# dakom/awsm-renderer

Hardware: AMD Instinct MI355X
Metric: frames/sec + shaded Mpix/s, 4K Sponza glTF, 1/2/4/8 MI355X (higher is better)
Workload: dtype f32; 1 GPU; Sponza-class procedural atrium (configs[3]): 262144 triangles, 25 materials, 69 textures, 3840x2160, geometry pass + opaque pass, single-sample, MipmapMode::None; triangles=262144, width=3840, height=2160, draws=92, frame_overlap=True, stream_handoff=device flags (k_handoff_signal / k_handoff_wait), camera=orbit, one turn per 240 frames, environment=uniform cubes (builder default), opaque_route=lean (k_shade_lean + k_shade_todo), library=awsm-renderer_amd/libawsm_hip.so

## Files before the change

__graft_entry__.py:

```python
import os
import subprocess
import sys

ROOT = os.path.dirname(os.path.abspath(__file__))
if ROOT not in sys.path:
    sys.path.insert(0, ROOT)


def build() -> None:
    import awsm_renderer_amd
    from awsm_renderer_amd import build as b
    hip_so, host_so = b.build_all()
    for p in (hip_so, host_so):
        assert os.path.exists(p), p
    from oracle import oracle_lib
    oracle_lib.build()
    mock_dir = os.path.join(ROOT, "tests", "mock")
    subprocess.check_call(["gcc", "-O1", "-std=c11", "-fPIC", "-shared", "-Wall", "-o", os.path.join(mock_dir, "libmock_backend.so"),
                           os.path.join(mock_dir, "mock_backend.c")])
    from awsm_renderer_amd import hip_backend, host
    host.load_library()
    import ctypes
    lib = ctypes.CDLL(hip_so)
    for name in hip_backend.EXPORTS:
        getattr(lib, name)
    print(f"built {hip_so}, {host_so}, oracle + mock; package {awsm_renderer_amd.__name__} imported")


def smoke() -> None:
    import numpy as np
    from awsm_renderer_amd import scenes
    from awsm_renderer_amd.hip_backend import HipDevice
    from awsm_renderer_amd.host import Renderer
    from oracle import oracle_lib
    from tests import helpers

    scene = scenes.helmet_scene(320, 180, segments=48, rings=36, tex_size=64)
    lut = oracle_lib.brdf_lut(32, 32)
    r = Renderer(scene, parity_tap=True, lut_rgba16f=oracle_lib.lut_rg_to_rgba16f(lut))
    stats = r.render(sync=True)
    dev = HipDevice.from_ctx(r.host.device_ctx, scene.width, scene.height)
    model = helpers.build_model(scene)
    orc = helpers.oracle_frame(model, lut)
    res = helpers.compare_frames(orc, dev)
    dev.close()
    r.close()
    assert res["key_mismatch"] == 0 and res["clip_mismatch"] == 0, res
    assert res["rgb_over_tol"] == 0 and res["f16_max_ulp"] <= 2, res
    print("smoke ok:", {k: stats[k] for k in ("ms_total", "triangles_in", "covered_pixels")}, res)


if __name__ == "__main__":
    build()
    if len(sys.argv) > 1 and sys.argv[1] == "smoke":
        smoke()
```

awsm-renderer_amd/build.py:

```python
from __future__ import annotations

import os
import shutil
import subprocess
import sys

from . import PACKAGE_DIR


def _run_make(directory: str, target: str, env=None):
    e = dict(os.environ)
    if env:
        e.update(env)
    proc = subprocess.run(["make", "-C", directory, target], stdout=subprocess.PIPE, stderr=subprocess.STDOUT, text=True, env=e)
    if proc.returncode != 0:
        raise RuntimeError(f"building {target} in {directory} failed:\n{proc.stdout[-4000:]}")
    return proc.stdout


def build_hip(jobs: int = 3, arch: str = "gfx950") -> str:
    hipcc = shutil.which("hipcc") or "/opt/rocm/bin/hipcc"
    if not os.path.exists(hipcc):
        raise RuntimeError("hipcc not found: libawsm_hip.so cannot be built and there is no CPU fallback")
    proc = subprocess.run(["make", "-C", os.path.join(PACKAGE_DIR, "csrc"), f"-j{jobs}", "../libawsm_hip.so", f"HIPCC={hipcc}", f"ARCH={arch}"],
                          stdout=subprocess.PIPE, stderr=subprocess.STDOUT, text=True)
    if proc.returncode != 0:
        raise RuntimeError(f"hipcc build failed:\n{proc.stdout[-4000:]}")
    try:
        over = check_register_budgets(hipcc, arch)
    except (OSError, subprocess.CalledProcessError) as e:
        print(f"awsm-renderer_amd build: VGPR budgets not checked ({e})", file=sys.stderr)
        over = []
    for line in over:
        print("awsm-renderer_amd build: " + line, file=sys.stderr)
    if over and os.environ.get("AWSM_STRICT_VGPR") == "1":
        raise RuntimeError("VGPR budgets exceeded (AWSM_STRICT_VGPR=1):\n" + "\n".join(over))
    return os.path.join(PACKAGE_DIR, "libawsm_hip.so")


VGPR_BUDGETS = {"kernels_shade.o": {"k_shade_leanILb0ELi0ELb0E": 80, "k_shade_todoILi0ELb0E": 112,
                                    "k_shade_leanILb0ELi0ELb1E": 80, "k_shade_leanILb0ELi1ELb0E": 96, "k_shade_leanILb0ELi1ELb1E": 96,
                                    "k_shade_todoILi1ELb0E": 128, "k_shade_todoILi0ELb1E": 128, "k_shade_todoILi1ELb1E": 128},
                "kernels_geometry.o": {"k_deform_transformILb0E": 80, "k_binILb0E": 112, "k_binILb1E": 112, "k_bin_bigILb0E": 112, "k_bin_scan": 112, "k_raster_tileILi1E": 112, "k_raster_tileILi4E": 96,
                                       "k_handoff_signal": 32, "k_handoff_wait": 32}}


def check_register_budgets(hipcc: str, arch: str = "gfx950") -> list:
    import re
    import tempfile
    llvm = os.path.join(os.path.dirname(os.path.dirname(os.path.realpath(hipcc))), "lib", "llvm", "bin")
    if not os.path.exists(os.path.join(llvm, "llvm-objcopy")):
        llvm = "/opt/rocm/lib/llvm/bin"
    over = []
    with tempfile.TemporaryDirectory() as tmp:
        for obj, budgets in VGPR_BUDGETS.items():
            fat, co = os.path.join(tmp, "fat.bin"), os.path.join(tmp, "code.co")
            subprocess.check_call([os.path.join(llvm, "llvm-objcopy"), f"--dump-section=.hip_fatbin={fat}", os.path.join(PACKAGE_DIR, "csrc", obj)])
            subprocess.check_call([os.path.join(llvm, "clang-offload-bundler"), "--unbundle", "--type=o", f"--targets=hipv4-amdgcn-amd-amdhsa--{arch}", f"--input={fat}", f"--output={co}"])
            notes = subprocess.run([os.path.join(llvm, "llvm-readelf"), "--notes", co], stdout=subprocess.PIPE, text=True, check=True).stdout
            found = dict(re.findall(r"\.name:\s+(\S+)\n(?:.*\n)*?\s+\.vgpr_count:\s+(\d+)", notes))
            for key, budget in budgets.items():
                hits = {n: int(v) for n, v in found.items() if key in n}
                if not hits:
                    over.append(f"{obj}: no kernel matching {key} in the code object (budget list out of date?)")
                for n, v in hits.items():
                    if v > budget:
                        over.append(f"{obj}: {n} uses {v} VGPRs, more than the {budget} it may use to be placed beside k_shade_lean (slower overlap, same results)")
    return over


def build_host() -> str:
    _run_make(os.path.join(PACKAGE_DIR, "host"), "../libawsm_host.so")
    return os.path.join(PACKAGE_DIR, "libawsm_host.so")


def build_all():
    return build_hip(), build_host()
```

awsm-renderer_amd/csrc/awsm_hip.cpp:

```cpp
#include <hip/hip_runtime.h>
#include <algorithm>
#include <cmath>
#include <cstdarg>
#include <cstdio>
#include <cstring>
#include <ctime>
#include <string>
#include <vector>

#include "frame_params.hpp"
#include "dirty_log.hpp"

using namespace awsm;

extern "C" {
void awsm_launch_bin_big(const FrameDev* f, int fill, hipStream_t s);
void awsm_launch_gen_mip_level(uint8_t* chain, uint32_t src_off, uint32_t dst_off, uint32_t sw, uint32_t sh, uint32_t dw, uint32_t dh, uint32_t layers,
                               const uint32_t* kinds, hipStream_t s);
void awsm_launch_pick(const DevScene* sc, const FrameDev* f, int x, int y, uint32_t* out, hipStream_t s);
void awsm_launch_transform(const DevScene* sc, const FrameDev* f, uint32_t n_blocks, hipStream_t s);
void awsm_launch_hud_merge(const unsigned long long* world, const unsigned long long* hud, unsigned long long* out, size_t first, size_t n, hipStream_t s);
void awsm_launch_transform_forward(const DevScene* sc, const FrameDev* f, uint32_t n_blocks, hipStream_t s);
void awsm_launch_forward(const DevScene* sc, const FrameDev* f, hipStream_t s);
void awsm_launch_post(const void* args, uint32_t flags, uint32_t msaa, void* bloom_a, void* bloom_b, hipStream_t s);
void awsm_launch_upload_words(void* dst, const void* src_pinned, uint32_t n_words, hipStream_t s);
void awsm_launch_bin_count(const FrameDev* f, hipStream_t s);
void awsm_launch_bin_scan(const FrameDev* f, hipStream_t s);
void awsm_launch_bin_fill(const FrameDev* f, hipStream_t s);
void awsm_launch_raster(const FrameDev* f, hipStream_t s);
void awsm_launch_shade(const DevScene* sc, const FrameDev* f, hipStream_t s);
int awsm_shade_is_lean(const FrameDev* f);
int awsm_launch_shade_todo(const DevScene* sc, const FrameDev* f, hipStream_t s);
void awsm_launch_gbuffer_dump(const FrameDev* f, float* out, hipStream_t s);
void awsm_launch_handoff_signal(uint32_t* flag, uint32_t serial, unsigned long long* stamp, hipStream_t s);
void awsm_launch_handoff_wait(const uint32_t* flag, uint32_t serial, unsigned long long budget_ticks, uint32_t* timeouts_host, uint32_t timeouts_known,
                              uint32_t* poison, uint32_t poison_serial, hipStream_t s);
void awsm_launch_resolve_draws(const DevScene* sc, const FrameDev* f, hipStream_t s);
void awsm_launch_count_covered(const FrameDev* f, hipStream_t s);
void awsm_launch_msaa_halo_export(const FrameDev* f, unsigned long long* dst, uint32_t bands_out, hipStream_t s);
void awsm_launch_vis_digest(const unsigned long long* vis, size_t n, unsigned long long* out, hipStream_t s);
void awsm_launch_brdf_lut(uint32_t* out_rg16f, uint32_t w, uint32_t h, hipStream_t s);
void awsm_launch_cube_border(const awsm::CubeDev* cd, uint2* out, uint32_t total, hipStream_t s);
void awsm_launch_rgba16f_to_rg16f(const uint16_t* in, uint32_t* out, uint32_t n, hipStream_t s);
}

namespace {

#ifndef AWSM_SLOTS
#define AWSM_SLOTS 2
#endif
constexpr int kSlots = AWSM_SLOTS;
constexpr int kLeanWgsPerCu = 0;
struct DevBuf {
    void* ptr = nullptr;
    size_t size = 0;
};

enum { EV_START = 0, EV_TRANSFORM, EV_BIN, EV_RASTER, EV_SHADE_BEGIN, EV_SHADE_LEAN, EV_SHADE, EV_FWD_BEGIN, EV_FWD, EV_COUNT };

struct FrameBufs {
    DevBuf wpos;
    DevBuf frag_rec, frag_color, frag_first;
    uint32_t frag_cap = 0;
    DevBuf tex_slots;
    DevBuf draw_mat;
    DevBuf tri_shade, draw_lean;
    DevBuf clip, nrm, tan, tri_rec, tri_flags, draws_dev, draw_shade, tile_count, tile_offset, tile_cursor, tile_order, bin_list, big_list, counters, vis;
    DevBuf camera;
    DevBuf scan_tmp;
    DevBuf tile_split, raster_scratch;
    uint32_t raster_extra_cap = 0, raster_slot_cap = 0;
    uint32_t bin_capacity = 0;
    float pix2view[16] = {}, view_rot[9] = {}, cam_pos[3] = {}, ortho_view_dir[3] = {};
    uint32_t cam_ortho = 0;
    size_t tri_cap = 0, draw_cap = 0;
    uint32_t sized_w = 0, sized_h = 0;
    std::vector<DrawDev> draws_uploaded;
    void* draws_uploaded_ptr = nullptr;
    bool draws_uploaded_valid = false;
    uint64_t draws_version = 0;
    std::vector<DrawDev> tail_uploaded;
    void* tail_uploaded_ptr = nullptr;
    size_t tail_uploaded_at = 0;
    bool tail_uploaded_valid = false;
    DevBuf wcache, draws_prev;
    DevBuf block_map;
    bool block_map_valid = false;
    DevBuf cache_mark;
    uint32_t cached_n_draws = 0;
    bool cache_valid = false;
    bool cached_is_prev = false;
    bool cache_had_tri_shade = false;
    uint64_t cache_seq = 0;
    uint32_t cache_serial = 0;
};

}

struct AwsmHipCtx {
    int device = 0;
    uint32_t flags = 0;
    hipStream_t stream = nullptr;
    bool own_stream = false;
    bool stage_timers = true;
    std::string last_error;

    DevBuf bufs[AWSM_BUF_COUNT];
    bool camera_written_since_snapshot = false;
    uint8_t camera_host[512] = {};
    DevScene scene{};
    DevScene* scene_dev = nullptr;
    bool scene_dirty = true;
    DevBuf tex[kMaxTexArrays];
    DevBuf lut;
    DevBuf cube_tex[3], cube_bordered[3];

    uint32_t width = 0, height = 0;
    uint32_t y0 = 0, y1 = 0;
    uint32_t band_n = 1, band_r = 0, band_compact = 0;
    uint32_t msaa = 0;
    DevBuf mip_kinds;
    DevBuf msaa_color0[kSlots], msaa_edges[kSlots];
    DevBuf msaa_edge_bits[kSlots];
    DevBuf msaa_cells[kSlots];
    DevBuf out16[kSlots], out32[kSlots];
    DevBuf digest;
    uint32_t lean_grid = 0;
    DevBuf shade_todo[kSlots];
    void* bound_out = nullptr;
    size_t bound_out_bytes = 0;
    const uint8_t* slot_out_lo[kSlots] = {}; const uint8_t* slot_out_hi[kSlots] = {};

    bool overlap = false;
    hipStream_t shade_streams[kSlots] = {};
    bool shade_recorded[kSlots] = {};
    bool uploads_recorded[kSlots] = {};
    struct ResolveKey { uint64_t write_seq, draws_version; const void* ptrs[5]; uint32_t n_draws, mipmap, has_opaque, lights_cap; } resolved[kSlots] = {};
    hipEvent_t ev_geom_done[kSlots] = {}, ev_shade_done[kSlots] = {}, ev_uploads[kSlots] = {} ;
    hipEvent_t ev_flush = nullptr;
    uint64_t write_seq = 0, geom_write_seq[kSlots] = {};
    DirtyLog dirty_log;
    bool geometry_cache = true;
    uint32_t cache_blocks_last = 0;
    bool shade_pending[kSlots] = {};
    bool handoff = false;
    uint32_t* handoff_flags = nullptr;
    uint32_t geom_sig[kSlots] = {}, shade_sig[kSlots] = {}, lean_sig[kSlots] = {};
    bool lean_flagged[kSlots] = {};
    unsigned long long handoff_budget_ticks = 400000000ull;
    uint32_t clock_khz = 100000;
// ... 190 lines not shown
    if (rc) return rc;
    memcpy(st, src, len);
    if (len <= kKernelUploadMax && (len & 3u) == 0 && ((uintptr_t)dst & 3u) == 0 && ((uintptr_t)st & 3u) == 0) {
        awsm_launch_upload_words(dst, st, (uint32_t)(len >> 2), c->stream);
        HIPCHK(c, hipGetLastError());
    } else {
        HIPCHK(c, hipMemcpyAsync(dst, st, len, hipMemcpyHostToDevice, c->stream));
    }
    return AWSM_OK;
}

void shard(const AwsmHipCtx* c, uint32_t* y0, uint32_t* y1) {
    *y0 = c->y0; *y1 = c->y1;
    if (*y1 == 0 || *y1 > c->height) *y1 = c->height;
    if (*y0 > *y1) *y0 = *y1;
}

void log_dirty(AwsmHipCtx* c, AwsmBuf which, size_t lo, size_t hi) {
    if (c->geometry_cache) c->dirty_log.log((uint32_t)which, lo, hi, c->write_seq);
}

int scene_write_barrier(AwsmHipCtx* c, bool is_write = true) {
    if (is_write) c->write_seq++;
    if (!c->overlap) return AWSM_OK;
    for (int s = 0; s < kSlots; s++)
        if (c->shade_pending[s]) { HIPCHK(c, hipStreamWaitEvent(c->stream, c->ev_shade_done[s], 0)); c->shade_pending[s] = false; }
    return AWSM_OK;
}
int sync_all(AwsmHipCtx* c) {
    HIPCHK(c, hipStreamSynchronize(c->stream));
    HIPCHK(c, sync_shade_streams(c));
    for (bool& b : c->shade_pending) b = false;
    return AWSM_OK;
}

int sync_scene(AwsmHipCtx* c) {
    if (!c->scene_dirty) return AWSM_OK;
    c->write_seq++;
    { int rcb = scene_write_barrier(c, false); if (rcb) return rcb; }
    for (int i = 0; i < AWSM_BUF_COUNT; i++) c->scene.buf[i] = (const uint8_t*)c->bufs[i].ptr;
    c->scene.lut_rg16f = (const uint16_t*)c->lut.ptr;
    int rc = upload_small(c, c->scene_dev, &c->scene, sizeof(DevScene));
    if (rc) return rc;
    c->scene_dirty = false;
    return AWSM_OK;
}

void fill_frame(AwsmHipCtx* c, FrameDev* f) {
    memset(f, 0, sizeof *f);
    uint32_t y0, y1;
    shard(c, &y0, &y1);
    f->width = c->width; f->height = c->height; f->y0 = y0; f->y1 = y1; f->sy0 = y0; f->sy1 = y1;
    if (c->msaa && (y0 > 0 || y1 < c->height)) {
        f->y0 = y0 > 0 ? y0 - 1 : 0; f->y1 = std::min(c->height, y1 + 1);
    }
    f->tiles_x = (c->width + kTile - 1) / kTile;
    f->band_n = 1; f->band_r = 0; f->out_compact = 0;
    f->tile_row0 = f->y0 >> kTileShift;
    f->tiles_y = (f->y1 > f->y0) ? ((f->y1 + kTile - 1) / kTile - f->tile_row0) : 0;
    if (c->band_n > 1) {
        const uint32_t rows_full = (c->height + kTile - 1) / kTile;
        f->band_n = c->band_n; f->band_r = c->band_r; f->out_compact = c->band_compact;
        f->tile_row0 = c->band_r;
        f->tiles_y = c->band_r < rows_full ? (rows_full - c->band_r + c->band_n - 1) / c->band_n : 0;
    }
    f->n_draws = (uint32_t)c->draws_host.size();
    f->total_tris = c->total_tris; f->total_verts = c->total_verts;
    f->bin_capacity = FB(c).bin_capacity;
    f->draws = (const DrawDev*)FB(c).draws_dev.ptr;
    f->draw_shade = (DrawShadeDev*)FB(c).draw_shade.ptr;
    f->tex_slots = (TexSlotDev*)FB(c).tex_slots.ptr;
    f->draw_mat = (DrawMatDev*)FB(c).draw_mat.ptr;
    f->clip = (float4*)FB(c).clip.ptr; f->nrm = (float4*)FB(c).nrm.ptr; f->tan = (float4*)FB(c).tan.ptr;
    f->tri_info = (uint32_t*)FB(c).tri_flags.ptr;
    const bool lean_ok = !(c->flags & AWSM_CFG_GENERAL_SHADE_ONLY) && (uint64_t)c->width * c->height * (c->msaa == 4 ? 32u : 8u) < (1ull << 32) && (c->msaa == 0 || (c->msaa_edge_bits[c->slot].ptr && c->msaa_cells[c->slot].ptr)) && FB(c).tri_shade.ptr && FB(c).draw_lean.ptr && c->shade_todo[c->slot].ptr && ((uint64_t)c->total_tris + (c->hud_merged ? c->hud_total_tris : 0u)) * kTriRecBytes < (1ull << 32) &&
                         c->bufs[AWSM_BUF_ATTR_DATA].size < (1ull << 32) - 64;
    f->tri_shade = lean_ok ? (uint4*)FB(c).tri_shade.ptr : nullptr;
    f->attr_data_bytes = (uint32_t)std::min<size_t>(c->bufs[AWSM_BUF_ATTR_DATA].size, 0xFFFFFFFFu);
    f->draw_lean = lean_ok ? (LeanDrawDev*)FB(c).draw_lean.ptr : nullptr;
    f->shade_todo = (uint32_t*)c->shade_todo[c->slot].ptr;
    f->shade_todo_cap = f->shade_todo ? (uint32_t)(c->shade_todo[c->slot].size / 4 - 4 - 1024) : 0u;
    f->lean_next = f->shade_todo ? f->shade_todo + 4 + f->shade_todo_cap : nullptr;
    f->lean_grid = c->lean_grid;
    f->tri_rec = (TriRec*)FB(c).tri_rec.ptr;
    f->tile_count = (uint32_t*)FB(c).tile_count.ptr; f->tile_offset = (uint32_t*)FB(c).tile_offset.ptr;
    f->tile_cursor = (uint32_t*)FB(c).tile_cursor.ptr; f->bin_list = (uint32_t*)FB(c).bin_list.ptr;
    f->tile_order = (uint32_t*)FB(c).tile_order.ptr;
    f->scan_tmp = (uint32_t*)FB(c).scan_tmp.ptr;
    f->tile_split = (uint32_t*)FB(c).tile_split.ptr; f->raster_scratch = (unsigned long long*)FB(c).raster_scratch.ptr;
    f->raster_extra_cap = FB(c).raster_extra_cap; f->raster_slot_cap = FB(c).raster_slot_cap;
    f->big_list = (uint32_t*)FB(c).big_list.ptr;
    f->counters = (uint32_t*)FB(c).counters.ptr;
#ifdef AWSM_STAMP
    {
        static unsigned long long* stamps = nullptr;
        if (!stamps && hipMalloc((void**)&stamps, 4ull * 16384 * 8 * 8) == hipSuccess) (void)hipMemset(stamps, 0, 4ull * 16384 * 8 * 8);
        f->stamps = stamps;
        static bool told = false;
        if (!told) { told = true; FILE* fp = fopen("/tmp/awsm_stamps_ptr", "w"); if (fp) { fprintf(fp, "%llu\n", (unsigned long long)(uintptr_t)stamps); fclose(fp); } }
    }
#endif
    f->poison = c->handoff_poison ? c->handoff_poison + c->slot : nullptr;
    f->host_bin_status = c->counters_host + 16 + 2 * c->slot;
    f->frame_serial = c->frame_serial;
    f->vis = (unsigned long long*)FB(c).vis.ptr;
    f->camera = (const uint8_t*)FB(c).camera.ptr;
    f->camera_snap = nullptr; f->camera_snap_words = 0;
    memcpy(f->pix2view, FB(c).pix2view, sizeof f->pix2view); memcpy(f->view_rot, FB(c).view_rot, sizeof f->view_rot); memcpy(f->cam_pos, FB(c).cam_pos, sizeof f->cam_pos);
    memcpy(f->ortho_view_dir, FB(c).ortho_view_dir, sizeof f->ortho_view_dir); f->cam_ortho = FB(c).cam_ortho;
    f->msaa = c->msaa;
    f->msaa_color0 = (float4*)c->msaa_color0[c->slot].ptr;
    f->msaa_edges = (uint32_t*)c->msaa_edges[c->slot].ptr;
    f->msaa_edge_bits = (lean_ok && c->msaa == 4) ? (unsigned long long*)c->msaa_edge_bits[c->slot].ptr : nullptr;
    f->msaa_cells = (uint2*)c->msaa_cells[c->slot].ptr;
    f->hud_vis = c->hud_geometry_done ? (const unsigned long long*)c->hud[c->slot].vis.ptr : nullptr;
    f->hud_draws = (const DrawDev*)c->hud[c->slot].draws_dev.ptr; f->hud_tri_info = (const uint32_t*)c->hud[c->slot].tri_flags.ptr;
    if (c->hud_geometry_done && c->hud_merged) {
        f->n_draws = (uint32_t)c->hud_combined.size();
        f->total_tris = c->total_tris + c->hud_total_tris; f->total_verts = 3u * f->total_tris;
        f->vis = (unsigned long long*)c->merged_vis[c->slot].ptr;
        f->hud_draws = f->draws; f->hud_tri_info = f->tri_info;
    }
    f->hud_pass = 0;
    f->msaa_halo = (const unsigned long long*)c->msaa_halo;
    f->halo_bands = c->band_n > 1 ? ((c->height + kTile - 1) / kTile + c->band_n - 1) / c->band_n : 0u;
    f->out_rgba16f = (uint16_t*)(c->bound_out ? (uint8_t*)c->bound_out - (size_t)c->out_first_row * c->width * 8 : c->out16[c->slot].ptr);
    f->out_rgba32f = (float*)c->out32[c->slot].ptr;
    f->lights_pre = (float4*)c->lights_pre[c->slot].ptr;
    f->lights_cap = (uint32_t)(c->lights_pre[c->slot].size / 32);
}

void compose_pixel_to_view(AwsmHipCtx* c, FrameBufs& b) {
    float cam[128];
    memcpy(cam, c->camera_host, 512);
    const float* proj = cam + 16; const float* inv_proj = cam + 64; const float* inv_view = cam + 80;
    const double W = (double)c->width, H = (double)c->height;
    const double A[16] = {2.0 / W, 0, 0, 0,   0, -2.0 / H, 0, 0,   0, 0, 1, 0,   1.0 / W - 1.0, 1.0 - 1.0 / H, 0, 1};
    for (int col = 0; col < 4; col++) for (int row = 0; row < 4; row++) {
        double s = 0.0;
        for (int k = 0; k < 4; k++) s += (double)inv_proj[k * 4 + row] * A[col * 4 + k];
        b.pix2view[col * 4 + row] = (float)s;
    }
    for (int col = 0; col < 3; col++) for (int row = 0; row < 3; row++) b.view_rot[col * 3 + row] = inv_view[col * 4 + row];
    for (int i = 0; i < 3; i++) b.cam_pos[i] = cam[96 + i];
    b.cam_ortho = proj[15] > 0.9f ? 1u : 0u;
    const double vx = inv_view[8], vy = inv_view[9], vz = inv_view[10], l = std::sqrt(vx * vx + vy * vy + vz * vz);
    b.ortho_view_dir[0] = l > 0.0 ? (float)(vx / l) : 0.0f; b.ortho_view_dir[1] = l > 0.0 ? (float)(vy / l) : 0.0f; b.ortho_view_dir[2] = l > 0.0 ? (float)(vz / l) : 1.0f;
}

int record(AwsmHipCtx* c, int which, hipStream_t s = nullptr) {
    if (!c->stage_timers) { c->ev_valid[which] = false; return AWSM_OK; }
    HIPCHK(c, hipEventRecord(c->ev[which], s ? s : c->stream));
    c->ev_valid[which] = true;
    return AWSM_OK;
}

AwsmHipCtx::ResolveKey resolve_key(AwsmHipCtx* c, const FrameDev& f) {
    AwsmHipCtx::ResolveKey k;
    memset(&k, 0, sizeof k);
    k.write_seq = c->write_seq + (c->scene_dirty ? 1u : 0u); k.draws_version = FB(c).draws_version;
    k.ptrs[0] = f.draw_shade; k.ptrs[1] = f.draw_mat; k.ptrs[2] = f.tex_slots; k.ptrs[3] = f.draw_lean; k.ptrs[4] = f.lights_pre;
    k.n_draws = f.n_draws; k.mipmap = c->last_opaque.mipmap; k.has_opaque = c->last_opaque.has_opaque; k.lights_cap = f.lights_cap;
    return k;
}
bool resolve_stale(AwsmHipCtx* c, const FrameDev& f) {
    const AwsmHipCtx::ResolveKey k = resolve_key(c, f);
    return memcmp(&k, &c->resolved[c->slot], sizeof k) != 0;
// ... 82 lines not shown
    HostTrace ht(c->frame_serial);
    FrameDev f;
    fill_frame(c, &f);
    f.has_opaque = c->last_opaque.has_opaque;
    f.mipmap = c->last_opaque.mipmap;
    f.aniso = (c->flags & AWSM_CFG_ANISOTROPIC) ? 1u : 0u;
    if (c->bound_out) {
        if (c->out_rows_mode) {
            if (f.out_compact || f.sy0 < c->out_first_row || (size_t)(f.sy1 - c->out_first_row) * c->width * 8 > c->bound_out_bytes)
                return fail(c, AWSM_ERR_INVALID_ARGUMENT, "opaque_pass: bound output starts at row %u and holds %zu bytes, the shard shades rows [%u, %u)", c->out_first_row, c->bound_out_bytes, f.sy0, f.sy1);
        } else {
            const size_t need = (f.out_compact ? (size_t)f.tiles_y * kTile : (size_t)c->height) * c->width * 8;
            if (c->bound_out_bytes < need) return fail(c, AWSM_ERR_INVALID_ARGUMENT, "opaque_pass: bound output holds %zu bytes, this shard layout writes %zu", c->bound_out_bytes, need);
        }
    }
    int rc = sync_scene(c);
    if (rc) return rc;
    hipStream_t ss = shade_stream_of(c);
    const bool want_resolve = f.sy1 > f.sy0 && f.has_opaque && (resolve_stale(c, f) || c->stage_timers);
    if (want_resolve) c->resolved[c->slot] = resolve_key(c, f);
    const bool early = c->uploads_recorded[c->slot] && c->overlap && !c->stage_timers && want_resolve && c->geometry_done && c->geom_write_seq[c->slot] == c->write_seq;
    if (early) {
        HIPCHK(c, hipStreamWaitEvent(ss, c->ev_uploads[c->slot], 0));
        awsm_launch_resolve_draws(c->scene_dev, &f, ss);
    }
    ht.mark("opaque: sync_scene + early resolve");
    if (c->overlap) {
        if (c->handoff) {
            ++c->geom_sig[c->slot];
            if (c->handoff_test_drop) c->handoff_test_drop--;
            else awsm_launch_handoff_signal(c->handoff_flags + c->slot, c->geom_sig[c->slot], trace_slot(c, 1), c->stream);
            awsm_launch_handoff_wait(c->handoff_flags + c->slot, c->geom_sig[c->slot], c->handoff_budget_ticks, handoff_timeouts(c), c->handoff_timeouts_seen, c->handoff_poison + c->slot, c->frame_serial, ss);
        } else {
            if (c->trace_dev) awsm_launch_handoff_signal(nullptr, 0u, trace_slot(c, 1), c->stream);
            HIPCHK(c, hipEventRecord(c->ev_geom_done[c->slot], c->stream));
            HIPCHK(c, hipStreamWaitEvent(ss, c->ev_geom_done[c->slot], 0));
        }
        const uint8_t* lo = (const uint8_t*)c->bound_out; const uint8_t* hi = lo ? lo + c->bound_out_bytes : nullptr;
        const int p = prev_slot(c);
        const bool same_image = lo && c->slot_out_lo[p] && lo < c->slot_out_hi[p] && c->slot_out_lo[p] < hi;
        if (c->shade_recorded[p]) HIPCHK(c, wait_prev_slot(c, ss, !(same_image || (c->msaa != 0 && c->msaa_halo))));
        c->slot_out_lo[c->slot] = lo; c->slot_out_hi[c->slot] = hi;
    }
    ht.mark("opaque: hand-off launches");
    if (want_resolve && !early) awsm_launch_resolve_draws(c->scene_dev, &f, ss);
    if ((rc = record(c, EV_SHADE_BEGIN, ss))) return rc;
    c->ev_valid[EV_SHADE_LEAN] = false;
    c->lean_flagged[c->slot] = false;
    if (c->overlap && c->handoff && f.sy1 > f.sy0 && awsm_shade_is_lean(&f)) {
        f.lean_done_flag = c->handoff_flags + 2 * kSlots + c->slot; f.lean_done_serial = ++c->lean_sig[c->slot];
        c->lean_flagged[c->slot] = true;
    }
    if (f.sy1 > f.sy0) {
        awsm_launch_shade(c->scene_dev, &f, ss);
        if (c->stage_timers && awsm_shade_is_lean(&f) && (rc = record(c, EV_SHADE_LEAN, ss))) return rc;
        (void)awsm_launch_shade_todo(c->scene_dev, &f, ss);
    }
    if ((rc = record(c, EV_SHADE, ss))) return rc;
    ht.mark("opaque: shade launches");
    if (c->overlap) HIPCHK(c, mark_shade_done(c, ss));
    else if (c->trace_dev) awsm_launch_handoff_signal(nullptr, 0u, trace_slot(c, 2), ss);
    ht.mark("opaque: shade-done signal + event");
    HIPCHK(c, hipGetLastError());
    return AWSM_OK;
}

inline FrameBufs& TR(AwsmHipCtx* c) { return (c->hud_transparent ? c->htr : c->tr)[c->slot]; }

void fill_frame_forward(AwsmHipCtx* c, FrameDev* f) {
    fill_frame(c, f);
    FrameBufs& t = TR(c);
    const int which = c->hud_transparent ? 1 : 0;
    f->vis = (unsigned long long*)FB(c).vis.ptr;
    f->n_draws = (uint32_t)c->tr_draws_host[which].size();
    f->total_tris = c->tr_total_tris[which]; f->total_verts = 3u * c->tr_total_tris[which];
    f->bin_capacity = t.bin_capacity;
    f->draws = (const DrawDev*)t.draws_dev.ptr;
    f->draw_shade = (DrawShadeDev*)t.draw_shade.ptr;
    f->tex_slots = (TexSlotDev*)t.tex_slots.ptr;
    f->draw_mat = (DrawMatDev*)t.draw_mat.ptr;
    f->clip = (float4*)t.clip.ptr; f->nrm = (float4*)t.nrm.ptr; f->tan = (float4*)t.tan.ptr; f->wpos = (float4*)t.wpos.ptr;
    f->tri_info = (uint32_t*)t.tri_flags.ptr;
    f->tri_shade = nullptr; f->draw_lean = nullptr; f->shade_todo = nullptr; f->shade_todo_cap = 0; f->lean_next = nullptr; f->lean_grid = 0;
    f->tri_rec = (TriRec*)t.tri_rec.ptr;
    f->tile_count = (uint32_t*)t.tile_count.ptr; f->tile_offset = (uint32_t*)t.tile_offset.ptr;
    f->tile_cursor = (uint32_t*)t.tile_cursor.ptr; f->bin_list = (uint32_t*)t.bin_list.ptr;
    f->tile_order = (uint32_t*)t.tile_order.ptr;
    f->scan_tmp = (uint32_t*)t.scan_tmp.ptr;
    f->tile_split = (uint32_t*)t.tile_split.ptr; f->raster_scratch = nullptr;
    f->raster_extra_cap = 0; f->raster_slot_cap = 0;
    f->big_list = (uint32_t*)t.big_list.ptr;
    f->counters = (uint32_t*)t.counters.ptr;
    f->opaque_rgba16f = c->opaque_src ? (const uint16_t*)c->opaque_src : f->out_rgba16f;
    f->out_compact = 0;
    f->frag_rec = (uint4*)t.frag_rec.ptr; f->frag_color = (float4*)t.frag_color.ptr; f->frag_first = (uint32_t*)t.frag_first.ptr; f->frag_cap = t.frag_cap;
    f->out_rgba16f = (uint16_t*)(c->bound_comp ? c->bound_comp : c->comp16.ptr);
    f->out_rgba32f = (float*)c->comp32.ptr;
    f->has_opaque = c->last_opaque.has_opaque;
    f->mipmap = c->last_opaque.mipmap;
    f->aniso = (c->flags & AWSM_CFG_ANISOTROPIC) ? 1u : 0u;
    if (c->hud_transparent) {
        f->hud_pass = 1;
        f->opaque_rgba16f = f->out_rgba16f;
    }
}

int enqueue_transparent(AwsmHipCtx* c) {
    FrameDev f;
    fill_frame_forward(c, &f);
    const uint32_t n_tiles = f.tiles_x * f.tiles_y;
    int rc = sync_scene(c);
    if (rc) return rc;
    hipStream_t ss = shade_stream_of(c);
    if (c->overlap && c->shade_recorded[prev_slot(c)]) HIPCHK(c, wait_prev_slot(c, ss));
    if ((rc = record(c, EV_FWD_BEGIN, ss))) return rc;
    const bool has_geometry = f.total_tris && n_tiles;
    if (!has_geometry) {
        HIPCHK(c, hipMemsetAsync(TR(c).counters.ptr, 0, 8 * sizeof(uint32_t), ss));
        HIPCHK(c, hipMemsetAsync((uint32_t*)TR(c).counters.ptr + 12, 0, 2 * sizeof(uint32_t), ss));
        if (n_tiles) HIPCHK(c, hipMemsetAsync(TR(c).tile_count.ptr, 0, n_tiles * sizeof(uint32_t), ss));
    } else {
        awsm_launch_resolve_draws(c->scene_dev, &f, ss);
        awsm_launch_transform_forward(c->scene_dev, &f, c->tr_n_blocks[c->hud_transparent ? 1 : 0], ss);
    }
    if (n_tiles) {
        if (f.total_tris) { awsm_launch_bin_count(&f, ss); awsm_launch_bin_big(&f, 0, ss); }
        awsm_launch_bin_scan(&f, ss);
        if (f.total_tris) { awsm_launch_bin_fill(&f, ss); awsm_launch_bin_big(&f, 1, ss); }
        awsm_launch_forward(c->scene_dev, &f, ss);
    }
    if ((rc = record(c, EV_FWD, ss))) return rc;
    if (c->overlap) HIPCHK(c, mark_shade_done(c, ss));
    HIPCHK(c, hipGetLastError());
    return AWSM_OK;
}

int ensure_bin_capacity_of(AwsmHipCtx* c, FrameBufs& b, uint32_t entries) {
    if (entries <= b.bin_capacity && b.bin_list.ptr) return AWSM_OK;
    uint32_t cap = std::max(entries, b.bin_capacity + b.bin_capacity / 2);
    int rc = dev_realloc(c, b.bin_list, (size_t)cap * 4, false);
    if (rc) return rc;
    b.bin_capacity = cap;
    return AWSM_OK;
}

int ensure_fragment_capacity(AwsmHipCtx* c, FrameBufs& b, uint32_t fragments) {
    if (fragments <= b.frag_cap && b.frag_rec.ptr) return AWSM_OK;
    const uint32_t cap = std::max(fragments, b.frag_cap + b.frag_cap / 2);
    int rc = dev_realloc(c, b.frag_rec, (size_t)cap * 16, false);
    if (!rc) rc = dev_realloc(c, b.frag_color, (size_t)cap * 16, false);
    if (rc) return rc;
    b.frag_cap = cap;
    return AWSM_OK;
}

int build_draw_list(AwsmHipCtx* c, const char* pass, const AwsmDraw* draws, uint32_t n, AwsmBuf data, uint32_t bytes_per_tri,
                    std::vector<DrawDev>& out, uint64_t* tris_out, uint64_t* blocks_out) {
    out.clear();
    uint64_t tris = 0, blocks = 0;
    for (uint32_t i = 0; i < n; i++) {
        const AwsmDraw& d = draws[i];
        if (d.inst_count != 0) {
            const DevBuf& ib = c->bufs[AWSM_BUF_INSTANCES];
            if (!ib.ptr) return fail(c, AWSM_ERR_NOT_READY, "%s: draw %u: instanced, but the instance-transform buffer was never created", pass, i);
            if ((d.inst_off & 15u) || (uint64_t)d.inst_off + 64ull * d.inst_count > ib.size)
                return fail(c, AWSM_ERR_OUT_OF_RANGE, "%s: draw %u: %u instances at %u exceed the instance-transform buffer", pass, i, d.inst_count, d.inst_off);
        }
        if (d.vis_data_off & (bytes_per_tri ? 15u : 3u)) return fail(c, AWSM_ERR_INVALID_ARGUMENT, "%s: draw %u: vertex data offset %u misaligned", pass, i, d.vis_data_off);
        if ((uint64_t)d.vis_data_off + (uint64_t)bytes_per_tri * d.tri_count > c->bufs[data].size || (!bytes_per_tri && d.tri_count && (uint64_t)d.vis_data_off + 40 > c->bufs[data].size))
            return fail(c, AWSM_ERR_OUT_OF_RANGE, "%s: draw %u: %u triangles at %u exceed the vertex buffer", pass, i, d.tri_count, d.vis_data_off);
        if ((uint64_t)d.geom_meta_off + 40 > c->bufs[AWSM_BUF_GEOM_META].size || (d.geom_meta_off & 3u))
            return fail(c, AWSM_ERR_OUT_OF_RANGE, "%s: draw %u: geometry meta offset %u out of range", pass, i, d.geom_meta_off);
        if (d.tri_count == 0) continue;
        const uint32_t copies = d.inst_count ? d.inst_count : 1u;
        for (uint32_t k = 0; k < copies; k++) {
            DrawDev dd{};
            dd.geom_meta_off = d.geom_meta_off; dd.vis_data_off = d.vis_data_off; dd.tri_count = d.tri_count; dd.flags = d.flags & 0x7Fu;
            if (d.inst_count) { dd.flags |= kDrawInstanced; dd.inst_off = d.inst_off + 64u * k; }
            dd.first_tri = (uint32_t)tris; dd.first_block = (uint32_t)blocks;
            out.push_back(dd);
            tris += d.tri_count;
            blocks += (3ull * d.tri_count + 255) / 256;
            if (tris > 0x55555555ull) return fail(c, AWSM_ERR_UNSUPPORTED, "%s: more than 2^32/3 triangles in one pass", pass);
            if (out.size() >= (1u << 24)) return fail(c, AWSM_ERR_UNSUPPORTED, "%s: more than 2^24 non-empty draws (instances included) in one pass", pass);
        }
    }
    *tris_out = tris; *blocks_out = blocks;
    return AWSM_OK;
}

int reserve_raster_items(AwsmHipCtx* c, FrameBufs& b, bool forward) {
    const uint32_t tiles_x = (c->width + kTile - 1) / kTile, tiles_y_full = (c->height + kTile - 1) / kTile;
    const size_t n_tiles_full = (size_t)tiles_x * tiles_y_full;
    const uint32_t extra_cap = forward ? 0u : b.bin_capacity / 256u + 1u, slot_cap = forward ? 0u : b.bin_capacity / 128u + 2u;
    int rc;
    if ((rc = dev_reserve(c, b.tile_order, (n_tiles_full + extra_cap) * 4))) return rc;
    if (!forward && (rc = dev_reserve(c, b.raster_scratch, (size_t)slot_cap * kTile * kTile * 8 * (c->msaa == 4u ? 4u : 1u)))) return rc;
    b.raster_extra_cap = extra_cap; b.raster_slot_cap = slot_cap;
    return AWSM_OK;
}

int size_pass_buffers(AwsmHipCtx* c, FrameBufs& b, size_t tri_cap, size_t draw_cap, bool forward) {
    int rc;
    const size_t nd = std::max<size_t>(draw_cap, 1), nv = std::max<size_t>(3 * tri_cap, 1), nt = std::max<size_t>(tri_cap, 1);
    if ((rc = dev_reserve(c, b.draws_dev, nd * sizeof(DrawDev)))) return rc;
    const bool world_pass = &b >= c->fb && &b < c->fb + kSlots;
    if (world_pass && c->geometry_cache) {
        if ((rc = dev_reserve(c, b.draws_prev, nd * sizeof(DrawDev)))) return rc;
        if ((rc = dev_reserve(c, b.wcache, nv * 16))) return rc;
        const size_t blocks_bound = nv / 256 + nd + 1;
        if ((rc = dev_reserve(c, b.block_map, blocks_bound * 4))) return rc;
        b.block_map_valid = false;
        if (b.cache_mark.size < blocks_bound * 4) { if ((rc = dev_realloc(c, b.cache_mark, (blocks_bound + blocks_bound / 2) * 4, true))) return rc; }
    }
    b.cache_valid = false;
    if ((rc = dev_reserve(c, b.draw_shade, nd * sizeof(DrawShadeDev)))) return rc;
    if ((rc = dev_reserve(c, b.tex_slots, nd * kCoreTextures * sizeof(TexSlotDev)))) return rc;
    if ((rc = dev_reserve(c, b.draw_mat, nd * sizeof(DrawMatDev)))) return rc;
    if ((rc = dev_reserve(c, b.clip, nv * 16))) return rc;
    if ((rc = dev_reserve(c, b.nrm, nv * 16))) return rc;
    if ((rc = dev_reserve(c, b.tan, nv * 16))) return rc;
    if (forward && (rc = dev_reserve(c, b.wpos, nv * 16))) return rc;
    if ((rc = dev_reserve(c, b.tri_flags, nt * 4))) return rc;
    if (!forward && (rc = dev_reserve(c, b.tri_shade, nt * 32))) return rc;
    if (!forward && (rc = dev_reserve(c, b.draw_lean, nd * sizeof(LeanDrawDev)))) return rc;
    if ((rc = dev_reserve(c, b.big_list, nt * 4))) return rc;
    if ((rc = dev_reserve(c, b.tri_rec, nt * kTriRecBytes))) return rc;
    const uint32_t tiles_x = (c->width + kTile - 1) / kTile, tiles_y_full = (c->height + kTile - 1) / kTile;
    const size_t n_tiles_full = (size_t)tiles_x * tiles_y_full;
    if ((rc = dev_reserve(c, b.tile_count, n_tiles_full * 4))) return rc;
    if ((rc = dev_reserve(c, b.tile_offset, (n_tiles_full + 1) * 4))) return rc;
    if ((rc = dev_reserve(c, b.tile_cursor, n_tiles_full * 4))) return rc;
    if ((rc = dev_reserve(c, b.tile_split, n_tiles_full * 8))) return rc;
    if ((rc = dev_reserve(c, b.scan_tmp, (((n_tiles_full + 255) / 256) * 2 + 1) * 40 * 4))) return rc;
    if ((rc = ensure_bin_capacity_of(c, b, (c->flags & AWSM_CFG_SMALL_BIN_LIST) ? 4096u : (uint32_t)std::min<size_t>(std::max<size_t>(4 * tri_cap + 65536u, 1u << 18), 0xFFFFFFF0u)))) return rc;
    if ((rc = reserve_raster_items(c, b, forward))) return rc;
    b.tri_cap = tri_cap; b.draw_cap = draw_cap; b.sized_w = c->width; b.sized_h = c->height;
    return AWSM_OK;
}

int ensure_pass_capacity(AwsmHipCtx* c, FrameBufs& b, const std::vector<DrawDev>& draws_host, uint32_t total_tris, bool forward) {
    int rc;
    if (total_tris > b.tri_cap || draws_host.size() > b.draw_cap || b.sized_w != c->width || b.sized_h != c->height || !b.bin_list.ptr) {
        bool instanced = false;
        for (const DrawDev& d : draws_host) instanced |= (d.flags & kDrawInstanced) != 0;
        const size_t tri_bound = forward || instanced ? ~size_t(0) : c->bufs[AWSM_BUF_VIS_GEOM_DATA].size / 168u;
        const size_t tri_cap = std::max<size_t>(std::min<size_t>((size_t)total_tris + total_tris / 4 + 4096, std::max<size_t>(tri_bound, total_tris)), b.tri_cap);
        const size_t draw_cap = std::max<size_t>(draws_host.size() + draws_host.size() / 4 + 64, b.draw_cap);
        FrameBufs* set = forward ? ((&b >= c->htr && &b < c->htr + kSlots) ? c->htr : c->tr) : ((&b >= c->hud && &b < c->hud + kSlots) ? c->hud : c->fb);
        for (int sl = 0; sl < n_slots(c); sl++) {
            FrameBufs& t = set[(c->slot + sl) % kSlots];
            if ((rc = size_pass_buffers(c, t, std::max(tri_cap, t.tri_cap), std::max(draw_cap, t.draw_cap), forward))) return rc;
        }
    }
    return AWSM_OK;
}

int upload_draws_at(AwsmHipCtx* c, FrameBufs& b, size_t at, const std::vector<DrawDev>& list) {
    const size_t bytes = list.size() * sizeof(DrawDev);
    uint8_t* dst = (uint8_t*)b.draws_dev.ptr + at * sizeof(DrawDev);
    if (bytes <= (1u << 20)) return upload_small(c, dst, list.data(), bytes);
    HIPCHK(c, hipMemcpyAsync(dst, list.data(), bytes, hipMemcpyHostToDevice, c->stream));
    HIPCHK(c, hipStreamSynchronize(c->stream));
    return AWSM_OK;
}

int upload_draw_list(AwsmHipCtx* c, FrameBufs& b, const std::vector<DrawDev>& draws_host, bool keep_prev) {
    const bool same_draws = b.draws_uploaded_valid && b.draws_uploaded_ptr == b.draws_dev.ptr && b.draws_uploaded.size() == draws_host.size() &&
                            (draws_host.empty() || memcmp(b.draws_uploaded.data(), draws_host.data(), draws_host.size() * sizeof(DrawDev)) == 0);
    auto upload_block_map = [&]() -> int {
        b.block_map_valid = false;
        if (!keep_prev || !b.block_map.ptr) return AWSM_OK;
        std::vector<uint32_t> map;
        for (size_t i = 0; i < draws_host.size(); i++) map.insert(map.end(), (3ull * draws_host[i].tri_count + 255) / 256, (uint32_t)i);
        if (map.size() * 4 > b.block_map.size || map.size() * 4 > (1u << 20)) return AWSM_OK;
        const int rc = upload_small(c, b.block_map.ptr, map.data(), map.size() * 4);
        if (!rc) b.block_map_valid = true;
        return rc;
    };
    if (draws_host.empty()) return AWSM_OK;
    if (same_draws) return (keep_prev && !b.block_map_valid) ? upload_block_map() : AWSM_OK;
    if (keep_prev && b.cache_valid && !b.cached_is_prev && b.draws_prev.ptr && b.draws_prev.size == b.draws_dev.size) {
        std::swap(b.draws_dev, b.draws_prev);
        b.cached_is_prev = true;
    } else if (keep_prev && !b.cached_is_prev) b.cache_valid = false;
    b.draws_uploaded = draws_host; b.draws_uploaded_ptr = b.draws_dev.ptr; b.draws_uploaded_valid = true; b.draws_version++;
    b.tail_uploaded_valid = false;
    { const int rc = upload_block_map(); if (rc) return rc; }
    return upload_draws_at(c, b, 0, draws_host);
}

int reserve_pass_buffers(AwsmHipCtx* c, FrameBufs& b, const std::vector<DrawDev>& draws_host, uint32_t total_tris, bool forward) {
    int rc = ensure_pass_capacity(c, b, draws_host, total_tris, forward);
    if (rc) return rc;
    return upload_draw_list(c, b, draws_host, !forward && &b >= c->fb && &b < c->fb + kSlots);
}

uint32_t mip_levels_full(uint32_t w, uint32_t h) {
    uint32_t m = std::max(w, h), n = 0;
    while (m > 1u) { m >>= 1; n++; }
    return n + 1u;
}

int ensure_bin_capacity(AwsmHipCtx* c, uint32_t entries) { return ensure_bin_capacity_of(c, FB(c), entries); }

}

extern "C" {

uint32_t awsm_hip_abi_version(void) { return AWSM_HIP_ABI_VERSION; }
// ... 20 lines not shown
    }
    if (cfg->stream) { c->stream = (hipStream_t)cfg->stream; c->own_stream = false; }
    else { if (hipStreamCreateWithFlags(&c->stream, hipStreamNonBlocking) != hipSuccess) return bail(AWSM_ERR_DEVICE); c->own_stream = true; }
    for (int i = 0; i < EV_COUNT; i++) if (hipEventCreate(&c->ev[i]) != hipSuccess) return bail(AWSM_ERR_DEVICE);
    if (hipMalloc((void**)&c->scene_dev, sizeof(DevScene)) != hipSuccess) return bail(AWSM_ERR_OUT_OF_MEMORY);
    c->overlap = (cfg->flags & AWSM_CFG_OVERLAP_FRAMES) != 0;
    { const char* e = getenv("AWSM_GEOMETRY_CACHE"); c->geometry_cache = !(e && e[0] == '0'); }
    {
        const char* e = getenv("AWSM_LEAN_WGS_PER_CU");
        const int per_cu = e ? atoi(e) : (c->overlap ? kLeanWgsPerCu : 0);
        c->lean_grid = per_cu > 0 ? (uint32_t)(per_cu * prop.multiProcessorCount) & ~7u : 0u;
    }
    for (int s = 0; s < n_slots(c); s++) {
        if (hipMalloc(&c->fb[s].counters.ptr, 16 * sizeof(uint32_t)) != hipSuccess || hipMemset(c->fb[s].counters.ptr, 0, 16 * sizeof(uint32_t)) != hipSuccess) return bail(AWSM_ERR_OUT_OF_MEMORY);
        c->fb[s].counters.size = 16 * sizeof(uint32_t);
        if (hipMalloc(&c->tr[s].counters.ptr, 16 * sizeof(uint32_t)) != hipSuccess) return bail(AWSM_ERR_OUT_OF_MEMORY);
        c->tr[s].counters.size = 16 * sizeof(uint32_t);
        if (hipMalloc(&c->htr[s].counters.ptr, 16 * sizeof(uint32_t)) != hipSuccess) return bail(AWSM_ERR_OUT_OF_MEMORY);
        c->htr[s].counters.size = 16 * sizeof(uint32_t);
        if (hipMalloc(&c->hud[s].counters.ptr, 16 * sizeof(uint32_t)) != hipSuccess) return bail(AWSM_ERR_OUT_OF_MEMORY);
        c->hud[s].counters.size = 16 * sizeof(uint32_t);
        if (hipMalloc(&c->fb[s].camera.ptr, 512) != hipSuccess || hipMemset(c->fb[s].camera.ptr, 0, 512) != hipSuccess) return bail(AWSM_ERR_OUT_OF_MEMORY);
        c->fb[s].camera.size = 512;
    }

    if (c->overlap) {
        for (int s = 0; s < kSlots; s++) {
#ifdef AWSM_DEBUG_SWITCHES
            if (const char* m = getenv("AWSM_SHADE_CU_MASK")) {
                std::vector<uint32_t> words;
                for (const char* p = m; *p; ) { char* end = nullptr; words.push_back((uint32_t)strtoul(p, &end, 16)); p = (*end == ',') ? end + 1 : end; if (end == p && *p) break; }
                if (words.empty() || hipExtStreamCreateWithCUMask(&c->shade_streams[s], (uint32_t)words.size(), words.data()) != hipSuccess) return bail(AWSM_ERR_DEVICE);
            } else
#endif
            if (hipStreamCreateWithFlags(&c->shade_streams[s], hipStreamNonBlocking) != hipSuccess) return bail(AWSM_ERR_DEVICE);
            const unsigned ev_flags = hipEventDisableTiming | hipEventReleaseToDevice;
            if (hipEventCreateWithFlags(&c->ev_geom_done[s], ev_flags) != hipSuccess || hipEventCreateWithFlags(&c->ev_shade_done[s], ev_flags) != hipSuccess ||
                hipEventCreateWithFlags(&c->ev_uploads[s], ev_flags) != hipSuccess) return bail(AWSM_ERR_DEVICE);
            if (s == 0 && hipEventCreateWithFlags(&c->ev_flush, hipEventDisableTiming) != hipSuccess) return bail(AWSM_ERR_DEVICE);
        }
    }
    if (hipHostMalloc((void**)&c->counters_host, (16 + 2 * kSlots + 1) * sizeof(uint32_t), hipHostMallocDefault) != hipSuccess) return bail(AWSM_ERR_OUT_OF_MEMORY);
    memset(c->counters_host, 0, (16 + 2 * kSlots + 1) * sizeof(uint32_t));
    if (c->overlap) {
        const char* e = getenv("AWSM_DEVICE_HANDOFF");
        c->handoff = !(e && e[0] == '0');
        { int khz = 0; if (hipDeviceGetAttribute(&khz, hipDeviceAttributeWallClockRate, c->device) == hipSuccess && khz > 0) c->clock_khz = (uint32_t)khz; }
        double budget_ms = 4000.0;
        if (const char* p = getenv("AWSM_HANDOFF_TIMEOUT_MS")) { const double v = atof(p); if (v > 0.0) budget_ms = v; }
        c->handoff_budget_ticks = (unsigned long long)(budget_ms * (double)c->clock_khz) + 1ull;
        if (hipMalloc((void**)&c->handoff_flags, 3 * kSlots * sizeof(uint32_t)) != hipSuccess || hipMalloc((void**)&c->handoff_poison, kSlots * sizeof(uint32_t)) != hipSuccess) return bail(AWSM_ERR_OUT_OF_MEMORY);
        if (hipMemset(c->handoff_flags, 0, 3 * kSlots * sizeof(uint32_t)) != hipSuccess || hipMemset(c->handoff_poison, 0xFF, kSlots * sizeof(uint32_t)) != hipSuccess ||
            hipDeviceSynchronize() != hipSuccess) return bail(AWSM_ERR_DEVICE);
        if (const char* d = getenv("AWSM_TEST_HANDOFF_DROP")) c->handoff_test_drop = (uint32_t)atoi(d);
        for (int k = 0; c->handoff && k < 2 * kSlots; k++) {
            hipStream_t ss = c->shade_streams[k % kSlots], waiter = k < kSlots ? ss : c->stream, setter = k < kSlots ? c->stream : ss;
            const uint32_t serial = ++c->geom_sig[0];
            awsm_launch_handoff_wait(c->handoff_flags, serial, 10ull * c->clock_khz , handoff_timeouts(c), 0u, nullptr, 0u, waiter);
            awsm_launch_handoff_signal(c->handoff_flags, serial, nullptr, setter);
            if (hipStreamSynchronize(waiter) != hipSuccess || hipStreamSynchronize(setter) != hipSuccess) return bail(AWSM_ERR_DEVICE);
            if (*(volatile uint32_t*)handoff_timeouts(c) != 0u) { c->handoff = false; c->handoff_timeouts_seen = *(volatile uint32_t*)handoff_timeouts(c); }
        }
    }
    memset(&c->scene, 0, sizeof c->scene);
    c->scene.skybox_rgba[3] = 1.0f;
    for (int i = 0; i < 3; i++) { c->scene.prefiltered_rgb[i] = 1.0f; c->scene.irradiance_rgb[i] = 1.0f; }
    *out = c;
    return AWSM_OK;
}

int awsm_hip_destroy(AwsmHipCtx* c) {
    if (!c) return AWSM_ERR_INVALID_ARGUMENT;
    (void)hipSetDevice(c->device);
    if (c->stream) (void)hipStreamSynchronize(c->stream);
    (void)sync_shade_streams(c);
    auto fr = [](DevBuf& b) { if (b.ptr) (void)hipFree(b.ptr); b.ptr = nullptr; b.size = 0; };
    for (auto& b : c->bufs) fr(b);
    for (auto& b : c->tex) fr(b);
    for (auto& b : c->merged_vis) fr(b);
    fr(c->lut); for (auto& b : c->cube_tex) fr(b); for (auto& b : c->cube_bordered) fr(b); fr(c->digest); for (auto& b : c->shade_todo) fr(b); for (int sl = 0; sl < kSlots; sl++) { fr(c->msaa_color0[sl]); fr(c->msaa_edges[sl]); fr(c->msaa_edge_bits[sl]); fr(c->msaa_cells[sl]); } fr(c->mip_kinds); for (auto& b : c->out16) fr(b); for (auto& b : c->out32) fr(b); fr(c->comp16); fr(c->comp32); for (auto& b : c->lights_pre) fr(b);
    for (auto& b : c->display8) fr(b); fr(c->effects16); fr(c->bloom_a); fr(c->bloom_b); fr(c->dof_lc); fr(c->dof_blur);
    for (int k = 0; k < 4 * kSlots; k++) {
        FrameBufs& b = k < kSlots ? c->fb[k] : (k < 2 * kSlots ? c->tr[k - kSlots] : (k < 3 * kSlots ? c->hud[k - 2 * kSlots] : c->htr[k - 3 * kSlots]));
        fr(b.vis); fr(b.wpos); fr(b.frag_rec); fr(b.frag_color); fr(b.frag_first); fr(b.tex_slots); fr(b.draw_mat); fr(b.clip); fr(b.nrm); fr(b.tan); fr(b.tri_rec); fr(b.tri_flags); fr(b.tri_shade); fr(b.draw_lean); fr(b.draws_dev); fr(b.draw_shade); fr(b.tile_count); fr(b.tile_offset);
        fr(b.wcache); fr(b.draws_prev); fr(b.cache_mark); fr(b.block_map); fr(b.tile_cursor); fr(b.tile_order); fr(b.scan_tmp); fr(b.tile_split); fr(b.raster_scratch); fr(b.bin_list); fr(b.big_list); fr(b.counters); fr(b.camera);
    }
    for (hipStream_t st : c->shade_streams) if (st) (void)hipStreamDestroy(st);
    for (int i = 0; i < kSlots; i++) { if (c->ev_geom_done[i]) (void)hipEventDestroy(c->ev_geom_done[i]); if (c->ev_shade_done[i]) (void)hipEventDestroy(c->ev_shade_done[i]); if (c->ev_uploads[i]) (void)hipEventDestroy(c->ev_uploads[i]); }
    if (c->ev_flush) (void)hipEventDestroy(c->ev_flush);
    if (c->scene_dev) (void)hipFree(c->scene_dev);
    if (c->stage) (void)hipHostFree(c->stage);
    if (c->counters_host) (void)hipHostFree(c->counters_host);
    if (c->handoff_flags) (void)hipFree(c->handoff_flags);
    if (c->handoff_poison) (void)hipFree(c->handoff_poison);
    if (c->trace_dev) (void)hipFree(c->trace_dev);
    for (int i = 0; i < EV_COUNT; i++) if (c->ev[i]) (void)hipEventDestroy(c->ev[i]);
    if (c->own_stream && c->stream) (void)hipStreamDestroy(c->stream);
    delete c;
    return AWSM_OK;
}

int awsm_hip_device_info(AwsmHipCtx* c, char* name_out, size_t name_cap, uint32_t* cu_count, uint64_t* hbm_bytes) {
    if (!c) return AWSM_ERR_INVALID_ARGUMENT;
    hipDeviceProp_t prop;
    HIPCHK(c, hipGetDeviceProperties(&prop, c->device));
    if (name_out && name_cap) snprintf(name_out, name_cap, "%s (%s)", prop.name, prop.gcnArchName);
    if (cu_count) *cu_count = (uint32_t)prop.multiProcessorCount;
    if (hbm_bytes) *hbm_bytes = (uint64_t)prop.totalGlobalMem;
    return AWSM_OK;
}

int awsm_hip_buffer_create(AwsmHipCtx* c, AwsmBuf which, size_t bytes) {
    if (!c || (int)which < 0 || which >= AWSM_BUF_COUNT) return fail(c, AWSM_ERR_INVALID_ARGUMENT, "buffer_create: bad buffer id %d", (int)which);
    HIPCHK(c, hipSetDevice(c->device));
    { int rcb = scene_write_barrier(c); if (rcb) return rcb; }
    log_dirty(c, which, 0, ~size_t(0));
    if (bytes && c->bufs[which].ptr && c->bufs[which].size == bytes) {
        if (which == AWSM_BUF_CAMERA) memset(c->camera_host, 0, sizeof c->camera_host);
        HIPCHK(c, hipMemsetAsync(c->bufs[which].ptr, 0, bytes + 16, c->stream));
        return AWSM_OK;
    }
    int rc = dev_realloc(c, c->bufs[which], bytes ? bytes + 16 : 0, true);
    if (rc) return rc;
    if (bytes) c->bufs[which].size = bytes;
    if (which == AWSM_BUF_CAMERA) memset(c->camera_host, 0, sizeof c->camera_host);
    if (which == AWSM_BUF_LIGHTS) for (int sl = 0; sl < n_slots(c); sl++) if ((rc = dev_realloc(c, c->lights_pre[sl], std::max<size_t>(bytes / 64, 1) * 32, true))) return rc;
    c->scene_dirty = true;
    return AWSM_OK;
}

int awsm_hip_buffer_write(AwsmHipCtx* c, AwsmBuf which, size_t dst_off, const void* src, size_t len) {
    if (!c || (int)which < 0 || which >= AWSM_BUF_COUNT || (!src && len)) return fail(c, AWSM_ERR_INVALID_ARGUMENT, "buffer_write: bad argument");
    if ((dst_off & 3) || (len & 3)) return fail(c, AWSM_ERR_INVALID_ARGUMENT, "buffer_write: offset %zu / size %zu not 4-byte aligned", dst_off, len);
    DevBuf& b = c->bufs[which];
    if (!b.ptr) return fail(c, AWSM_ERR_NOT_READY, "buffer_write: buffer %d was never created", (int)which);
    if (dst_off > b.size || len > b.size - dst_off) return fail(c, AWSM_ERR_OUT_OF_RANGE, "buffer_write: [%zu,+%zu) outside buffer %d of %zu bytes", dst_off, len, (int)which, b.size);
    if (len == 0) return AWSM_OK;
    HIPCHK(c, hipSetDevice(c->device));
    if (which != AWSM_BUF_CAMERA) { int rcb = scene_write_barrier(c); if (rcb) return rcb; log_dirty(c, which, dst_off, dst_off + len); }
    else { if (dst_off < 512) memcpy(c->camera_host + dst_off, src, std::min<size_t>(len, 512 - dst_off)); c->camera_written_since_snapshot = true; }
    uint8_t* dst = (uint8_t*)b.ptr + dst_off;
    if (len <= (1u << 20)) return upload_small(c, dst, src, len);
    HIPCHK(c, hipMemcpyAsync(dst, src, len, hipMemcpyHostToDevice, c->stream));
    HIPCHK(c, hipStreamSynchronize(c->stream));
    return AWSM_OK;
}

int awsm_hip_resize(AwsmHipCtx* c, uint32_t width, uint32_t height, uint32_t msaa) {
    if (!c || width == 0 || height == 0 || width > 16384 || height > 16384) return fail(c, AWSM_ERR_INVALID_ARGUMENT, "resize: bad size %ux%u", width, height);
    if (msaa == 1) msaa = 0;
    if (msaa != 0 && msaa != 4) return fail(c, AWSM_ERR_UNSUPPORTED, "resize: MSAA x%u (the reference supports None or 4, anti_alias.rs:28-38)", msaa);
    HIPCHK(c, hipSetDevice(c->device));
    const size_t px = (size_t)width * height, samples = msaa == 4 ? 4 : 1;
    int rc;
    if ((rc = sync_all(c))) return rc;
    for (int s = 0; s < n_slots(c); s++) {
        if ((rc = dev_realloc(c, c->fb[s].vis, px * samples * 8, false))) return rc;
        HIPCHK(c, hipMemsetAsync(c->fb[s].vis.ptr, 0xFF, px * samples * 8, c->stream));
    }
    if (msaa == 4) for (int sl = 0; sl < n_slots(c); sl++) {
        const size_t blocks = (size_t)((width + 15) / 16) * ((height + 15) / 16);
        if ((rc = dev_realloc(c, c->msaa_edge_bits[sl], blocks * 4 * 16, true))) return rc;
        if ((rc = dev_realloc(c, c->msaa_cells[sl], px * 8, false))) return rc;
        if ((rc = dev_realloc(c, c->msaa_color0[sl], px * 16, false))) return rc;
        if ((rc = dev_realloc(c, c->msaa_edges[sl], blocks * 260, false))) return rc;
    }
    c->msaa = msaa;
// ... 197 lines not shown
    c->scene_dirty = true;
    return AWSM_OK;
}

int awsm_hip_read_brdf_lut(AwsmHipCtx* c, uint16_t* out) {
    if (!c || !out) return AWSM_ERR_INVALID_ARGUMENT;
    if (!c->lut.ptr) return fail(c, AWSM_ERR_NOT_READY, "no BRDF LUT");
    HIPCHK(c, hipSetDevice(c->device));
    HIPCHK(c, hipStreamSynchronize(c->stream));
    HIPCHK(c, hipMemcpy(out, c->lut.ptr, (size_t)c->scene.lut_w * c->scene.lut_h * 4, hipMemcpyDeviceToHost));
    return AWSM_OK;
}

int awsm_hip_geometry_pass(AwsmHipCtx* c, const AwsmDraw* draws, uint32_t n) {
    if (!c || (!draws && n)) return AWSM_ERR_INVALID_ARGUMENT;
    if (c->width == 0) return fail(c, AWSM_ERR_NOT_READY, "geometry_pass before resize");
    static const AwsmBuf need[] = {AWSM_BUF_TRANSFORMS, AWSM_BUF_CAMERA, AWSM_BUF_GEOM_META, AWSM_BUF_VIS_GEOM_DATA};
    if (n) for (AwsmBuf b : need) if (!c->bufs[b].ptr) return fail(c, AWSM_ERR_NOT_READY, "geometry_pass: buffer %d missing", (int)b);
    HIPCHK(c, hipSetDevice(c->device));

    HostTrace ht(c->frame_serial + 1u);
    std::vector<DrawDev> new_draws;
    uint64_t tris = 0, blocks = 0;
    int rc = build_draw_list(c, "geometry_pass", draws, n, AWSM_BUF_VIS_GEOM_DATA, 168u, new_draws, &tris, &blocks);
    if (rc) return rc;
    ht.mark("geometry_pass: draw list");
    if ((rc = handoff_check(c))) return rc;
    c->hud_geometry_done = false; c->hud_merged = false;
    c->frame_serial++;
    if (c->overlap) {
        c->slot = (c->slot + 1) % kSlots;
        if (c->shade_pending[c->slot]) {
            if (hipEventQuery(c->ev_shade_done[c->slot]) != hipSuccess) HIPCHK(c, wait_slot_free(c));
            c->shade_pending[c->slot] = false;
        }
    }
    ht.mark("geometry_pass: slot-free wait");
    c->draws_api.assign(draws, draws + n);
    c->draws_host.swap(new_draws);
    {
        uint32_t need = 0;
        for (int s = 0; s < kSlots; s++) {
            const volatile uint32_t* st = c->counters_host + 16 + 2 * s;
            const uint32_t entries = st[0], serial = st[1];
            if (serial == c->status_seen[s]) continue;
            c->status_seen[s] = serial;
            if (serial >> 31) c->dropped_frames++;
            need = std::max(need, entries);
        }
        for (int s = 0; s < n_slots(c); s++)
            if (need && (uint64_t)need * 4 > (uint64_t)c->fb[s].bin_capacity * 3 && c->fb[s].bin_list.ptr && !(c->flags & AWSM_CFG_SMALL_BIN_LIST)) {
                if ((rc = ensure_bin_capacity_of(c, c->fb[s], need + need / 2 + 1024))) return rc;
                if ((rc = reserve_raster_items(c, c->fb[s], false))) return rc;
            }
    }
    c->total_tris = (uint32_t)tris; c->total_verts = (uint32_t)(3 * tris); c->n_blocks = (uint32_t)blocks;
    ht.mark("geometry_pass: bin capacity");
    compose_pixel_to_view(c, FB(c));
    if ((rc = reserve_pass_buffers(c, FB(c), c->draws_host, c->total_tris, false))) return rc;
    ht.mark("geometry_pass: reserve + draw-list upload");
    if ((rc = enqueue_geometry(c))) return rc;
    c->camera_written_since_snapshot = false;
    c->geometry_done = true; c->opaque_done = false; c->transparent_done = false; c->hud_transparent_done = false; c->hud_geometry_done = false; c->post_done = false;
    return AWSM_OK;
}

static int enqueue_hud_geometry(AwsmHipCtx* c) {
    FrameBufs& hb = c->hud[c->slot];
    FrameDev f;
    { const bool hd = c->hud_geometry_done; c->hud_geometry_done = false; fill_frame(c, &f); c->hud_geometry_done = hd; }
    f.bin_capacity = hb.bin_capacity;
    f.shade_todo = nullptr; f.shade_todo_cap = 0; f.lean_next = nullptr; f.lean_grid = 0;
    if (c->hud_merged) {
        f.n_draws = (uint32_t)c->hud_combined.size();
        f.total_tris = c->total_tris + c->hud_total_tris; f.total_verts = 3u * f.total_tris;
        f.rank0 = c->total_tris; f.block0 = c->n_blocks;
    } else {
    f.n_draws = (uint32_t)c->hud_draws_host.size();
    f.total_tris = c->hud_total_tris; f.total_verts = 3u * c->hud_total_tris;
    f.draws = (const DrawDev*)hb.draws_dev.ptr;
    f.clip = (float4*)hb.clip.ptr; f.nrm = (float4*)hb.nrm.ptr; f.tan = (float4*)hb.tan.ptr;
    f.tri_info = (uint32_t*)hb.tri_flags.ptr;
    f.tri_shade = nullptr; f.draw_lean = nullptr;
    f.tri_rec = (TriRec*)hb.tri_rec.ptr;
    }
    f.tile_count = (uint32_t*)hb.tile_count.ptr; f.tile_offset = (uint32_t*)hb.tile_offset.ptr;
    f.tile_cursor = (uint32_t*)hb.tile_cursor.ptr; f.bin_list = (uint32_t*)hb.bin_list.ptr;
    f.tile_order = (uint32_t*)hb.tile_order.ptr; f.scan_tmp = (uint32_t*)hb.scan_tmp.ptr;
    f.tile_split = (uint32_t*)hb.tile_split.ptr; f.raster_scratch = (unsigned long long*)hb.raster_scratch.ptr;
    f.raster_extra_cap = hb.raster_extra_cap; f.raster_slot_cap = hb.raster_slot_cap;
    f.big_list = (uint32_t*)hb.big_list.ptr;
    f.counters = (uint32_t*)hb.counters.ptr;
    f.host_bin_status = nullptr;
    f.camera_snap = nullptr; f.camera_snap_words = 0;
    f.vis = (unsigned long long*)hb.vis.ptr;
    f.hud_vis = nullptr;
    int rc;
    if ((rc = sync_scene(c))) return rc;
    const uint32_t n_tiles = f.tiles_x * f.tiles_y;
    awsm_launch_transform(c->scene_dev, &f, c->hud_n_blocks, c->stream);
    if (n_tiles) {
        awsm_launch_bin_count(&f, c->stream); awsm_launch_bin_big(&f, 0, c->stream);
        awsm_launch_bin_scan(&f, c->stream);
        awsm_launch_bin_fill(&f, c->stream); awsm_launch_bin_big(&f, 1, c->stream);
        awsm_launch_raster(&f, c->stream);
    }
    if (c->hud_merged) {
        const size_t spp = c->msaa == 4 ? 4 : 1, first = (size_t)f.y0 * c->width * spp, n = (size_t)(f.y1 - f.y0) * c->width * spp;
        awsm_launch_hud_merge((const unsigned long long*)FB(c).vis.ptr, (const unsigned long long*)hb.vis.ptr, (unsigned long long*)c->merged_vis[c->slot].ptr, first, n, c->stream);
    }
    HIPCHK(c, hipGetLastError());
    return AWSM_OK;
}

int awsm_hip_hud_geometry_pass(AwsmHipCtx* c, const AwsmDraw* draws, uint32_t n) {
    if (!c || (!draws && n)) return AWSM_ERR_INVALID_ARGUMENT;
    if (!c->geometry_done || c->opaque_done) return fail(c, AWSM_ERR_NOT_READY, "hud_geometry_pass goes between the geometry pass and the opaque pass of a frame");
    HIPCHK(c, hipSetDevice(c->device));
    uint64_t tris = 0, blocks = 0;
    int rc = build_draw_list(c, "hud_geometry_pass", draws, n, AWSM_BUF_VIS_GEOM_DATA, 168u, c->hud_draws_host, &tris, &blocks);
    if (rc) return rc;
    c->hud_total_tris = (uint32_t)tris; c->hud_n_blocks = (uint32_t)blocks;
    c->hud_merged = false;
    if (!tris) { c->hud_geometry_done = false; return AWSM_OK; }
    FrameBufs& hb = c->hud[c->slot];
    const size_t px = (size_t)c->width * c->height, spp = c->msaa == 4 ? 4 : 1;
    if ((rc = dev_reserve(c, hb.vis, px * 8 * spp))) return rc;
    if ((rc = reserve_pass_buffers(c, hb, c->hud_draws_host, c->hud_total_tris, false))) return rc;
    if (c->msaa == 4) {
        if ((uint64_t)c->total_tris + tris > 0x55555555ull) return fail(c, AWSM_ERR_UNSUPPORTED, "hud_geometry_pass: more than 2^32/3 triangles in the frame");
        c->hud_combined = c->draws_host;
        for (DrawDev d : c->hud_draws_host) { d.first_tri += c->total_tris; d.first_block += c->n_blocks; c->hud_combined.push_back(d); }
        if (c->hud_combined.size() >= (1u << 24)) return fail(c, AWSM_ERR_UNSUPPORTED, "hud_geometry_pass: more than 2^24 draws in the frame");
        FrameBufs& wb = FB(c);
        const void* before[3] = {wb.clip.ptr, wb.tri_rec.ptr, wb.tri_flags.ptr};
        if ((rc = ensure_pass_capacity(c, wb, c->hud_combined, c->total_tris + c->hud_total_tris, false))) return rc;
        if ((rc = upload_draw_list(c, wb, c->draws_host, true))) return rc;
        {
            const size_t at = c->draws_host.size();
            const std::vector<DrawDev> tail(c->hud_combined.begin() + (long)at, c->hud_combined.end());
            const bool same = wb.tail_uploaded_valid && wb.tail_uploaded_ptr == wb.draws_dev.ptr && wb.tail_uploaded_at == at && wb.tail_uploaded.size() == tail.size() &&
                              memcmp(wb.tail_uploaded.data(), tail.data(), tail.size() * sizeof(DrawDev)) == 0;
            if (!same) {
                if ((rc = upload_draws_at(c, wb, at, tail))) return rc;
                wb.tail_uploaded = tail; wb.tail_uploaded_ptr = wb.draws_dev.ptr; wb.tail_uploaded_at = at; wb.tail_uploaded_valid = true; wb.draws_version++;
                c->uploads_recorded[c->slot] = false;
            }
        }
        if ((rc = dev_reserve(c, c->merged_vis[c->slot], px * 8 * spp))) return rc;
        if (before[0] != wb.clip.ptr || before[1] != wb.tri_rec.ptr || before[2] != wb.tri_flags.ptr) {
            if ((rc = enqueue_geometry(c, true))) return rc;
        }
        c->hud_merged = true;
    }
    if ((rc = enqueue_hud_geometry(c))) return rc;
    c->hud_geometry_done = true;
    return AWSM_OK;
}

int awsm_hip_opaque_pass(AwsmHipCtx* c, const AwsmOpaqueParams* p) {
    if (!c || !p) return AWSM_ERR_INVALID_ARGUMENT;
    if (p->mipmap > 1) return fail(c, AWSM_ERR_INVALID_ARGUMENT, "opaque_pass: mipmap must be 0 (MipmapMode::None) or 1 (MipmapMode::Gradient)");
    if (c->width == 0) return fail(c, AWSM_ERR_NOT_READY, "opaque_pass before resize");
    if (p->has_opaque) {
        if (!c->geometry_done) return fail(c, AWSM_ERR_NOT_READY, "opaque_pass before geometry_pass");
        static const AwsmBuf need[] = {AWSM_BUF_CAMERA, AWSM_BUF_GEOM_META, AWSM_BUF_MATERIAL_META, AWSM_BUF_MATERIALS, AWSM_BUF_ATTR_INDEX,
                                       AWSM_BUF_ATTR_DATA, AWSM_BUF_TEXTURE_TRANSFORMS, AWSM_BUF_LIGHTS_INFO, AWSM_BUF_LIGHTS};
        for (AwsmBuf b : need) if (!c->bufs[b].ptr) return fail(c, AWSM_ERR_NOT_READY, "opaque_pass: buffer %d missing", (int)b);
        if (!c->lut.ptr) return fail(c, AWSM_ERR_NOT_READY, "opaque_pass: no BRDF LUT (env_upload or brdf_lut_generate)");
    }
    if (c->msaa == 4 && c->band_n > 1 && p->has_opaque) {
        const size_t need = (size_t)c->band_n * awsm_hip_msaa_halo_bands(c) * 2 * c->width * 8;
        if (!c->msaa_halo || c->msaa_halo_bytes < need)
            return fail(c, AWSM_ERR_NOT_READY, "opaque_pass: MSAA with band sharding needs the gathered halo keys (awsm_hip_msaa_halo_export -> all-gather -> awsm_hip_msaa_halo_bind, %zu bytes)", need);
    }
    HIPCHK(c, hipSetDevice(c->device));
    c->last_opaque = *p;
    if (!p->has_opaque && c->camera_written_since_snapshot && c->bufs[AWSM_BUF_CAMERA].ptr) {
        int rcs = sync_all(c);
        if (rcs) return rcs;
        compose_pixel_to_view(c, FB(c));
        HIPCHK(c, hipMemcpy(FB(c).camera.ptr, c->bufs[AWSM_BUF_CAMERA].ptr, std::min<size_t>(512, c->bufs[AWSM_BUF_CAMERA].size), hipMemcpyDeviceToDevice));
        c->camera_written_since_snapshot = false;
    }
    int rc = enqueue_opaque(c);
    if (rc) return rc;
    c->opaque_done = true; c->transparent_done = false; c->hud_transparent_done = false;
    return AWSM_OK;
}

static int transparent_pass_body(AwsmHipCtx* c, const AwsmDraw* draws, uint32_t n, bool hud);
static int transparent_pass_impl(AwsmHipCtx* c, const AwsmDraw* draws, uint32_t n, bool hud) {
    const int rc = transparent_pass_body(c, draws, n, hud);
    if (c) c->hud_transparent = false;
    return rc;
}
static int transparent_pass_body(AwsmHipCtx* c, const AwsmDraw* draws, uint32_t n, bool hud) {
    if (!c || (!draws && n)) return AWSM_ERR_INVALID_ARGUMENT;
    if (!c->geometry_done || !c->opaque_done) return fail(c, AWSM_ERR_NOT_READY, "transparent_pass needs the geometry and opaque passes of the same frame first");
    if (hud && !c->transparent_done) return fail(c, AWSM_ERR_NOT_READY, "hud_transparent_pass draws over the composite: call transparent_pass first (n_draws = 0 is valid)");
    c->hud_transparent = hud;
    const bool sharded = c->band_n > 1 || (c->y1 != 0 && !(c->y0 == 0 && c->y1 >= c->height));
    if (sharded && !c->opaque_src)
        return fail(c, AWSM_ERR_UNSUPPORTED, "transparent_pass on a sharded context: screen-space transmission reads the whole opaque image — gather it and bind it with awsm_hip_bind_opaque_source first");
    if (c->opaque_src && c->opaque_src_bytes < (size_t)c->width * c->height * 8)
        return fail(c, AWSM_ERR_INVALID_ARGUMENT, "transparent_pass: the bound opaque source holds %zu bytes, the frame needs %zu", c->opaque_src_bytes, (size_t)c->width * c->height * 8);
    static const AwsmBuf need[] = {AWSM_BUF_TRANSFORMS, AWSM_BUF_CAMERA, AWSM_BUF_GEOM_META, AWSM_BUF_MATERIAL_META, AWSM_BUF_MATERIALS, AWSM_BUF_ATTR_INDEX,
                                   AWSM_BUF_ATTR_DATA, AWSM_BUF_TEXTURE_TRANSFORMS, AWSM_BUF_LIGHTS_INFO, AWSM_BUF_LIGHTS, AWSM_BUF_TRANSPARENCY_GEOM_DATA};
    if (n) {
        for (AwsmBuf b : need) if (!c->bufs[b].ptr) return fail(c, AWSM_ERR_NOT_READY, "transparent_pass: buffer %d missing", (int)b);
        if (!c->lut.ptr) return fail(c, AWSM_ERR_NOT_READY, "transparent_pass: no BRDF LUT (env_upload or brdf_lut_generate)");
    }
    HIPCHK(c, hipSetDevice(c->device));
    uint64_t tris = 0, blocks = 0;
    const int which = hud ? 1 : 0;
    int rc = build_draw_list(c, hud ? "hud_transparent_pass" : "transparent_pass", draws, n, AWSM_BUF_TRANSPARENCY_GEOM_DATA, 0u, c->tr_draws_host[which], &tris, &blocks);
    if (rc) return rc;
    c->tr_total_tris[which] = (uint32_t)tris; c->tr_n_blocks[which] = (uint32_t)blocks;
    const size_t px = (size_t)c->width * c->height;
    if (!c->bound_comp && (rc = dev_reserve(c, c->comp16, px * 8))) return rc;
    if (c->bound_comp && c->bound_comp_bytes < px * 8) return fail(c, AWSM_ERR_INVALID_ARGUMENT, "transparent_pass: bound composite holds %zu bytes, the frame needs %zu", c->bound_comp_bytes, px * 8);
    if ((c->flags & AWSM_CFG_PARITY_TAP) && (rc = dev_reserve(c, c->comp32, px * 16))) return rc;
    if ((rc = reserve_pass_buffers(c, TR(c), c->tr_draws_host[which], c->tr_total_tris[which], true))) return rc;
    if ((rc = dev_reserve(c, TR(c).frag_first, px * 4))) return rc;
    if ((rc = ensure_fragment_capacity(c, TR(c), (c->flags & AWSM_CFG_SMALL_BIN_LIST) ? 4096u : (uint32_t)std::max<size_t>(px / 2, 1u << 20)))) return rc;
    if (c->overlap) {
        HIPCHK(c, hipEventRecord(c->ev_geom_done[c->slot], c->stream));
        HIPCHK(c, hipStreamWaitEvent(shade_stream_of(c), c->ev_geom_done[c->slot], 0));
    }
    if ((rc = enqueue_transparent(c))) return rc;
    if (hud) c->hud_transparent_done = true; else { c->transparent_done = true; c->hud_transparent_done = false; }
    return AWSM_OK;
}
// ... 426 lines not shown
```

awsm-renderer_amd/csrc/frame_params.hpp:

```cpp
#pragma once
#include <hip/hip_runtime.h>
#include <stdint.h>
#include "../../include/awsm_hip.h"

namespace awsm {

constexpr int kTile = 32;
constexpr int kTileShift = 5;
constexpr int kMaxTexArrays = 64;
constexpr int kMaxSamplers = 32;

constexpr uint32_t kDrawInstanced = 0x80u;

struct DrawDev {
    uint32_t geom_meta_off;
    uint32_t vis_data_off;
    uint32_t tri_count;
    uint32_t flags;
    uint32_t first_tri;
    uint32_t first_block;
    uint32_t inst_off;
    uint32_t pad1;
};

struct DrawShadeDev {
    uint32_t first_tri;
    uint32_t material_word;
    uint32_t attr_indices_word;
    uint32_t attr_data_word;
    uint32_t stride_words;
    uint32_t uv_sets_index;
    uint32_t flags;
    uint32_t color_sets;
};

struct TexSlotDev {
    const uint32_t* base;
    uint32_t width, height;
    uint32_t flags;
    float tt[6];
    uint32_t layer_levels;
    const uint32_t* level_off;
    const uint32_t* array_base;
};
static_assert(sizeof(TexSlotDev) == 64, "TexSlotDev must be 64 bytes");
constexpr int kCoreTextures = 5;

struct DrawMatDev {
    float base_color[4];
    float metallic, roughness, normal_scale, occlusion_strength;
    float emissive[3];
    float ior;
    uint32_t shader_alpha;
    uint32_t debug_bitmask;
    uint32_t ext_mask;
    float alpha_cutoff;
};
static_assert(sizeof(DrawMatDev) == 64, "DrawMatDev must be 64 bytes");

struct LeanDrawDev {
    uint32_t flags;
    float metallic, roughness, normal_scale;
    float base_color[3]; float occlusion_strength;
    float emissive[3];
    float normal_bias;
    uint32_t tex[kCoreTextures][2];
    float occlusion_bias;
    uint32_t pad1;
    uint32_t gtex[kCoreTextures][4];
    float tt[6];
    uint32_t pad2[2];
};
static_assert(sizeof(LeanDrawDev) == 208, "LeanDrawDev must be 208 bytes");

constexpr int kMaxMipLevels = 16;
struct TexArrayDev {
    const uint8_t* texels;
    uint32_t width, height, layers;
    uint32_t mips;
    uint32_t level_off[kMaxMipLevels];
};

struct CubeDev {
    const uint2* texels;
    uint32_t size, mips;
    uint32_t level_off[kMaxMipLevels];
    const uint2* bordered;
    uint32_t b_level_off[kMaxMipLevels];
};
enum { kCubeSkybox = 0, kCubePrefiltered = 1, kCubeIrradiance = 2 };

struct DevScene {
    const uint8_t* buf[AWSM_BUF_COUNT];
    TexArrayDev tex[kMaxTexArrays];
    AwsmSampler samplers[kMaxSamplers];
    uint32_t n_tex, n_samplers;
    float skybox_rgba[4];
    float prefiltered_rgb[4];
    float irradiance_rgb[4];
    const uint16_t* lut_rg16f;
    uint32_t lut_w, lut_h;
    CubeDev cube[3];
};

struct TriRec;
constexpr size_t kTriRecBytes = 80;
constexpr uint32_t kMaxDirtyRanges = 12;

struct FrameDev {
    uint32_t width, height;
    uint32_t y0, y1;
    uint32_t sy0, sy1;
    uint32_t tiles_x, tiles_y;
    uint32_t tile_row0;
    uint32_t band_n, band_r;
    uint32_t out_compact;
    uint32_t n_draws;
    uint32_t total_tris;
    uint32_t total_verts;
    uint32_t rank0, block0;
    uint32_t bin_capacity;
    uint32_t has_opaque;
    uint32_t mipmap;
    uint32_t aniso;
    uint32_t msaa;
    const uint8_t* camera;
    float pix2view[16];
    float view_rot[9];
    float cam_pos[3];
    float ortho_view_dir[3];
    uint32_t cam_ortho;
    const DrawDev* draws;
    DrawShadeDev* draw_shade;
    TexSlotDev* tex_slots;
    DrawMatDev* draw_mat;
    float4* lights_pre;
    uint32_t lights_cap;
    float4* clip;
    float4* nrm;
    float4* tan;
    float4* wpos;
    const uint32_t* block_draw;
    float4* wcache;
    const DrawDev* prev_draws;
    uint32_t prev_n_draws;
    uint32_t cache_on;
    uint32_t cache_serial;
    uint32_t* cache_mark;
    uint32_t n_dirty;
    uint32_t dirty[12][3];
    TriRec* tri_rec;
    uint32_t* tri_info;
    uint4* tri_shade;
    uint32_t attr_data_bytes;
    LeanDrawDev* draw_lean;
    uint32_t* shade_todo;
    uint32_t shade_todo_cap;
    uint32_t* lean_done_flag;
    uint32_t lean_done_serial;
    uint32_t* camera_snap;
    uint32_t camera_snap_words;
    uint32_t* lean_next;
    uint32_t lean_grid;
    uint32_t* tile_count;
    uint32_t* tile_offset;
    uint32_t* tile_cursor;
    uint32_t* scan_tmp;
    uint32_t* tile_order;
    uint32_t* tile_split;
    unsigned long long* raster_scratch;
    uint32_t raster_extra_cap, raster_slot_cap;
    uint32_t* bin_list;
    uint32_t* big_list;
#ifdef AWSM_STAMP
    unsigned long long* stamps;
#endif
    const uint32_t* poison;
    uint32_t* host_bin_status;
    uint32_t frame_serial;
    uint32_t* counters;
    unsigned long long* vis;
    uint16_t* out_rgba16f;
    float* out_rgba32f;
    float4* msaa_color0;
    uint32_t* msaa_edges;
    unsigned long long* msaa_edge_bits;
    uint2* msaa_cells;
    const unsigned long long* hud_vis;
    const DrawDev* hud_draws;
    const uint32_t* hud_tri_info;
    uint32_t hud_pass;
    const unsigned long long* msaa_halo;
    uint32_t halo_bands;
    const uint16_t* opaque_rgba16f;
    uint4* frag_rec;
    float4* frag_color;
    uint32_t* frag_first;
    uint32_t frag_cap;
};

struct PostArgs {
    uint32_t width, height;
    const uint2* src;
    const unsigned long long* vis;
    const uint32_t* frag_first;
    const uint4* frag_rec;
    uint32_t frag_cap;
    const TriRec* tri_rec;
    const float* camera;
    float2* dof_lc;
    float4* dof_blur;
    const uint2* stage_in;
    uint2* stage_out;
    uint2* effects;
    uint32_t* display;
    uint32_t tonemap;
    uint32_t dof;
    const uint32_t* poison;
    uint32_t frame_serial;
};

#ifdef __HIPCC__
__device__ __forceinline__ bool frame_poisoned(const FrameDev& f) {
    return f.poison != nullptr && *(const __attribute__((address_space(4))) uint32_t*)f.poison == f.frame_serial;
}
#endif

}
```

awsm-renderer_amd/csrc/kernels_geometry.hip:

```cpp
#include "frame_params.hpp"
#include "raster_setup.hpp"

#ifndef AWSM_GEOM_PRIO
#define AWSM_GEOM_PRIO 3
#endif

namespace awsm {

#ifdef AWSM_STAMP
#define AWSM_STAMP_AT(f, kernel, slot) do { if (threadIdx.x == 0 && (f).stamps && blockIdx.x < 16384u) (f).stamps[((size_t)(kernel) * 16384u + blockIdx.x) * 8u + (slot)] = __builtin_amdgcn_s_memrealtime(); } while (0)
#else
#define AWSM_STAMP_AT(f, kernel, slot) do { } while (0)
#endif

struct GeomMetaDev {
    uint32_t mesh_key_high, mesh_key_low;
    uint32_t morph_len, morph_weights_off, morph_values_off;
    uint32_t skin_sets, skin_matrices_off, skin_index_weights_off;
    uint32_t transform_off, material_meta_off;
};

AWSM_DI bool draw_unchanged(const DevScene* __restrict__ sc, const FrameDev& f, const DrawDev& d, const DrawDev& p, const uint32_t* __restrict__ gmp) {
    if (d.geom_meta_off != p.geom_meta_off || d.vis_data_off != p.vis_data_off || d.tri_count != p.tri_count || d.flags != p.flags || d.first_tri != p.first_tri ||
        d.first_block != p.first_block || d.inst_off != p.inst_off) return false;
// ... 164 lines not shown
    f3 tangent_ortho = tangent_raw - world_normal * dot(tangent_raw, world_normal);
    const float tlen_sq = dot(tangent_ortho, tangent_ortho);
    if (tlen_sq > 1e-8f) {
        tangent_ortho = tangent_ortho * inverse_sqrt(tlen_sq);
    } else {
        const f3 axis = (fabsf(world_normal.z) > 0.999f) ? mk3(0.0f, 1.0f, 0.0f) : mk3(0.0f, 0.0f, 1.0f);
        tangent_ortho = normalize(cross(axis, world_normal));
    }

    const uint32_t lv = local0 + tid;
    const size_t gv = (size_t)3u * d.first_tri + lv;
    f.clip[gv] = make_float4(clip.x, clip.y, clip.z, clip.w);
    if (!FWD && f.wcache) f.wcache[gv] = make_float4(world_pos.x, world_pos.y, world_pos.z, world_pos.w);
    f.nrm[gv] = make_float4(world_normal.x, world_normal.y, world_normal.z, 0.0f);
    f.tan[gv] = make_float4(tangent_ortho.x, tangent_ortho.y, tangent_ortho.z, tangent.w);
    if (FWD) f.wpos[gv] = make_float4(world_pos.x, world_pos.y, world_pos.z, 1.0f);
    if (lv % 3u == 0u) {
        const uint32_t info = lo | ((d.flags & 0x7Fu) << 24)  | ((FWD && (f.draw_shade[lo].flags & 2u)) ? 0x80000000u : 0u);
        f.tri_info[d.first_tri + lv / 3u] = info;
        if (!FWD && f.tri_shade) {
            uint4 ts0 = make_uint4(info, 0u, 0u, 0u), ts1 = make_uint4(0u, 0u, 0u, 0u);
            if (sc->buf[AWSM_BUF_MATERIAL_META] && sc->buf[AWSM_BUF_ATTR_INDEX] && sc->buf[AWSM_BUF_ATTR_DATA]) {
                const uint32_t* mm = reinterpret_cast<const uint32_t*>(sc->buf[AWSM_BUF_MATERIAL_META] + (size_t)(gmp[9] / 256u) * 256u);
                const uint32_t* ai = reinterpret_cast<const uint32_t*>(sc->buf[AWSM_BUF_ATTR_INDEX]) + mm[9] / 4u + lv;
                const uint32_t data_word = mm[10] / 4u, stride_words = mm[11] / 4u, uv0 = mm[12];
                const uint32_t* ad = reinterpret_cast<const uint32_t*>(sc->buf[AWSM_BUF_ATTR_DATA]);
                const uint32_t w0 = data_word + ai[0] * stride_words + uv0, w1 = data_word + ai[1] * stride_words + uv0, w2 = data_word + ai[2] * stride_words + uv0;
                const uint32_t n_words = f.attr_data_bytes >> 2;
                if (w0 < n_words && w0 + 1u < n_words) { ts0.z = ad[w0]; ts0.w = ad[w0 + 1u]; }
                if (w1 < n_words && w1 + 1u < n_words) { ts1.x = ad[w1]; ts1.y = ad[w1 + 1u]; }
                if (w2 < n_words && w2 + 1u < n_words) { ts1.z = ad[w2]; ts1.w = ad[w2 + 1u]; }
            }
            f.tri_shade[2u * (d.first_tri + lv / 3u)] = ts0;
            f.tri_shade[2u * (d.first_tri + lv / 3u) + 1u] = ts1;
        }
    }
}

constexpr uint32_t kBinWindow = 2048;

template <bool FILL>
AWSM_DI void bin_emit(const FrameDev& f, int tx, int l, uint32_t rank) {
    const uint32_t idx = (uint32_t)l * f.tiles_x + (uint32_t)tx;
    if (!FILL) {
        atomicAdd(&f.tile_count[idx], 1u);
    } else {
        const uint32_t slot = atomicAdd(&f.tile_cursor[idx], 1u);
        const uint32_t pos = f.tile_offset[idx] + slot;
        if (pos < f.bin_capacity) f.bin_list[pos] = rank;
    }
}

struct BinTri {
    TriSetup t;
    int tx0, tx1, ty0, ty1, wdt, ntiles;
    bool ok, big, small;
};
template <bool SETUP>
AWSM_DI void bin_tri_load(const FrameDev& f, uint32_t r, BinTri& b) {
    b.ok = false;
    if (r < f.total_tris) {
        if (SETUP) {
            const float4 v0 = f.clip[(size_t)r * 3], v1 = f.clip[(size_t)r * 3 + 1], v2 = f.clip[(size_t)r * 3 + 2];
            bool outside = false;
            if ((f.band_n > 1u || f.y0 > 0u || f.y1 < f.height) && v0.w > 0.0f && v1.w > 0.0f && v2.w > 0.0f) {
                const float hh = 0.5f * (float)f.height;
                const float ya = (1.0f - v0.y / v0.w) * hh, yb = (1.0f - v1.y / v1.w) * hh, yc = (1.0f - v2.y / v2.w) * hh;
                const float lo = fminf(fminf(ya, yb), yc) - 1.0f, hi = fmaxf(fmaxf(ya, yb), yc) + 1.0f;
                if (hi < (float)f.y0 || lo >= (float)f.y1) outside = true;
                else if (f.band_n > 1u && lo >= (float)f.y0 && hi < (float)f.y1) {
                    const int bn = (int)f.band_n, row0 = (int)f.tile_row0;
                    const int a0 = ((int)floorf(lo) >> kTileShift) - row0, a1 = ((int)floorf(hi) >> kTileShift) - row0;
                    const int t0 = (max(a0, 0) + bn - 1) / bn, t1 = a1 >= 0 ? a1 / bn : -1;
                    outside = t0 > t1;
                }
            }
            if (outside) { tri_rec_store_invalid(f.tri_rec + r); b.ok = false; }
            else {
                const bool cull_back = ((f.tri_info[r] >> 24) & AWSM_DRAW_CULL_BACK) != 0;
                b.ok = tri_setup(v0, v1, v2, cull_back, f.width, f.height, f.y0, f.y1, b.t);
                if (!b.ok) { b.t.minx = 0; b.t.maxx = 0; b.t.miny = 0; b.t.maxy = 0; }
                tri_rec_store(f.tri_rec + r, b.t, b.ok);
            }
        } else {
            b.ok = tri_rec_load(f.tri_rec + r, b.t);
        }
    }
    b.tx0 = 0; b.tx1 = -1; b.ty0 = 0; b.ty1 = -1;
    const int bn = (int)f.band_n, row0 = (int)f.tile_row0;
    if (b.ok) {
        b.tx0 = b.t.minx >> kTileShift; b.tx1 = b.t.maxx >> kTileShift;
        const int a0 = (b.t.miny >> kTileShift) - row0, a1 = (b.t.maxy >> kTileShift) - row0;
        b.ty0 = (a0 + bn - 1) / bn; b.ty1 = a1 >= 0 ? a1 / bn : -1;
        b.ok = b.ty0 <= b.ty1;
    }
    b.wdt = b.tx1 - b.tx0 + 1;
    b.ntiles = b.ok ? b.wdt * (b.ty1 - b.ty0 + 1) : 0;
    b.big = b.ntiles > 16;
    b.small = b.ok && !b.big;
}
AWSM_DI bool bin_tile_hit(const FrameDev& f, const TriSetup& t, int ntiles, int tx, int l) {
    const int ty = (int)f.tile_row0 + l * (int)f.band_n;
    return ntiles == 1 || tile_may_overlap(t, tx << kTileShift, ty << kTileShift, (tx + 1) << kTileShift, (ty + 1) << kTileShift);
}

constexpr uint32_t kBinBatches = 1;
static_assert(kBinBatches == 1, "k_bin keeps its triangle in registers across the phases");

template <bool FILL>
AWSM_DI void bin_big_walk(const FrameDev& f, uint32_t block, uint32_t n_blocks) {
    const uint32_t n_big = f.counters[4];
    const int lane = threadIdx.x & 63;
    const uint32_t wave = block * 4u + (threadIdx.x >> 6), n_waves = n_blocks * 4u;
    for (uint32_t i = wave; i < n_big; i += n_waves) {
        const uint32_t r = f.big_list[i];
        BinTri b;
        bin_tri_load<false>(f, r, b);
        for (int k = lane; k < b.ntiles; k += 64) {
            const int l = b.ty0 + k / b.wdt, tx = b.tx0 + k % b.wdt;
            if (bin_tile_hit(f, b.t, b.ntiles, tx, l)) bin_emit<FILL>(f, tx, l, r);
        }
    }
}
constexpr uint32_t kBinBigBlocks = 64;

template <bool FILL>
__global__ __launch_bounds__(256) void k_bin(FrameDev f) {
#if AWSM_GEOM_PRIO
    __builtin_amdgcn_s_setprio(AWSM_GEOM_PRIO);
#endif
    __shared__ int win[4];
    __shared__ uint32_t n_ok, n_big_wg, big_base;
    __shared__ uint32_t lcount[kBinWindow];
    __shared__ uint32_t lbase[FILL ? kBinWindow : 1];

    const uint32_t tid = threadIdx.x;
    if (frame_poisoned(f)) return;
    AWSM_STAMP_AT(f, FILL ? 2 : 0, 0);
    if (FILL && blockIdx.x < kBinBigBlocks) { bin_big_walk<true>(f, blockIdx.x, kBinBigBlocks); AWSM_STAMP_AT(f, 2, 7); return; }
    const uint32_t r0 = f.rank0 + (blockIdx.x - (FILL ? kBinBigBlocks : 0u)) * (256u * kBinBatches) + tid;
    const int lane = tid & 63;
    if (tid == 0) { win[0] = 0x7fffffff; win[1] = 0x7fffffff; win[2] = -1; win[3] = -1; n_ok = 0; n_big_wg = 0; }
    __syncthreads();

    uint32_t my_ok = 0;
    BinTri keep;
    for (uint32_t j = 0; j < kBinBatches; j++) {
        const uint32_t r = r0 + j * 256u;
        BinTri& b = keep;
        bin_tri_load<!FILL>(f, r, b);
        AWSM_STAMP_AT(f, FILL ? 2 : 0, 7);
        my_ok += b.ok ? 1u : 0u;
        {
            int wx0 = b.small ? b.tx0 : 0x7fffffff, wy0 = b.small ? b.ty0 : 0x7fffffff, wx1 = b.small ? b.tx1 : -1, wy1 = b.small ? b.ty1 : -1;
#pragma unroll
            for (int off = 32; off > 0; off >>= 1) {
                wx0 = min(wx0, __shfl_xor(wx0, off)); wy0 = min(wy0, __shfl_xor(wy0, off));
                wx1 = max(wx1, __shfl_xor(wx1, off)); wy1 = max(wy1, __shfl_xor(wy1, off));
            }
            if (lane == 0 && wx1 >= 0) { atomicMin(&win[0], wx0); atomicMin(&win[1], wy0); atomicMax(&win[2], wx1); atomicMax(&win[3], wy1); }
        }
    }
    uint32_t big_slot = 0;
    if (!FILL) {
        const unsigned long long mask = __ballot(keep.big);
        if (mask) {
// ... 702 lines not shown
```

awsm-renderer_amd/csrc/kernels_shade.hip:

```cpp
#include <type_traits>
#include "frame_params.hpp"
#include "raster_setup.hpp"

#ifndef AWSM_LEAN_WAVES
#define AWSM_LEAN_WAVES 6
#endif

namespace awsm {

struct GBufferTexel {
    f4 packed_nt;
    float bx, by;
    f4 bary_derivs;
};
template <bool DERIVS>
AWSM_DI GBufferTexel reconstruct_core(const TriSetup& t, float4 n0, float4 n1, float4 n2, float4 t0, float4 t1, float4 t2, int cx, int cy) {
    GBufferTexel g;
    g.bary_derivs = {0.0f, 0.0f, 0.0f, 0.0f};
    const double Xc = sample_coord((cx << 8) + 128), Yc = sample_coord((cy << 8) + 128);
    const EdgeVals ev = tri_edges_d(t, Xc, Yc);
    const float e0 = (float)ev.E[0] * t.iw[0], e1 = (float)ev.E[1] * t.iw[1], e2 = (float)ev.E[2] * t.iw[2];
    const float inv_esum = 1.0f / ((e0 + e1) + e2);
    const float b0 = e0 * inv_esum, b1 = e1 * inv_esum, b2 = e2 * inv_esum;
    const f3 Ni = {(b0 * n0.x + b1 * n1.x) + b2 * n2.x, (b0 * n0.y + b1 * n1.y) + b2 * n2.y, (b0 * n0.z + b1 * n1.z) + b2 * n2.z};
    const f4 Ti = {(b0 * t0.x + b1 * t1.x) + b2 * t2.x, (b0 * t0.y + b1 * t1.y) + b2 * t2.y,
                   (b0 * t0.z + b1 * t1.z) + b2 * t2.z, (b0 * t0.w + b1 * t1.w) + b2 * t2.w};
    const f4 p = pack_normal_tangent(normalize(Ni), normalize(mk3(Ti.x, Ti.y, Ti.z)), Ti.w);
    g.packed_nt = {round_f16(p.x), round_f16(p.y), round_f16(p.z), round_f16(p.w)};
    g.bx = round_f16(b0);
    g.by = round_f16(b1);
    if (DERIVS) {
        const EdgeVals eh = tri_edges_d(t, sample_coord(((cx ^ 1) << 8) + 128), Yc), evv = tri_edges_d(t, Xc, sample_coord(((cy ^ 1) << 8) + 128));
        const float h0 = (float)eh.E[0] * t.iw[0], h1 = (float)eh.E[1] * t.iw[1], h2 = (float)eh.E[2] * t.iw[2];
        const float w0 = (float)evv.E[0] * t.iw[0], w1 = (float)evv.E[1] * t.iw[1], w2 = (float)evv.E[2] * t.iw[2];
        const float ish = 1.0f / ((h0 + h1) + h2), isv = 1.0f / ((w0 + w1) + w2);
        const float hb0 = h0 * ish, hb1 = h1 * ish, vb0 = w0 * isv, vb1 = w1 * isv;
        const float ddx0 = (cx & 1) ? b0 - hb0 : hb0 - b0, ddx1 = (cx & 1) ? b1 - hb1 : hb1 - b1;
        const float ddy0 = (cy & 1) ? b0 - vb0 : vb0 - b0, ddy1 = (cy & 1) ? b1 - vb1 : vb1 - b1;
        g.bary_derivs = {round_f16(ddx0), round_f16(ddy0), round_f16(ddx1), round_f16(ddy1)};
    }
    return g;
}
template <bool DERIVS>
AWSM_DI GBufferTexel reconstruct_gbuffer(const FrameDev& f, uint32_t rank, int cx, int cy) {
    TriSetup t;
    tri_rec_load(f.tri_rec + rank, t);
    const float4 n0 = f.nrm[(size_t)rank * 3], n1 = f.nrm[(size_t)rank * 3 + 1], n2 = f.nrm[(size_t)rank * 3 + 2];
    const float4 t0 = f.tan[(size_t)rank * 3], t1 = f.tan[(size_t)rank * 3 + 1], t2 = f.tan[(size_t)rank * 3 + 2];
    return reconstruct_core<DERIVS>(t, n0, n1, n2, t0, t1, t2, cx, cy);
}

AWSM_DI f2 strict_oct_of(const FrameDev& f, uint32_t rank, int cx, int cy) {
    TriSetup t;
    tri_rec_load(f.tri_rec + rank, t);
    const float4 n0 = f.nrm[(size_t)rank * 3], n1 = f.nrm[(size_t)rank * 3 + 1], n2 = f.nrm[(size_t)rank * 3 + 2];
    const double Xc = sample_coord((cx << 8) + 128), Yc = sample_coord((cy << 8) + 128);
    const EdgeVals ev = tri_edges_d(t, Xc, Yc);
    const float e0 = (float)ev.E[0] * t.iw[0], e1 = (float)ev.E[1] * t.iw[1], e2 = (float)ev.E[2] * t.iw[2];
    const float inv_esum = 1.0f / ((e0 + e1) + e2);
    const float b0 = e0 * inv_esum, b1 = e1 * inv_esum, b2 = e2 * inv_esum;
    const f3 Ni = {(b0 * n0.x + b1 * n1.x) + b2 * n2.x, (b0 * n0.y + b1 * n1.y) + b2 * n2.y, (b0 * n0.z + b1 * n1.z) + b2 * n2.z};
    const f2 oct = encode_octahedral(normalize(Ni));
    return mk2(round_f16(oct.x), round_f16(oct.y));
}
AWSM_DI f3 strict_normal_of(const FrameDev& f, uint32_t rank, int cx, int cy) { return decode_octahedral(strict_oct_of(f, rank, cx, cy)); }
AWSM_DI uint32_t oct_word(f2 oct) { return (uint32_t)f16_bits(oct.x) | ((uint32_t)f16_bits(oct.y) << 16); }
AWSM_DI f2 oct_of_word(uint32_t w) { return mk2(__half2float(__ushort_as_half((unsigned short)(w & 0xFFFFu))), __half2float(__ushort_as_half((unsigned short)(w >> 16)))); }

AWSM_DI bool row_owned(const FrameDev& f, int py) {
    if (py < (int)f.sy0 || py >= (int)f.sy1) return false;
    return f.band_n <= 1u || (((uint32_t)py >> kTileShift) % f.band_n) == f.band_r;
}

constexpr float kEdgeNormalThreshold = 0.95f, kEdgeDepthThreshold = 0.02f, kEdgeMsaaDepthThreshold = 0.02f;
AWSM_DI float view_space_depth(const m4& inv_proj, float depth, float px, float py, float W, float H) {
    if (inv_proj.c[0].z == 0.0f && inv_proj.c[1].z == 0.0f && inv_proj.c[0].w == 0.0f && inv_proj.c[1].w == 0.0f)
        return (inv_proj.c[2].z * depth + inv_proj.c[3].z) / (inv_proj.c[2].w * depth + inv_proj.c[3].w);
    const f4 view_pos = mul(inv_proj, mk4((px / W) * 2.0f - 1.0f, 1.0f - (py / H) * 2.0f, depth, 1.0f));
    return view_pos.z / view_pos.w;
}
AWSM_DI float key_depth(unsigned long long k) { return k == ~0ull ? 1.0f : __uint_as_float((uint32_t)(k >> 32)); }
AWSM_DI uint32_t key_rank(unsigned long long k) { return 0xFFFFFFFFu - (uint32_t)(k & 0xFFFFFFFFull); }
AWSM_DI bool edge_mask_depth_msaa(const m4& inv_proj, const unsigned long long k4[4], float pcx, float pcy, float W, float H) {
    uint32_t count = 0; float dmin = 1e9f, dmax = -1e9f;
#pragma unroll
    for (int s = 0; s < 4; s++) {
        if (k4[s] == ~0ull) continue;
        count++;
        const float vd = view_space_depth(inv_proj, key_depth(k4[s]), pcx, pcy, W, H);
        dmin = fminf(dmin, vd); dmax = fmaxf(dmax, vd);
    }
    if (count < 2u) return false;
    return fabsf(dmax - dmin) > (kEdgeMsaaDepthThreshold * fabsf((dmax + dmin) * 0.5f));
}

AWSM_DI bool depth_only_projection(const m4& inv_proj) { return inv_proj.c[0].z == 0.0f && inv_proj.c[1].z == 0.0f && inv_proj.c[0].w == 0.0f && inv_proj.c[1].w == 0.0f; }
AWSM_DI float view_depth_approx(const m4& inv_proj, float depth) { return (inv_proj.c[2].z * depth + inv_proj.c[3].z) * __builtin_amdgcn_rcpf(inv_proj.c[2].w * depth + inv_proj.c[3].w); }
AWSM_DI bool edge_mask_depth_msaa_filtered(const m4& inv_proj, const unsigned long long k4[4], float pcx, float pcy, float W, float H) {
    if (depth_only_projection(inv_proj)) {
        uint32_t count = 0; float dmin = 1e9f, dmax = -1e9f;
#pragma unroll
        for (int s = 0; s < 4; s++) {
            if (k4[s] == ~0ull) continue;
            count++;
            const float vd = view_depth_approx(inv_proj, key_depth(k4[s]));
            dmin = fminf(dmin, vd); dmax = fmaxf(dmax, vd);
        }
        if (count < 2u) return false;
        const float lhs = fabsf(dmax - dmin), rhs = kEdgeMsaaDepthThreshold * fabsf((dmax + dmin) * 0.5f), margin = 4e-6f * fmaxf(fabsf(dmax), fabsf(dmin));
        if (lhs > rhs + margin) return true;
        if (lhs < rhs - margin) return false;
    }
    return edge_mask_depth_msaa(inv_proj, k4, pcx, pcy, W, H);
}

AWSM_DI f3 strict_world_position(const m4& inv_proj, const m4& inv_view, int cx, int cy, float W, float H, float depth) {
    const float uvx = ((float)cx + 0.5f) / W, uvy = ((float)cy + 0.5f) / H;
    const f4 view_h = mul(inv_proj, mk4(uvx * 2.0f - 1.0f, 1.0f - uvy * 2.0f, depth, 1.0f));
    const float vw = fmaxf(view_h.w, 1e-8f);
    const f4 wp = mul(inv_view, mk4(view_h.x / vw, view_h.y / vw, view_h.z / vw, 1.0f));
    return {wp.x, wp.y, wp.z};
}

#pragma clang fp contract(fast)
// ... 1484 lines not shown
#pragma unroll
    for (int i = 0; i < 4; i++) { const f32x4 v = cload<f32x4>(base, byte_off + 16u * i); m.c[i] = {v.x, v.y, v.z, v.w}; }
    return m;
}

namespace lean {
struct Tap { uint32_t t00, t10, t01, t11; float fx, fy; };
struct Tex { unsigned long long base; uint32_t lw, lh; };
AWSM_DI Tex decode(uint32_t lo, uint32_t hi) { return {((unsigned long long)(hi & 0xFFFFu) << 32) | lo, (hi >> 16) & 15u, (hi >> 20) & 15u}; }
AWSM_DI void fetch(const Tex& x, float u, float v, Tap& t) {
    const float xf = __builtin_amdgcn_ldexpf(u, (int)x.lw) - 0.5f, yf = __builtin_amdgcn_ldexpf(v, (int)x.lh) - 0.5f;
    const float flx = floorf(xf), fly = floorf(yf);
    t.fx = xf - flx; t.fy = yf - fly;
    const uint32_t xi = (uint32_t)(int)flx, yi = (uint32_t)(int)fly;
    const uint32_t i0 = __builtin_amdgcn_ubfe(xi, 0u, x.lw), j0 = __builtin_amdgcn_ubfe(yi, 0u, x.lh), j1 = __builtin_amdgcn_ubfe(yi + 1u, 0u, x.lh);
    const uint32_t sh = x.lw + 2u, i0b = i0 << 2;
    const u32x2a4 p0 = gload64<u32x2a4>(x.base, (j0 << sh) | i0b), p1 = gload64<u32x2a4>(x.base, (j1 << sh) | i0b);
    t.t00 = p0.x; t.t10 = p0.y; t.t01 = p1.x; t.t11 = p1.y;
    if (__builtin_amdgcn_ubfe(xi + 1u, 0u, x.lw) == 0u) {
        t.t10 = gload64<uint32_t>(x.base, j0 << sh); t.t11 = gload64<uint32_t>(x.base, j1 << sh);
    }
}
struct Weights { float w00, w10, w01, w11; };
AWSM_DI Weights weights(const Tap& t) {
    const float gx = 1.0f - t.fx, gy = 1.0f - t.fy;
    return {gx * gy, t.fx * gy, gx * t.fy, t.fx * t.fy};
}
template <int BYTE> AWSM_DI float ub(uint32_t t) {
    return (float)((t >> (8 * BYTE)) & 255u);
}
template <int BYTE> AWSM_DI float channel(const Tap& t, const Weights& w) {
    return ub<BYTE>(t.t00) * w.w00 + ub<BYTE>(t.t10) * w.w10 + ub<BYTE>(t.t01) * w.w01 + ub<BYTE>(t.t11) * w.w11;
}
AWSM_DI f2 brdf_lut(const uint16_t* lut, uint32_t lut_w, uint32_t lut_h, float n_dot_v, float roughness) {
    const float u = saturate(n_dot_v), v = saturate(roughness);
    const int W = (int)lut_w, H = (int)lut_h;
    const float x = u * (float)W - 0.5f, y = v * (float)H - 0.5f;
    const float flx = floorf(x), fly = floorf(y);
    const float fx = x - flx, fy = y - fly;
    const int xi = (int)flx, yi = (int)fly;
    const int i0 = max(xi, 0), i1 = min(xi + 1, W - 1), j0 = max(yi, 0), j1 = min(yi + 1, H - 1);
    const uint32_t r0 = (uint32_t)(j0 * W) << 2, r1 = (uint32_t)(j1 * W) << 2;
    const uint32_t t00 = gload<uint32_t>(lut, r0 + ((uint32_t)i0 << 2)), t10 = gload<uint32_t>(lut, r0 + ((uint32_t)i1 << 2));
    const uint32_t t01 = gload<uint32_t>(lut, r1 + ((uint32_t)i0 << 2)), t11 = gload<uint32_t>(lut, r1 + ((uint32_t)i1 << 2));
    const float gx = 1.0f - fx, gy = 1.0f - fy;
    const float r_top = f16_bits_to_f32((unsigned short)(t00 & 0xFFFFu)) * gx + f16_bits_to_f32((unsigned short)(t10 & 0xFFFFu)) * fx;
    const float r_bot = f16_bits_to_f32((unsigned short)(t01 & 0xFFFFu)) * gx + f16_bits_to_f32((unsigned short)(t11 & 0xFFFFu)) * fx;
    const float g_top = f16_bits_to_f32((unsigned short)(t00 >> 16)) * gx + f16_bits_to_f32((unsigned short)(t10 >> 16)) * fx;
    const float g_bot = f16_bits_to_f32((unsigned short)(t01 >> 16)) * gx + f16_bits_to_f32((unsigned short)(t11 >> 16)) * fx;
    return {r_top * gy + r_bot * fy, g_top * gy + g_bot * fy};
}
struct Lit {
    f3 n, v, F0, df90, bd;
    float ndv_raw, ndv_dir, ndv4, a2m1, a2_g1v, gk, one_m_gk, occlusion, F0max, df90max;
};
AWSM_DI void direct(const Lit& s, f3 l, f3 radiance, f3& color) {
    const float ndl = saturate(fm::fdot(s.n, l));
#ifndef AWSM_NO_LIGHT_SKIP
    if (__builtin_amdgcn_ballot_w64(ndl > 0.0f) == 0ull) return;
#endif
    const f3 sum = s.v + l;
    const float len_sq = fm::fdot(sum, sum);
    const bool has_half = len_sq > 1e-8f;
    const float inv_len = has_half ? fm::rsq(len_sq) : 0.0f;
    const float ndh = saturate(fm::fdot(s.n, sum) * inv_len);
    const float vdh = fm::fdot(s.v, sum) * inv_len;
    const float p = saturate(1.0f - (has_half ? vdh : s.ndv_dir));
    const float p2 = p * p, p5 = (p2 * p2) * p;
    const f3 F = {s.F0.x + s.df90.x * p5, s.F0.y + s.df90.y * p5, s.F0.z + s.df90.z * p5};
    const float dd = (ndh * ndh) * s.a2m1 + 1.0f;
    const float den = (((kPi * dd) * dd + kEps) * (ndl * s.one_m_gk + s.gk)) * fmaxf(s.ndv4 * ndl, kEps);
    const float spec = has_half ? (s.a2_g1v * ndl) * fm::rcp(den) : 0.0f;
    const float k_d = 1.0f - (s.F0max + s.df90max * p5);
    const float w = ndl * s.occlusion;
    color.x += (s.bd.x * k_d + F.x * spec) * (radiance.x * w);
    color.y += (s.bd.y * k_d + F.y * spec) * (radiance.y * w);
    color.z += (s.bd.z * k_d + F.z * spec) * (radiance.z * w);
}
}

#ifndef AWSM_LEAN_SLOTS
#define AWSM_LEAN_SLOTS 16u
#endif
constexpr uint32_t kLeanSlots = AWSM_LEAN_SLOTS, kLeanChunks = 13u, kLeanNone = 0xFFFFFFFFu;
struct LeanStage { uint4 q[kLeanSlots][kLeanChunks]; };
#define AWSM_AS3 __attribute__((address_space(3)))
AWSM_DI float4 bits_float4(uint4 v) { return make_float4(__uint_as_float(v.x), __uint_as_float(v.y), __uint_as_float(v.z), __uint_as_float(v.w)); }
AWSM_DI double2 bits_double2(uint4 v) { return make_double2(__hiloint2double((int)v.y, (int)v.x), __hiloint2double((int)v.w, (int)v.z)); }
AWSM_DI uint4 as_uint4(u32x4 v) { return make_uint4(v.x, v.y, v.z, v.w); }

namespace lean {
struct TexS { const void* base; uint32_t lw, lh; };
AWSM_DI TexS decode_s(uint32_t lo, uint32_t hi) { return {reinterpret_cast<const void*>(((unsigned long long)(hi & 0xFFFFu) << 32) | lo), (hi >> 16) & 15u, (hi >> 20) & 15u}; }
AWSM_DI void fetch_s(const TexS& x, float u, float v, Tap& t) {
    const float xf = __builtin_amdgcn_ldexpf(u, (int)x.lw) - 0.5f, yf = __builtin_amdgcn_ldexpf(v, (int)x.lh) - 0.5f;
    const float flx = floorf(xf), fly = floorf(yf);
    t.fx = xf - flx; t.fy = yf - fly;
    const uint32_t xi = (uint32_t)(int)flx, yi = (uint32_t)(int)fly;
    const uint32_t i0 = __builtin_amdgcn_ubfe(xi, 0u, x.lw), j0 = __builtin_amdgcn_ubfe(yi, 0u, x.lh), j1 = __builtin_amdgcn_ubfe(yi + 1u, 0u, x.lh);
    const uint32_t sh = x.lw + 2u, i0b = i0 << 2;
    const u32x2a4 p0 = gload<u32x2a4>(x.base, (j0 << sh) | i0b), p1 = gload<u32x2a4>(x.base, (j1 << sh) | i0b);
    t.t00 = p0.x; t.t10 = p0.y; t.t01 = p1.x; t.t11 = p1.y;
    if (__builtin_amdgcn_ubfe(xi + 1u, 0u, x.lw) == 0u) {
        t.t10 = gload<uint32_t>(x.base, j0 << sh); t.t11 = gload<uint32_t>(x.base, j1 << sh);
    }
}
template <typename BASE> struct TexGT { BASE base; uint32_t lw, levels, layer, layers; };
typedef TexGT<const void*> TexG;
typedef TexGT<unsigned long long> TexGL;
AWSM_DI TexG decode_g(uint32_t w0, uint32_t w1, uint32_t w2, uint32_t w3) {
    return {reinterpret_cast<const void*>(((unsigned long long)(w1 & 0xFFFFu) << 32) | w0), w1 >> 24, (w1 >> 16) & 15u, w2, w3};
}
AWSM_DI TexGL decode_gl(uint32_t w0, uint32_t w1, uint32_t w2, uint32_t w3) {
    return {((unsigned long long)(w1 & 0xFFFFu) << 32) | w0, w1 >> 24, (w1 >> 16) & 15u, w2, w3};
}
template <typename T> AWSM_DI T gload_any(const void* base, uint32_t off) { return gload<T>(base, off); }
template <typename T> AWSM_DI T gload_any(unsigned long long base, uint32_t off) { return gload64<T>(base, off); }
struct Lod { uint32_t lo, hi; float f; };
template <typename BASE> AWSM_DI Lod select_lod(const TexGT<BASE>& x, float m2) {
    const float rho2 = __builtin_amdgcn_ldexpf(m2, (int)(2u * x.lw));
    float lod = 0.5f * __builtin_amdgcn_logf(fmaxf(rho2, 1e-12f));
    Lod r = {0u, 0u, 0.0f};
    if (lod > 0.0f && x.levels > 1u) {
        lod = fminf(lod, (float)(x.levels - 1u));
        const float fl = floorf(lod);
        r.lo = (uint32_t)fl; r.hi = min(r.lo + 1u, x.levels - 1u); r.f = (r.hi != r.lo) ? lod - fl : 0.0f;
    }
    return r;
}
template <typename BASE> AWSM_DI void fetch_g(const TexGT<BASE>& x, uint32_t level, float u, float v, Tap& t) {
    const uint32_t lwl = x.lw - level;
    const uint32_t g_all = __builtin_amdgcn_ubfe(0x55555555u, 0u, 2u * (x.lw + 1u)), g_rest = __builtin_amdgcn_ubfe(0x55555555u, 0u, 2u * (lwl + 1u));
    const uint32_t first = x.layers * (g_all - g_rest) + (x.layer << (2u * lwl));
    const float xf = __builtin_amdgcn_ldexpf(u, (int)lwl) - 0.5f, yf = __builtin_amdgcn_ldexpf(v, (int)lwl) - 0.5f;
    const float flx = floorf(xf), fly = floorf(yf);
    t.fx = xf - flx; t.fy = yf - fly;
    const uint32_t xi = (uint32_t)(int)flx, yi = (uint32_t)(int)fly;
    const uint32_t i0 = __builtin_amdgcn_ubfe(xi, 0u, lwl), j0 = __builtin_amdgcn_ubfe(yi, 0u, lwl), j1 = __builtin_amdgcn_ubfe(yi + 1u, 0u, lwl);
    const uint32_t r0 = (first + (j0 << lwl)) << 2, r1 = (first + (j1 << lwl)) << 2, i0b = i0 << 2;
    const u32x2a4 p0 = gload_any<u32x2a4>(x.base, r0 + i0b), p1 = gload_any<u32x2a4>(x.base, r1 + i0b);
    t.t00 = p0.x; t.t10 = p0.y; t.t01 = p1.x; t.t11 = p1.y;
    if (__builtin_amdgcn_ubfe(xi + 1u, 0u, lwl) == 0u) {
        t.t10 = gload_any<uint32_t>(x.base, r0); t.t11 = gload_any<uint32_t>(x.base, r1);
    }
}
AWSM_DI f4 cube_level_b(const void* base, const void* scene, uint32_t which, uint32_t size, uint32_t level, uint32_t face, float sn, float tn) {
    const uint32_t N = max(size >> level, 1u), P = N + 2u;
    const uint32_t lvl0 = gload<uint32_t>(scene, (uint32_t)(offsetof(DevScene, cube) + which * sizeof(CubeDev) + offsetof(CubeDev, b_level_off)) + level * 4u);
    float x = sn * (float)N - 0.5f, y = tn * (float)N - 0.5f;
    if (!(x >= -0.5f)) x = -0.5f;
    if (!(y >= -0.5f)) y = -0.5f;
    x = fminf(x, (float)N - 0.5f); y = fminf(y, (float)N - 0.5f);
    const float flx = floorf(x), fly = floorf(y), fx = x - flx, fy = y - fly;
    const uint32_t ib = (uint32_t)((int)flx + 1), jb = (uint32_t)((int)fly + 1);
    const uint32_t t0 = (lvl0 + (face * P + jb) * P + ib) << 3;
    typedef uint32_t u32x4a8 __attribute__((ext_vector_type(4), aligned(8)));
    const u32x4a8 r0 = gload<u32x4a8>(base, t0), r1 = gload<u32x4a8>(base, t0 + (P << 3));
    const f4 c00 = half4(make_uint2(r0.x, r0.y)), c10 = half4(make_uint2(r0.z, r0.w)), c01 = half4(make_uint2(r1.x, r1.y)), c11 = half4(make_uint2(r1.z, r1.w));
    return lerp4(lerp4(c00, c10, fx), lerp4(c01, c11, fx), fy);
}
template <uint32_t WHICH>
AWSM_DI f4 cube_sample(const DevScene* sc, f3 d, float level) {
    const uint32_t o = (uint32_t)(offsetof(DevScene, cube) + WHICH * sizeof(CubeDev));
    const u32x2 bp = cload<u32x2>(sc, o + (uint32_t)offsetof(CubeDev, bordered));
    const u32x2 sm = cload<u32x2>(sc, o + (uint32_t)offsetof(CubeDev, size));
    const void* base = reinterpret_cast<const void*>(((unsigned long long)bp.y << 32) | bp.x);
    const uint32_t size = sm.x, mips = sm.y;
    const float ax = fabsf(d.x), ay = fabsf(d.y), az = fabsf(d.z);
    uint32_t face; float scd, tcd, ma;
    if (az >= ax && az >= ay) { face = d.z < 0.0f ? 5u : 4u; scd = d.z < 0.0f ? -d.x : d.x; tcd = -d.y; ma = az; }
    else if (ay >= ax) { face = d.y < 0.0f ? 3u : 2u; scd = d.x; tcd = d.y < 0.0f ? -d.z : d.z; ma = ay; }
    else { face = d.x < 0.0f ? 1u : 0u; scd = d.x < 0.0f ? d.z : -d.z; tcd = -d.y; ma = ax; }
    const float inv = fm::rcp(ma);
    const float sn = 0.5f * (scd * inv) + 0.5f, tn = 0.5f * (tcd * inv) + 0.5f;
    const float top = (float)(mips - 1u);
    float lod = level > 0.0f ? level : 0.0f;
    lod = fminf(lod, top);
    const float fl = floorf(lod), fr = lod - fl;
    const uint32_t l0 = (uint32_t)fl, l1 = min(l0 + 1u, mips - 1u);
    f4 r = cube_level_b(base, sc, WHICH, size, l0, face, sn, tn);
    if (__builtin_amdgcn_ballot_w64(fr > 0.0f && l1 != l0) != 0ull) { const f4 h = cube_level_b(base, sc, WHICH, size, l1, face, sn, tn); if (fr > 0.0f && l1 != l0) r = lerp4(r, h, fr); }
    return r;
}
AWSM_DI f3 irradiance(const DevScene* sc, f3 n) {
    if (!sc->cube[kCubeIrradiance].bordered) return sample_irradiance(sc, n);
    const f4 c = cube_sample<kCubeIrradiance>(sc, n, 0.0f);
    return {c.x, c.y, c.z};
}
AWSM_DI f3 prefiltered(const DevScene* sc, f3 dir, float roughness) {
// ... 19 lines not shown
    const float xf = __builtin_amdgcn_ldexpf(u, (int)lwl) - 0.5f, yf = __builtin_amdgcn_ldexpf(v, (int)lwl) - 0.5f;
    const float flx = floorf(xf), fly = floorf(yf);
    fx = xf - flx; fy = yf - fly;
    const uint32_t xi = (uint32_t)(int)flx, yi = (uint32_t)(int)fly;
    const uint32_t i0 = __builtin_amdgcn_ubfe(xi, 0u, lwl), j0 = __builtin_amdgcn_ubfe(yi, 0u, lwl), j1 = __builtin_amdgcn_ubfe(yi + 1u, 0u, lwl);
    ft.i0b = i0 << 2; ft.row0 = j0 << lwl; ft.row1 = j1 << lwl;
    ft.wrap = __builtin_amdgcn_ubfe(xi + 1u, 0u, lwl) == 0u;
    ft.g_rest = __builtin_amdgcn_ubfe(0x55555555u, 0u, 2u * (lwl + 1u)); ft.sh2 = 2u * lwl;
}
struct Quad { uint32_t t00, t10, t01, t11; };
template <typename BASE> AWSM_DI void fetch_q(const TexGT<BASE>& x, const Foot& ft, Quad& q) {
    const uint32_t g_all = __builtin_amdgcn_ubfe(0x55555555u, 0u, 2u * (x.lw + 1u));
    const uint32_t first = x.layers * (g_all - ft.g_rest) + (x.layer << ft.sh2);
    const uint32_t r0 = (first + ft.row0) << 2, r1 = (first + ft.row1) << 2;
    const u32x2a4 p0 = gload_any<u32x2a4>(x.base, r0 + ft.i0b), p1 = gload_any<u32x2a4>(x.base, r1 + ft.i0b);
    q.t00 = p0.x; q.t10 = p0.y; q.t01 = p1.x; q.t11 = p1.y;
    if (ft.wrap) { q.t10 = gload_any<uint32_t>(x.base, r0); q.t11 = gload_any<uint32_t>(x.base, r1); }
}
AWSM_DI TexG decode_any(const void*, uint32_t w0, uint32_t w1, uint32_t w2, uint32_t w3) { return decode_g(w0, w1, w2, w3); }
AWSM_DI TexGL decode_any(unsigned long long, uint32_t w0, uint32_t w1, uint32_t w2, uint32_t w3) { return decode_gl(w0, w1, w2, w3); }
struct W8 { float l00, l10, l01, l11, h00, h10, h01, h11; };
template <int BYTE> AWSM_DI float channel8(const Quad& lo, const Quad& hi, const W8& w) {
    return ((ub<BYTE>(lo.t00) * w.l00 + ub<BYTE>(lo.t10) * w.l10) + (ub<BYTE>(lo.t01) * w.l01 + ub<BYTE>(lo.t11) * w.l11)) +
           ((ub<BYTE>(hi.t00) * w.h00 + ub<BYTE>(hi.t10) * w.h10) + (ub<BYTE>(hi.t01) * w.h01 + ub<BYTE>(hi.t11) * w.h11));
}
}

struct LeanItem { int cx, cy; uint32_t rank; float depth; bool live; f3 color; };
template <int GRAD, bool MSAA, bool ITEMS>
AWSM_DI bool lean_core(const DevScene* __restrict__ sc, const FrameDev& f, const ShadeBlock& b, const uint32_t wg, const uint32_t tid, LeanStage* __restrict__ st, LeanItem* __restrict__ item) {
    const uint32_t lane = tid & 63u;
    const int cx = ITEMS ? item->cx : b.x0 + (int)(tid & 15u), cy = ITEMS ? item->cy : b.y0 + (int)(tid >> 4);
    const bool inside = ITEMS ? item->live : (cx < (int)f.width && cy < (int)f.sy1);
    const uint32_t pv = (uint32_t)cy * f.width + (uint32_t)cx;
    const uint32_t p = f.out_compact ? (((b.brow >> 1) << kTileShift) + ((uint32_t)cy & (uint32_t)(kTile - 1))) * f.width + (uint32_t)cx : pv;

    u32x2 key = {0xFFFFFFFFu, 0xFFFFFFFFu};
    bool want_c0 = false;
    if (ITEMS) { if (inside) key = {~item->rank, __float_as_uint(item->depth)}; }
    else if (!MSAA) { if (inside) key = gload<u32x2>(f.vis, pv << 3); }
    else {
        u32x4 ka = {0xFFFFFFFFu, 0xFFFFFFFFu, 0xFFFFFFFFu, 0xFFFFFFFFu}, kb = ka;
        if (inside) { ka = gload<u32x4>(f.vis, pv << 5); kb = gload<u32x4>(f.vis, (pv << 5) + 16u); }
        key = {ka.x, ka.y};
        const bool bg0 = (ka.x & ka.y) == 0xFFFFFFFFu, bg1 = (ka.z & ka.w) == 0xFFFFFFFFu, bg2 = (kb.x & kb.y) == 0xFFFFFFFFu, bg3 = (kb.z & kb.w) == 0xFFFFFFFFu;
        bool sure = false, test = false;
        if (!(bg0 && bg1 && bg2 && bg3)) {
            if (bg0) sure = true;
            else if (bg1 || bg2 || bg3 || ka.z != ka.x || kb.x != ka.x || kb.z != ka.x) {
                const m4 inv_proj = cload_m4(f.camera, 256u);
                const unsigned long long k4[4] = {((unsigned long long)ka.y << 32) | ka.x, ((unsigned long long)ka.w << 32) | ka.z, ((unsigned long long)kb.y << 32) | kb.x, ((unsigned long long)kb.w << 32) | kb.z};
                sure = edge_mask_depth_msaa_filtered(inv_proj, k4, (float)cx + 0.5f, (float)cy + 0.5f, (float)f.width, (float)f.height);
                test = !sure;
            }
        }
        const unsigned long long m_sure = __builtin_amdgcn_ballot_w64(sure), m_test = __builtin_amdgcn_ballot_w64(test);
        if (lane == 0u) *reinterpret_cast<ulonglong2*>(f.msaa_edge_bits + (size_t)(b.blk * 4u + (tid >> 6)) * 2u) = make_ulonglong2(m_sure, m_test);
        want_c0 = sure || test;
    }
    bool hud = false;
    if (!ITEMS && !MSAA && f.hud_vis && inside) { const u32x2 hk = gload<u32x2>(f.hud_vis, pv << 3); hud = (hk.x & hk.y) != 0xFFFFFFFFu; }
    if (hud) { store_pixel(f, p, f4{0.0f, 0.0f, 0.0f, 0.0f}); key = {0xFFFFFFFFu, 0xFFFFFFFFu}; }
    const bool hit = inside && (key.x & key.y) != 0xFFFFFFFFu;
    if (!ITEMS && inside && !hit && !hud) {
        const f4 sky = skybox_color(sc, f, cx, cy);
        store_pixel(f, p, sky);
        if (MSAA) {
            f.msaa_cells[pv] = make_uint2(0u, 0xFFFFFFFFu);
            if (want_c0) f.msaa_color0[pv] = make_float4(sky.x, sky.y, sky.z, sky.w);
        }
    }
    unsigned long long rem = __builtin_amdgcn_ballot_w64(hit);
    if (rem == 0ull) return true;
    const uint32_t rank = hit ? ~key.x : 0xFFFFFFFFu;
    const float depth = __uint_as_float(key.y);

    asm volatile("; MARK level1");
    unsigned long long src_base; uint32_t src_stride;
    {
        const uint32_t j = lane;
        const unsigned long long rec = (unsigned long long)f.tri_rec, nr = (unsigned long long)f.nrm, tn = (unsigned long long)f.tan, tsh = (unsigned long long)f.tri_shade;
        src_base = j < 5u ? rec + j * 16u : (j < 8u ? nr + (j - 5u) * 16u : (j < 11u ? tn + (j - 8u) * 16u : tsh + (j - 11u) * 16u));
        src_stride = j < 5u ? (uint32_t)kTriRecBytes : (j < 11u ? 48u : 32u);
    }
    uint32_t my_slot = kLeanNone, n_slots = 0u;
    while (rem != 0ull && n_slots < kLeanSlots) {
        const uint32_t r = (uint32_t)__builtin_amdgcn_readlane((int)rank, (int)__builtin_ctzll(rem));
        if (rank == r) my_slot = n_slots;
        if (lane < kLeanChunks)
            __builtin_amdgcn_global_load_lds((const AWSM_AS1 void*)(src_base + (unsigned long long)r * src_stride), (AWSM_AS3 void*)&st->q[n_slots][0], 16, 0, 0);
        rem &= ~__builtin_amdgcn_uicmp(rank, r, 32 );
        n_slots++;
    }
    asm volatile("s_waitcnt vmcnt(0)" ::: "memory");
    const bool staged = my_slot != kLeanNone;
    const uint4* rec = &st->q[staged ? my_slot : 0u][0];
    uint4 ts0 = rec[11], ts1 = rec[12];
    TriRecRaw raw;
    raw.q0 = bits_float4(rec[0]); raw.q1 = bits_float4(rec[1]); raw.q2 = bits_float4(rec[2]); raw.d3 = bits_double2(rec[3]); raw.d4 = bits_double2(rec[4]);
    float4 n0 = bits_float4(rec[5]), n1 = bits_float4(rec[6]), n2 = bits_float4(rec[7]);
    float4 t0 = bits_float4(rec[8]), t1 = bits_float4(rec[9]), t2 = bits_float4(rec[10]);
    if (hit && !staged) {
        ts0 = as_uint4(gload<u32x4>(f.tri_shade, rank << 5)); ts1 = as_uint4(gload<u32x4>(f.tri_shade, (rank << 5) + 16u));
        const uint32_t ro = rank * (uint32_t)kTriRecBytes, vo = rank * 48u;
        raw.q0 = as_float4(gload<f32x4>(f.tri_rec, ro)); raw.q1 = as_float4(gload<f32x4>(f.tri_rec, ro + 16u)); raw.q2 = as_float4(gload<f32x4>(f.tri_rec, ro + 32u));
        { const f64x2 a = gload<f64x2>(f.tri_rec, ro + 48u), c = gload<f64x2>(f.tri_rec, ro + 64u); raw.d3 = make_double2(a.x, a.y); raw.d4 = make_double2(c.x, c.y); }
        n0 = as_float4(gload<f32x4>(f.nrm, vo)); n1 = as_float4(gload<f32x4>(f.nrm, vo + 16u)); n2 = as_float4(gload<f32x4>(f.nrm, vo + 32u));
        t0 = as_float4(gload<f32x4>(f.tan, vo)); t1 = as_float4(gload<f32x4>(f.tan, vo + 16u)); t2 = as_float4(gload<f32x4>(f.tan, vo + 32u));
    }

    asm volatile("; MARK strict");
    TriSetup t;
    tri_rec_unpack(raw, t);
    const GBufferTexel g = reconstruct_core<(GRAD != 0)>(t, n0, n1, n2, t0, t1, t2, cx, cy);
    if (MSAA && hit) f.msaa_cells[pv] = make_uint2(oct_word(mk2(g.packed_nt.x, g.packed_nt.y)), key.y);
    const float bz = (1.0f - g.bx) - g.by;
    float u = interp3_strict(g.bx, g.by, bz, __uint_as_float(ts0.z), __uint_as_float(ts1.x), __uint_as_float(ts1.z));
    float v = interp3_strict(g.bx, g.by, bz, __uint_as_float(ts0.w), __uint_as_float(ts1.y), __uint_as_float(ts1.w));
    const uint32_t draw = ts0.x & 0x00FFFFFFu;
    const uint32_t d0 = (uint32_t)__builtin_amdgcn_readlane((int)draw, (int)__builtin_ctzll(__builtin_amdgcn_ballot_w64(hit)));
    const bool one_draw = __builtin_amdgcn_ballot_w64(hit && draw != d0) == 0ull;
    f2 ddx = {0.0f, 0.0f}, ddy = {0.0f, 0.0f};
    float m2 = 0.0f;
    float r2min = 0.0f; f2 major = {0.0f, 0.0f};
    if (GRAD) {
        const float x0 = __uint_as_float(ts0.z), y0 = __uint_as_float(ts0.w), x1 = __uint_as_float(ts1.x), y1 = __uint_as_float(ts1.y), x2 = __uint_as_float(ts1.z), y2 = __uint_as_float(ts1.w);
        const float dAlphaDx = g.bary_derivs.x, dAlphaDy = g.bary_derivs.y, dBetaDx = g.bary_derivs.z, dBetaDy = g.bary_derivs.w;
        const float dGammaDx = -dAlphaDx - dBetaDx, dGammaDy = -dAlphaDy - dBetaDy;
        ddx = {x0 * dAlphaDx + x1 * dBetaDx + x2 * dGammaDx, y0 * dAlphaDx + y1 * dBetaDx + y2 * dGammaDx};
        ddy = {x0 * dAlphaDy + x1 * dBetaDy + x2 * dGammaDy, y0 * dAlphaDy + y1 * dBetaDy + y2 * dGammaDy};
        const bool tiny = (fabsf(dAlphaDx) + fabsf(dAlphaDy) + fabsf(dBetaDx) + fabsf(dBetaDy)) < 1e-20f;
        const bool ok = (ddx.x == ddx.x) && (ddx.y == ddx.y) && (ddy.x == ddy.x) && (ddy.y == ddy.y);
        if (tiny || !ok) { ddx = {0.0f, 0.0f}; ddy = {0.0f, 0.0f}; }
    }
    if (GRAD == 0) {
    } else if (one_draw) {
        const uint32_t lo = d0 * (uint32_t)sizeof(LeanDrawDev);
        if (cload<uint32_t>(f.draw_lean, lo) & 8u) {
            const f32x4 ta = cload<f32x4>(f.draw_lean, lo + 176u); const f32x2a4 tb = cload<f32x2a4>(f.draw_lean, lo + 192u);
            const float u2 = affine2_strict(ta.x, ta.y, tb.x, u, v), v2 = affine2_strict(ta.z, ta.w, tb.y, u, v);
            u = u2; v = v2;
            if (GRAD) { ddx = {ta.x * ddx.x + ta.y * ddx.y, ta.z * ddx.x + ta.w * ddx.y}; ddy = {ta.x * ddy.x + ta.y * ddy.y, ta.z * ddy.x + ta.w * ddy.y}; }
        }
    } else {
        const uint32_t lo = draw * (uint32_t)sizeof(LeanDrawDev);
        const bool xf = (gload<uint32_t>(f.draw_lean, lo) & 8u) != 0u;
        if (__builtin_amdgcn_ballot_w64(xf) != 0ull) {
            const f32x4 ta = gload<f32x4>(f.draw_lean, lo + 176u); const f32x2a4 tb = gload<f32x2a4>(f.draw_lean, lo + 192u);
            const float u2 = affine2_strict(ta.x, ta.y, tb.x, u, v), v2 = affine2_strict(ta.z, ta.w, tb.y, u, v);
            if (xf) { u = u2; v = v2; }
            if (GRAD && xf) { ddx = {ta.x * ddx.x + ta.y * ddx.y, ta.z * ddx.x + ta.w * ddx.y}; ddy = {ta.x * ddy.x + ta.y * ddy.y, ta.z * ddy.x + ta.w * ddy.y}; }
        }
    }
    if (GRAD) {
        const float rx2 = ddx.x * ddx.x + ddx.y * ddx.y, ry2 = ddy.x * ddy.x + ddy.y * ddy.y;
        m2 = fmaxf(rx2, ry2);
        if (GRAD == 2) { r2min = fminf(rx2, ry2); major = rx2 >= ry2 ? ddx : ddy; }
    }
    bool todo = GRAD != 0 && __builtin_amdgcn_ballot_w64(hit && !(fabsf(u) <= 32768.0f && fabsf(v) <= 32768.0f)) != 0ull;

    asm volatile("; MARK fetch");
    f3 base, emissive;
    float metallic_in, roughness_in, normal_scale, occlusion_strength, normal_bias, occlusion_bias;
    uint32_t exists;
    lean::Tap tp0, tp1, tp2, tp3, tp4;
    lean::TapG tg0, tg1, tg2, tg3, tg4;
    constexpr uint32_t kNeed = GRAD == 2 ? 7u : (GRAD ? 3u : 1u);
    auto fetch_all = [&](float uu, float vv, float m2e, bool act, const uint32_t tex_mask = 31u, const bool factors = true) {
        if (one_draw) {
            const uint32_t lo = d0 * (uint32_t)sizeof(LeanDrawDev);
            const u32x4 L0 = cload<u32x4>(f.draw_lean, lo), L1 = cload<u32x4>(f.draw_lean, lo + 16u), L2 = cload<u32x4>(f.draw_lean, lo + 32u);
            const u32x4 L3 = cload<u32x4>(f.draw_lean, lo + 48u), L4 = cload<u32x4>(f.draw_lean, lo + 64u);
            const u32x2 L5 = cload<u32x2>(f.draw_lean, lo + 80u), L5s = cload<u32x2>(f.draw_lean, lo + 88u);
            if (GRAD == 0) {
                if (L0.x & 8u) {
                    const f32x4 ta = cload<f32x4>(f.draw_lean, lo + 176u); const f32x2a4 tb = cload<f32x2a4>(f.draw_lean, lo + 192u);
                    const float u2 = affine2_strict(ta.x, ta.y, tb.x, uu, vv), v2 = affine2_strict(ta.z, ta.w, tb.y, uu, vv);
                    uu = u2; vv = v2;
                }
                todo = todo || __builtin_amdgcn_ballot_w64(hit && !(fabsf(uu) <= 32768.0f && fabsf(vv) <= 32768.0f)) != 0ull;
            }
            todo = todo || (L0.x & kNeed) != kNeed;
            const uint32_t exs = todo ? 0u : L0.x >> 8;
            const uint32_t ex = act ? exs & tex_mask : 0u;
            if (GRAD) {
                const u32x4 G0 = cload<u32x4>(f.draw_lean, lo + 96u), G1 = cload<u32x4>(f.draw_lean, lo + 112u), G2 = cload<u32x4>(f.draw_lean, lo + 128u);
                const u32x4 G3 = cload<u32x4>(f.draw_lean, lo + 144u), G4 = cload<u32x4>(f.draw_lean, lo + 160u);
                if (ex & 1u) lean::fetch_trilinear(lean::decode_g(G0.x, G0.y, G0.z, G0.w), m2e, uu, vv, tg0);
                if (ex & 2u) lean::fetch_trilinear(lean::decode_g(G1.x, G1.y, G1.z, G1.w), m2e, uu, vv, tg1);
                if (ex & 4u) lean::fetch_trilinear(lean::decode_g(G2.x, G2.y, G2.z, G2.w), m2e, uu, vv, tg2);
                if (ex & 8u) lean::fetch_trilinear(lean::decode_g(G3.x, G3.y, G3.z, G3.w), m2e, uu, vv, tg3);
                if (ex & 16u) lean::fetch_trilinear(lean::decode_g(G4.x, G4.y, G4.z, G4.w), m2e, uu, vv, tg4);
            } else {
                if (ex & 1u) lean::fetch_s(lean::decode_s(L3.x, L3.y), uu, vv, tp0);
                if (ex & 2u) lean::fetch_s(lean::decode_s(L3.z, L3.w), uu, vv, tp1);
                if (ex & 4u) lean::fetch_s(lean::decode_s(L4.x, L4.y), uu, vv, tp2);
                if (ex & 8u) lean::fetch_s(lean::decode_s(L4.z, L4.w), uu, vv, tp3);
                if (ex & 16u) lean::fetch_s(lean::decode_s(L5.x, L5.y), uu, vv, tp4);
            }
            exists = exs;
            if (factors) {
            metallic_in = __uint_as_float(L0.y); roughness_in = __uint_as_float(L0.z); normal_scale = __uint_as_float(L0.w);
            base = {__uint_as_float(L1.x), __uint_as_float(L1.y), __uint_as_float(L1.z)}; occlusion_strength = __uint_as_float(L1.w);
            emissive = {__uint_as_float(L2.x), __uint_as_float(L2.y), __uint_as_float(L2.z)}; normal_bias = __uint_as_float(L2.w); occlusion_bias = __uint_as_float(L5s.x);
            }
        } else {
            const uint32_t lo = draw * (uint32_t)sizeof(LeanDrawDev);
            const u32x4 L0 = gload<u32x4>(f.draw_lean, lo), L1 = gload<u32x4>(f.draw_lean, lo + 16u), L2 = gload<u32x4>(f.draw_lean, lo + 32u);
            const u32x4 L3 = gload<u32x4>(f.draw_lean, lo + 48u), L4 = gload<u32x4>(f.draw_lean, lo + 64u);
            const u32x2 L5 = gload<u32x2>(f.draw_lean, lo + 80u), L5s = gload<u32x2>(f.draw_lean, lo + 88u);
            if (GRAD == 0) {
                if (__builtin_amdgcn_ballot_w64((L0.x & 8u) != 0u) != 0ull) {
                    const f32x4 ta = gload<f32x4>(f.draw_lean, lo + 176u); const f32x2a4 tb = gload<f32x2a4>(f.draw_lean, lo + 192u);
                    const float u2 = affine2_strict(ta.x, ta.y, tb.x, uu, vv), v2 = affine2_strict(ta.z, ta.w, tb.y, uu, vv);
                    if (L0.x & 8u) { uu = u2; vv = v2; }
                }
                todo = todo || __builtin_amdgcn_ballot_w64(hit && !(fabsf(uu) <= 32768.0f && fabsf(vv) <= 32768.0f)) != 0ull;
            }
            todo = todo || __builtin_amdgcn_ballot_w64(hit && (L0.x & kNeed) != kNeed) != 0ull;
            const uint32_t exs = (todo || !hit) ? 0u : L0.x >> 8;
            const uint32_t ex = act ? exs & tex_mask : 0u;
            if (GRAD) {
                const u32x4 G0 = gload<u32x4>(f.draw_lean, lo + 96u), G1 = gload<u32x4>(f.draw_lean, lo + 112u), G2 = gload<u32x4>(f.draw_lean, lo + 128u);
                const u32x4 G3 = gload<u32x4>(f.draw_lean, lo + 144u), G4 = gload<u32x4>(f.draw_lean, lo + 160u);
                if (ex & 1u) lean::fetch_trilinear(lean::decode_gl(G0.x, G0.y, G0.z, G0.w), m2e, uu, vv, tg0);
                if (ex & 2u) lean::fetch_trilinear(lean::decode_gl(G1.x, G1.y, G1.z, G1.w), m2e, uu, vv, tg1);
                if (ex & 4u) lean::fetch_trilinear(lean::decode_gl(G2.x, G2.y, G2.z, G2.w), m2e, uu, vv, tg2);
                if (ex & 8u) lean::fetch_trilinear(lean::decode_gl(G3.x, G3.y, G3.z, G3.w), m2e, uu, vv, tg3);
                if (ex & 16u) lean::fetch_trilinear(lean::decode_gl(G4.x, G4.y, G4.z, G4.w), m2e, uu, vv, tg4);
            } else {
                const lean::Tex x0 = lean::decode(L3.x, L3.y), x1 = lean::decode(L3.z, L3.w), x2 = lean::decode(L4.x, L4.y), x3 = lean::decode(L4.z, L4.w), x4 = lean::decode(L5.x, L5.y);
                if (ex & 1u) lean::fetch(x0, uu, vv, tp0);
                if (ex & 2u) lean::fetch(x1, uu, vv, tp1);
                if (ex & 4u) lean::fetch(x2, uu, vv, tp2);
                if (ex & 8u) lean::fetch(x3, uu, vv, tp3);
                if (ex & 16u) lean::fetch(x4, uu, vv, tp4);
            }
            exists = exs;
            if (factors) {
            metallic_in = __uint_as_float(L0.y); roughness_in = __uint_as_float(L0.z); normal_scale = __uint_as_float(L0.w);
            base = {__uint_as_float(L1.x), __uint_as_float(L1.y), __uint_as_float(L1.z)}; occlusion_strength = __uint_as_float(L1.w);
            emissive = {__uint_as_float(L2.x), __uint_as_float(L2.y), __uint_as_float(L2.z)}; normal_bias = __uint_as_float(L2.w); occlusion_bias = __uint_as_float(L5s.x);
            }
        }
    };
    float nf = 1.0f;
    if (GRAD == 2) {
        const uint32_t A = one_draw ? cload<uint32_t>(f.draw_lean, d0 * (uint32_t)sizeof(LeanDrawDev) + 92u) : gload<uint32_t>(f.draw_lean, draw * (uint32_t)sizeof(LeanDrawDev) + 92u);
        if (A > 1u && m2 > 0.0f) {
            const float Af = (float)min(A, 16u);
            nf = r2min * (Af * Af) <= m2 ? Af : __builtin_sqrtf(m2 / r2min);
            nf = fminf(fmaxf(nf, 1.0f), Af);
        }
    }
    const float m2c = GRAD == 2 ? m2 * fm::rcp(nf * nf) : m2;
    f3 world_position, surface_to_camera;
    TBN tbn;
    f3 normal;
    float occlusion = 1.0f;
    auto mid = [&]() {
    asm volatile("; MARK standard");
    const float pxf = (float)cx, pyf = (float)cy;
    const float* M = f.pix2view;
    const float hx = M[0] * pxf + (M[4] * pyf + (M[8] * depth + M[12])), hy = M[1] * pxf + (M[5] * pyf + (M[9] * depth + M[13]));
    const float hz = M[2] * pxf + (M[6] * pyf + (M[10] * depth + M[14])), hw = M[3] * pxf + (M[7] * pyf + (M[11] * depth + M[15]));
    const float ivw = fm::rcp(fmaxf(hw, 1e-8f));
    const f3 vp = {hx * ivw, hy * ivw, hz * ivw};
    const float* R = f.view_rot;
    const f3 rel = {R[0] * vp.x + (R[3] * vp.y + R[6] * vp.z), R[1] * vp.x + (R[4] * vp.y + R[7] * vp.z), R[2] * vp.x + (R[5] * vp.y + R[8] * vp.z)};
    world_position = {rel.x + f.cam_pos[0], rel.y + f.cam_pos[1], rel.z + f.cam_pos[2]};
#ifdef AWSM_STRICT_POSITION
    world_position = strict_world_position(cload_m4(f.camera, 256u), cload_m4(f.camera, 320u), cx, cy, (float)f.width, (float)f.height, depth);
#endif
    if (f.cam_ortho) {
        surface_to_camera = mk3(f.ortho_view_dir[0], f.ortho_view_dir[1], f.ortho_view_dir[2]);
    } else {
        const f3 to_camera = mk3(f.cam_pos[0], f.cam_pos[1], f.cam_pos[2]) - world_position;
        surface_to_camera = fm::fdot(to_camera, to_camera) > 0.0f ? fm::fsafe_normalize(to_camera) : mk3(0.0f, 0.0f, 1.0f);
    }
    asm volatile("; MARK tbn");
    tbn = fm::funpack_normal_tangent(g.packed_nt);
// ... 829 lines not shown
```

awsm-renderer_amd/csrc/raster_setup.hpp:

```cpp
#pragma once
#include "device_math.hpp"

namespace awsm {

struct TriSetup {
    float a[3], b[3];
    double c[3];
    float zq[3];
    float iw[3];
    int minx, maxx, miny, maxy;
    bool front;
    bool exact;
    bool small;
};

AWSM_DI bool finite4(float4 v) { return isfinite(v.x) && isfinite(v.y) && isfinite(v.z) && isfinite(v.w); }

constexpr float kSubPix = 256.0f;
constexpr float kGuardBand = 8388608.0f;

AWSM_DI bool tri_setup(float4 v0, float4 v1, float4 v2, bool cull_back, uint32_t width, uint32_t height,
                       uint32_t ry0, uint32_t ry1, TriSetup& t) {
    if (!finite4(v0) || !finite4(v1) || !finite4(v2)) return false;
    if (v0.x < -v0.w && v1.x < -v1.w && v2.x < -v2.w) return false;
// ... 48 lines not shown
        minx = max(minx, mnx >> 8); maxx = min(maxx, (mxx - 1) >> 8);
        miny = max(miny, mny >> 8); maxy = min(maxy, (mxy - 1) >> 8);
    } else {
        const float w0 = v0.w, w1 = v1.w, w2 = v2.w;
        const float X0 = (v0.x + v0.w) * hw, Y0 = (v0.w - v0.y) * hh;
        const float X1 = (v1.x + v1.w) * hw, Y1 = (v1.w - v1.y) * hh;
        const float X2 = (v2.x + v2.w) * hw, Y2 = (v2.w - v2.y) * hh;
        float a0 = Y1 * w2 - Y2 * w1, b0 = X2 * w1 - X1 * w2, c0 = X1 * Y2 - X2 * Y1;
        float a1 = Y2 * w0 - Y0 * w2, b1 = X0 * w2 - X2 * w0, c1 = X2 * Y0 - X0 * Y2;
        float a2 = Y0 * w1 - Y1 * w0, b2 = X1 * w0 - X0 * w1, c2 = X0 * Y1 - X1 * Y0;
        float det = (X0 * a0 + Y0 * b0) + w0 * c0;
        if (!(det != 0.0f) || !isfinite(det)) return false;
        if (cull_back && det > 0.0f) return false;
        t.front = det < 0.0f;
        t.exact = false; t.small = false;
        if (det < 0.0f) {
            a0 = -a0; b0 = -b0; c0 = -c0; a1 = -a1; b1 = -b1; c1 = -c1; a2 = -a2; b2 = -b2; c2 = -c2;
            det = -det;
        }
        t.a[0] = a0; t.b[0] = b0; t.c[0] = (double)c0;
        t.a[1] = a1; t.b[1] = b1; t.c[1] = (double)c1;
        t.a[2] = a2; t.b[2] = b2; t.c[2] = (double)c2;
        const float inv_det = 1.0f / det;
        t.zq[0] = v0.z * inv_det; t.zq[1] = v1.z * inv_det; t.zq[2] = v2.z * inv_det;
        t.iw[0] = 1.0f; t.iw[1] = 1.0f; t.iw[2] = 1.0f;
    }
    if (minx > maxx || miny > maxy) return false;
    t.minx = minx; t.maxx = maxx; t.miny = miny; t.maxy = maxy;
    return true;
}

struct alignas(16) TriRec {
    float a[3], b[3];
    float zq[3];
    float iw[3];
    double c[3];
    uint32_t bbox_x;
    uint32_t bbox_y;
};
static_assert(sizeof(TriRec) == 80, "TriRec must be 80 bytes");

AWSM_DI void tri_rec_store(TriRec* __restrict__ dst, const TriSetup& t, bool ok) {
    float4* q = reinterpret_cast<float4*>(dst);
    const uint32_t bx = ok ? ((uint32_t)t.minx | (t.small ? 0x8000u : 0u) | ((uint32_t)t.maxx << 16) | (t.exact ? 0x80000000u : 0u)) : 1u;
    const uint32_t by = ok ? ((uint32_t)t.miny | ((uint32_t)t.maxy << 16) | (t.front ? 0x80000000u : 0u)) : 1u;
    q[0] = make_float4(t.a[0], t.a[1], t.a[2], t.b[0]);
    q[1] = make_float4(t.b[1], t.b[2], t.zq[0], t.zq[1]);
    q[2] = make_float4(t.zq[2], t.iw[0], t.iw[1], t.iw[2]);
    double2* d = reinterpret_cast<double2*>(dst);
    d[3] = make_double2(t.c[0], t.c[1]);
    d[4] = make_double2(t.c[2], __hiloint2double((int)by, (int)bx));
}
AWSM_DI void tri_rec_store_invalid(TriRec* __restrict__ dst) {
    reinterpret_cast<double2*>(dst)[4] = make_double2(0.0, __hiloint2double(1, 1));
}
struct TriRecRaw { float4 q0, q1, q2; double2 d3, d4; };
AWSM_DI TriRecRaw tri_rec_fetch(const TriRec* __restrict__ src) {
    const float4* q = reinterpret_cast<const float4*>(src);
    const double2* d = reinterpret_cast<const double2*>(src);
    TriRecRaw r;
    r.q0 = q[0]; r.q1 = q[1]; r.q2 = q[2]; r.d3 = d[3]; r.d4 = d[4];
    return r;
}
AWSM_DI bool tri_rec_unpack(const TriRecRaw& r, TriSetup& t) {
    t.a[0] = r.q0.x; t.a[1] = r.q0.y; t.a[2] = r.q0.z; t.b[0] = r.q0.w;
    t.b[1] = r.q1.x; t.b[2] = r.q1.y; t.zq[0] = r.q1.z; t.zq[1] = r.q1.w;
    t.zq[2] = r.q2.x; t.iw[0] = r.q2.y; t.iw[1] = r.q2.z; t.iw[2] = r.q2.w;
    t.c[0] = r.d3.x; t.c[1] = r.d3.y; t.c[2] = r.d4.x;
    const uint32_t bx = (uint32_t)__double2loint(r.d4.y), by = (uint32_t)__double2hiint(r.d4.y);
    t.minx = (int)(bx & 0x7FFFu); t.small = (bx & 0x8000u) != 0u; t.maxx = (int)((bx >> 16) & 0x7FFFu); t.exact = (bx >> 31) != 0u; t.miny = (int)(by & 0xFFFFu); t.maxy = (int)((by >> 16) & 0x7FFFu);
    t.front = (by >> 31) != 0u;
    return t.minx <= t.maxx;
}
AWSM_DI bool tri_rec_load(const TriRec* __restrict__ src, TriSetup& t) { return tri_rec_unpack(tri_rec_fetch(src), t); }

struct EdgeVals { double E[3]; };
AWSM_DI double sample_coord(int p_sub) { return (double)p_sub * 0.00390625; }
AWSM_DI EdgeVals tri_edges_d(const TriSetup& t, double X, double Y) {
    EdgeVals r;
#pragma unroll
    for (int i = 0; i < 3; i++) r.E[i] = fma((double)t.a[i], X, fma((double)t.b[i], Y, t.c[i]));
    return r;
}
AWSM_DI bool edge_inside(double e, float a, float b) {
    return e > 0.0 || (e == 0.0 && (a > 0.0f || (a == 0.0f && b > 0.0f)));
}

AWSM_DI int msaa4_x(int k) { return k == 0 ? 96 : (k == 1 ? 224 : (k == 2 ? 32 : 160)); }
AWSM_DI int msaa4_y(int k) { return k == 0 ? 32 : (k == 1 ? 96 : (k == 2 ? 160 : 224)); }

AWSM_DI double edge_threshold(float a, float b) {
    return (a > 0.0f || (a == 0.0f && b > 0.0f)) ? __longlong_as_double((long long)0x8000000000000001ull) : 0.0;
}

AWSM_DI bool depth_key_bits(float zn, uint32_t& bits) { bits = __float_as_uint(zn + 0.0f); return bits <= 0x3F800000u; }
AWSM_DI bool depth_key_bits_sum(float zc_canonical, float dz, uint32_t& bits) { bits = __float_as_uint(zc_canonical + dz); return bits <= 0x3F800000u; }

AWSM_DI unsigned long long tri_key_from_edges(const TriSetup& t, const EdgeVals& ev, uint32_t rank);
AWSM_DI unsigned long long tri_sample_key_at(const TriSetup& t, double X, double Y, uint32_t rank) {
    return tri_key_from_edges(t, tri_edges_d(t, X, Y), rank);
}
AWSM_DI bool tri_covers(const TriSetup& t, const EdgeVals& ev) {
    return ((int)(ev.E[0] > edge_threshold(t.a[0], t.b[0])) & (int)(ev.E[1] > edge_threshold(t.a[1], t.b[1])) & (int)(ev.E[2] > edge_threshold(t.a[2], t.b[2]))) != 0;
}
AWSM_DI float tri_plane_depth(const TriSetup& t, const EdgeVals& ev) {
    const float e0 = (float)ev.E[0], e1 = (float)ev.E[1], e2 = (float)ev.E[2];
    return (e0 * t.zq[0] + e1 * t.zq[1]) + e2 * t.zq[2];
}
AWSM_DI void msaa_depth_steps(const float a[3], const float b[3], const float zq[3], float dz[4]) {
    const float gx = (a[0] * zq[0] + a[1] * zq[1]) + a[2] * zq[2];
    const float gy = (b[0] * zq[0] + b[1] * zq[1]) + b[2] * zq[2];
    dz[0] = gx * 0.375f + gy * 0.125f; dz[1] = gx * 0.875f + gy * 0.375f; dz[2] = gx * 0.125f + gy * 0.625f; dz[3] = gx * 0.625f + gy * 0.875f;
}
AWSM_DI unsigned long long tri_msaa_sample_key(const TriSetup& t, int px, int py, int k, float zc, const float dz[4], uint32_t rank) {
    if (!tri_covers(t, tri_edges_d(t, sample_coord((px << 8) + msaa4_x(k)), sample_coord((py << 8) + msaa4_y(k))))) return ~0ull;
    uint32_t zbits;
    if (!depth_key_bits_sum(zc, dz[k], zbits)) return ~0ull;
    return ((unsigned long long)zbits << 32) | (unsigned long long)(0xFFFFFFFFu - rank);
}
AWSM_DI unsigned long long tri_key_from_edges(const TriSetup& t, const EdgeVals& ev, uint32_t rank) {
    if (!tri_covers(t, ev)) return ~0ull;
    const float zn = tri_plane_depth(t, ev);
    uint32_t zbits;
    if (!depth_key_bits(zn, zbits)) return ~0ull;
    return ((unsigned long long)zbits << 32) | (unsigned long long)(0xFFFFFFFFu - rank);
}

AWSM_DI bool tile_may_overlap(const TriSetup& t, int tx0, int ty0, int tx1, int ty1 ) {
#pragma unroll
    for (int i = 0; i < 3; i++) {
        const double X = t.a[i] > 0.0f ? (double)tx1 : (double)tx0;
        const double Y = t.b[i] > 0.0f ? (double)ty1 : (double)ty0;
        const double ax = (double)t.a[i] * X, by = (double)t.b[i] * Y;
        const double e = (ax + by) + t.c[i];
        const double slack = 1e-15 * ((fabs(ax) + fabs(by)) + fabs(t.c[i]));
        if (e < -slack) return false;
    }
    return true;
}

}
```

Baseline: 3451 frames/s.

## Precompute integer edge equations for small triangles and share texel coordinates across textures

```diff
diff --git a/__graft_entry__.py b/__graft_entry__.py
--- a/__graft_entry__.py
+++ b/__graft_entry__.py
@@ -13,6 +13,7 @@
     hip_so, host_so = b.build_all()
     for p in (hip_so, host_so):
         assert os.path.exists(p), p
+    b.build_hip_variant("lean_percall_off", b.LEAN_PERCALL_OFF)
     from oracle import oracle_lib
     oracle_lib.build()
     mock_dir = os.path.join(ROOT, "tests", "mock")
diff --git a/awsm-renderer_amd/build.py b/awsm-renderer_amd/build.py
--- a/awsm-renderer_amd/build.py
+++ b/awsm-renderer_amd/build.py
@@ -38,6 +38,30 @@
     return os.path.join(PACKAGE_DIR, "libawsm_hip.so")
 
 
+LEAN_PERCALL_OFF = ("-DAWSM_NO_INT_EDGES", "-DAWSM_NO_SHARED_TEXCOORDS")
+
+
+def build_hip_variant(name: str, defines, arch: str = "gfx950") -> str:
+    hipcc = shutil.which("hipcc") or "/opt/rocm/bin/hipcc"
+    csrc = os.path.join(PACKAGE_DIR, "csrc")
+    out_dir = os.path.join(os.path.dirname(PACKAGE_DIR), "build", "variants")
+    os.makedirs(out_dir, exist_ok=True)
+    obj, lib = os.path.join(out_dir, f"var_{name}.o"), os.path.join(out_dir, f"lib_{name}.so")
+    src = os.path.join(csrc, "kernels_shade.hip")
+    deps = [os.path.join(csrc, n) for n in os.listdir(csrc) if n.endswith((".hip", ".hpp", ".cpp"))] + [os.path.join(os.path.dirname(PACKAGE_DIR), "include", "awsm_hip.h")]
+    if os.path.exists(lib) and all(os.path.getmtime(lib) >= os.path.getmtime(d) for d in deps):
+        return lib
+    build_hip(arch=arch)
+    flags = [f"--offload-arch={arch}", "-O3", "-std=c++17", "-fPIC", "-ffp-contract=off", "-fno-fast-math", "-fno-slp-vectorize", "-Wall", "-Wno-unused-function"]
+    for cmd in ([hipcc] + flags + list(defines) + ["-c", "-o", obj, src],
+                [hipcc, f"--offload-arch={arch}", "-shared", "-fPIC", "-o", lib] + [os.path.join(csrc, o) for o in ("awsm_hip.o", "kernels_geometry.o", "kernels_post.o")] + [obj]):
+        proc = subprocess.run(cmd, stdout=subprocess.PIPE, stderr=subprocess.STDOUT, text=True)
+        if proc.returncode != 0:
+            raise RuntimeError(f"building the {name} variant failed:\n{proc.stdout[-4000:]}")
+    os.remove(obj)
+    return lib
+
+
 VGPR_BUDGETS = {"kernels_shade.o": {"k_shade_leanILb0ELi0ELb0E": 80, "k_shade_todoILi0ELb0E": 112,
                                     "k_shade_leanILb0ELi0ELb1E": 80, "k_shade_leanILb0ELi1ELb0E": 96, "k_shade_leanILb0ELi1ELb1E": 96,
                                     "k_shade_todoILi1ELb0E": 128, "k_shade_todoILi0ELb1E": 128, "k_shade_todoILi1ELb1E": 128},
diff --git a/awsm-renderer_amd/csrc/awsm_hip.cpp b/awsm-renderer_amd/csrc/awsm_hip.cpp
--- a/awsm-renderer_amd/csrc/awsm_hip.cpp
+++ b/awsm-renderer_amd/csrc/awsm_hip.cpp
@@ -65,7 +65,7 @@
     DevBuf tex_slots;
     DevBuf draw_mat;
     DevBuf tri_shade, draw_lean;
-    DevBuf clip, nrm, tan, tri_rec, tri_flags, draws_dev, draw_shade, tile_count, tile_offset, tile_cursor, tile_order, bin_list, big_list, counters, vis;
+    DevBuf clip, nrm, tan, tri_rec, tri_edge, tri_flags, draws_dev, draw_shade, tile_count, tile_offset, tile_cursor, tile_order, bin_list, big_list, counters, vis;
     DevBuf camera;
     DevBuf scan_tmp;
     DevBuf tile_split, raster_scratch;
@@ -422,7 +422,7 @@
     f->shade_todo_cap = f->shade_todo ? (uint32_t)(c->shade_todo[c->slot].size / 4 - 4 - 1024) : 0u;
     f->lean_next = f->shade_todo ? f->shade_todo + 4 + f->shade_todo_cap : nullptr;
     f->lean_grid = c->lean_grid;
-    f->tri_rec = (TriRec*)FB(c).tri_rec.ptr;
+    f->tri_rec = (TriRec*)FB(c).tri_rec.ptr; f->tri_edge = (TriEdgeInt*)FB(c).tri_edge.ptr;
     f->tile_count = (uint32_t*)FB(c).tile_count.ptr; f->tile_offset = (uint32_t*)FB(c).tile_offset.ptr;
     f->tile_cursor = (uint32_t*)FB(c).tile_cursor.ptr; f->bin_list = (uint32_t*)FB(c).bin_list.ptr;
     f->tile_order = (uint32_t*)FB(c).tile_order.ptr;
@@ -671,7 +671,7 @@
     f->clip = (float4*)t.clip.ptr; f->nrm = (float4*)t.nrm.ptr; f->tan = (float4*)t.tan.ptr; f->wpos = (float4*)t.wpos.ptr;
     f->tri_info = (uint32_t*)t.tri_flags.ptr;
     f->tri_shade = nullptr; f->draw_lean = nullptr; f->shade_todo = nullptr; f->shade_todo_cap = 0; f->lean_next = nullptr; f->lean_grid = 0;
-    f->tri_rec = (TriRec*)t.tri_rec.ptr;
+    f->tri_rec = (TriRec*)t.tri_rec.ptr; f->tri_edge = (TriEdgeInt*)t.tri_edge.ptr;
     f->tile_count = (uint32_t*)t.tile_count.ptr; f->tile_offset = (uint32_t*)t.tile_offset.ptr;
     f->tile_cursor = (uint32_t*)t.tile_cursor.ptr; f->bin_list = (uint32_t*)t.bin_list.ptr;
     f->tile_order = (uint32_t*)t.tile_order.ptr;
@@ -815,6 +815,7 @@
     if (!forward && (rc = dev_reserve(c, b.draw_lean, nd * sizeof(LeanDrawDev)))) return rc;
     if ((rc = dev_reserve(c, b.big_list, nt * 4))) return rc;
     if ((rc = dev_reserve(c, b.tri_rec, nt * kTriRecBytes))) return rc;
+    if ((rc = dev_reserve(c, b.tri_edge, nt * kTriEdgeIntBytes))) return rc;
     const uint32_t tiles_x = (c->width + kTile - 1) / kTile, tiles_y_full = (c->height + kTile - 1) / kTile;
     const size_t n_tiles_full = (size_t)tiles_x * tiles_y_full;
     if ((rc = dev_reserve(c, b.tile_count, n_tiles_full * 4))) return rc;
@@ -1001,7 +1002,7 @@
     for (auto& b : c->display8) fr(b); fr(c->effects16); fr(c->bloom_a); fr(c->bloom_b); fr(c->dof_lc); fr(c->dof_blur);
     for (int k = 0; k < 4 * kSlots; k++) {
         FrameBufs& b = k < kSlots ? c->fb[k] : (k < 2 * kSlots ? c->tr[k - kSlots] : (k < 3 * kSlots ? c->hud[k - 2 * kSlots] : c->htr[k - 3 * kSlots]));
-        fr(b.vis); fr(b.wpos); fr(b.frag_rec); fr(b.frag_color); fr(b.frag_first); fr(b.tex_slots); fr(b.draw_mat); fr(b.clip); fr(b.nrm); fr(b.tan); fr(b.tri_rec); fr(b.tri_flags); fr(b.tri_shade); fr(b.draw_lean); fr(b.draws_dev); fr(b.draw_shade); fr(b.tile_count); fr(b.tile_offset);
+        fr(b.vis); fr(b.wpos); fr(b.frag_rec); fr(b.frag_color); fr(b.frag_first); fr(b.tex_slots); fr(b.draw_mat); fr(b.clip); fr(b.nrm); fr(b.tan); fr(b.tri_rec); fr(b.tri_edge); fr(b.tri_flags); fr(b.tri_shade); fr(b.draw_lean); fr(b.draws_dev); fr(b.draw_shade); fr(b.tile_count); fr(b.tile_offset);
         fr(b.wcache); fr(b.draws_prev); fr(b.cache_mark); fr(b.block_map); fr(b.tile_cursor); fr(b.tile_order); fr(b.scan_tmp); fr(b.tile_split); fr(b.raster_scratch); fr(b.bin_list); fr(b.big_list); fr(b.counters); fr(b.camera);
     }
     for (hipStream_t st : c->shade_streams) if (st) (void)hipStreamDestroy(st);
@@ -1365,7 +1366,7 @@
     f.clip = (float4*)hb.clip.ptr; f.nrm = (float4*)hb.nrm.ptr; f.tan = (float4*)hb.tan.ptr;
     f.tri_info = (uint32_t*)hb.tri_flags.ptr;
     f.tri_shade = nullptr; f.draw_lean = nullptr;
-    f.tri_rec = (TriRec*)hb.tri_rec.ptr;
+    f.tri_rec = (TriRec*)hb.tri_rec.ptr; f.tri_edge = (TriEdgeInt*)hb.tri_edge.ptr;
     }
     f.tile_count = (uint32_t*)hb.tile_count.ptr; f.tile_offset = (uint32_t*)hb.tile_offset.ptr;
     f.tile_cursor = (uint32_t*)hb.tile_cursor.ptr; f.bin_list = (uint32_t*)hb.bin_list.ptr;
@@ -1416,7 +1417,7 @@
         for (DrawDev d : c->hud_draws_host) { d.first_tri += c->total_tris; d.first_block += c->n_blocks; c->hud_combined.push_back(d); }
         if (c->hud_combined.size() >= (1u << 24)) return fail(c, AWSM_ERR_UNSUPPORTED, "hud_geometry_pass: more than 2^24 draws in the frame");
         FrameBufs& wb = FB(c);
-        const void* before[3] = {wb.clip.ptr, wb.tri_rec.ptr, wb.tri_flags.ptr};
+        const void* before[4] = {wb.clip.ptr, wb.tri_rec.ptr, wb.tri_flags.ptr, wb.tri_edge.ptr};
         if ((rc = ensure_pass_capacity(c, wb, c->hud_combined, c->total_tris + c->hud_total_tris, false))) return rc;
         if ((rc = upload_draw_list(c, wb, c->draws_host, true))) return rc;
         {
@@ -1431,7 +1432,7 @@
             }
         }
         if ((rc = dev_reserve(c, c->merged_vis[c->slot], px * 8 * spp))) return rc;
-        if (before[0] != wb.clip.ptr || before[1] != wb.tri_rec.ptr || before[2] != wb.tri_flags.ptr) {
+        if (before[0] != wb.clip.ptr || before[1] != wb.tri_rec.ptr || before[2] != wb.tri_flags.ptr || before[3] != wb.tri_edge.ptr) {
             if ((rc = enqueue_geometry(c, true))) return rc;
         }
         c->hud_merged = true;
diff --git a/awsm-renderer_amd/csrc/frame_params.hpp b/awsm-renderer_amd/csrc/frame_params.hpp
--- a/awsm-renderer_amd/csrc/frame_params.hpp
+++ b/awsm-renderer_amd/csrc/frame_params.hpp
@@ -105,6 +105,8 @@
 
 struct TriRec;
 constexpr size_t kTriRecBytes = 80;
+struct TriEdgeInt;
+constexpr size_t kTriEdgeIntBytes = 32;
 constexpr uint32_t kMaxDirtyRanges = 12;
 
 struct FrameDev {
@@ -150,6 +152,7 @@
     uint32_t n_dirty;
     uint32_t dirty[12][3];
     TriRec* tri_rec;
+    TriEdgeInt* tri_edge;
     uint32_t* tri_info;
     uint4* tri_shade;
     uint32_t attr_data_bytes;
diff --git a/awsm-renderer_amd/csrc/kernels_geometry.hip b/awsm-renderer_amd/csrc/kernels_geometry.hip
--- a/awsm-renderer_amd/csrc/kernels_geometry.hip
+++ b/awsm-renderer_amd/csrc/kernels_geometry.hip
@@ -270,6 +270,15 @@
                 if (!b.ok) { b.t.minx = 0; b.t.maxx = 0; b.t.miny = 0; b.t.maxy = 0; }
                 tri_rec_store(f.tri_rec + r, b.t, b.ok);
             }
+#ifndef AWSM_NO_INT_EDGES
+            if (f.tri_edge) {
+                TriEdgeInt ei;
+                tri_edge_int_make(b.t, b.ok && !outside, ei);
+                uint4* q = reinterpret_cast<uint4*>(f.tri_edge + r);
+                q[0] = make_uint4((uint32_t)ei.e[0], (uint32_t)ei.e[1], (uint32_t)ei.e[2], ei.ab[0]);
+                q[1] = make_uint4(ei.ab[1], ei.ab[2], ei.org, ei.valid);
+            }
+#endif
         } else {
             b.ok = tri_rec_load(f.tri_rec + r, b.t);
         }
diff --git a/awsm-renderer_amd/csrc/kernels_shade.hip b/awsm-renderer_amd/csrc/kernels_shade.hip
--- a/awsm-renderer_amd/csrc/kernels_shade.hip
+++ b/awsm-renderer_amd/csrc/kernels_shade.hip
@@ -13,13 +13,13 @@
     float bx, by;
     f4 bary_derivs;
 };
+struct EdgeF { float e0, e1, e2; };
+AWSM_DI EdgeF edges_f(const TriSetup& t, double X, double Y) { const EdgeVals ev = tri_edges_d(t, X, Y); return {(float)ev.E[0], (float)ev.E[1], (float)ev.E[2]}; }
 template <bool DERIVS>
-AWSM_DI GBufferTexel reconstruct_core(const TriSetup& t, float4 n0, float4 n1, float4 n2, float4 t0, float4 t1, float4 t2, int cx, int cy) {
+AWSM_DI GBufferTexel reconstruct_from_edges(const float iw[3], float4 n0, float4 n1, float4 n2, float4 t0, float4 t1, float4 t2, int cx, int cy, EdgeF ec, EdgeF eh, EdgeF ew) {
     GBufferTexel g;
     g.bary_derivs = {0.0f, 0.0f, 0.0f, 0.0f};
-    const double Xc = sample_coord((cx << 8) + 128), Yc = sample_coord((cy << 8) + 128);
-    const EdgeVals ev = tri_edges_d(t, Xc, Yc);
-    const float e0 = (float)ev.E[0] * t.iw[0], e1 = (float)ev.E[1] * t.iw[1], e2 = (float)ev.E[2] * t.iw[2];
+    const float e0 = ec.e0 * iw[0], e1 = ec.e1 * iw[1], e2 = ec.e2 * iw[2];
     const float inv_esum = 1.0f / ((e0 + e1) + e2);
     const float b0 = e0 * inv_esum, b1 = e1 * inv_esum, b2 = e2 * inv_esum;
     const f3 Ni = {(b0 * n0.x + b1 * n1.x) + b2 * n2.x, (b0 * n0.y + b1 * n1.y) + b2 * n2.y, (b0 * n0.z + b1 * n1.z) + b2 * n2.z};
@@ -30,9 +30,8 @@
     g.bx = round_f16(b0);
     g.by = round_f16(b1);
     if (DERIVS) {
-        const EdgeVals eh = tri_edges_d(t, sample_coord(((cx ^ 1) << 8) + 128), Yc), evv = tri_edges_d(t, Xc, sample_coord(((cy ^ 1) << 8) + 128));
-        const float h0 = (float)eh.E[0] * t.iw[0], h1 = (float)eh.E[1] * t.iw[1], h2 = (float)eh.E[2] * t.iw[2];
-        const float w0 = (float)evv.E[0] * t.iw[0], w1 = (float)evv.E[1] * t.iw[1], w2 = (float)evv.E[2] * t.iw[2];
+        const float h0 = eh.e0 * iw[0], h1 = eh.e1 * iw[1], h2 = eh.e2 * iw[2];
+        const float w0 = ew.e0 * iw[0], w1 = ew.e1 * iw[1], w2 = ew.e2 * iw[2];
         const float ish = 1.0f / ((h0 + h1) + h2), isv = 1.0f / ((w0 + w1) + w2);
         const float hb0 = h0 * ish, hb1 = h1 * ish, vb0 = w0 * isv, vb1 = w1 * isv;
         const float ddx0 = (cx & 1) ? b0 - hb0 : hb0 - b0, ddx1 = (cx & 1) ? b1 - hb1 : hb1 - b1;
@@ -40,6 +39,14 @@
         g.bary_derivs = {round_f16(ddx0), round_f16(ddy0), round_f16(ddx1), round_f16(ddy1)};
     }
     return g;
+}
+template <bool DERIVS>
+AWSM_DI GBufferTexel reconstruct_core(const TriSetup& t, float4 n0, float4 n1, float4 n2, float4 t0, float4 t1, float4 t2, int cx, int cy) {
+    const double Xc = sample_coord((cx << 8) + 128), Yc = sample_coord((cy << 8) + 128);
+    const EdgeF ec = edges_f(t, Xc, Yc);
+    EdgeF eh = ec, ew = ec;
+    if (DERIVS) { eh = edges_f(t, sample_coord(((cx ^ 1) << 8) + 128), Yc); ew = edges_f(t, Xc, sample_coord(((cy ^ 1) << 8) + 128)); }
+    return reconstruct_from_edges<DERIVS>(t.iw, n0, n1, n2, t0, t1, t2, cx, cy, ec, eh, ew);
 }
 template <bool DERIVS>
 AWSM_DI GBufferTexel reconstruct_gbuffer(const FrameDev& f, uint32_t rank, int cx, int cy) {
@@ -1690,7 +1697,12 @@
 #ifndef AWSM_LEAN_SLOTS
 #define AWSM_LEAN_SLOTS 16u
 #endif
-constexpr uint32_t kLeanSlots = AWSM_LEAN_SLOTS, kLeanChunks = 13u, kLeanNone = 0xFFFFFFFFu;
+#ifndef AWSM_NO_INT_EDGES
+constexpr uint32_t kLeanChunks = 15u;
+#else
+constexpr uint32_t kLeanChunks = 13u;
+#endif
+constexpr uint32_t kLeanSlots = AWSM_LEAN_SLOTS, kLeanNone = 0xFFFFFFFFu;
 struct LeanStage { uint4 q[kLeanSlots][kLeanChunks]; };
 #define AWSM_AS3 __attribute__((address_space(3)))
 AWSM_DI float4 bits_float4(uint4 v) { return make_float4(__uint_as_float(v.x), __uint_as_float(v.y), __uint_as_float(v.z), __uint_as_float(v.w)); }
@@ -1713,6 +1725,28 @@
         t.t10 = gload<uint32_t>(x.base, j0 << sh); t.t11 = gload<uint32_t>(x.base, j1 << sh);
     }
 }
+#ifndef AWSM_NO_SHARED_TEXCOORDS
+struct TexCoords { uint32_t o0, o1, i0b; float fx, fy; bool wrap; };
+AWSM_DI void texcoords_s(uint32_t lw, uint32_t lh, float u, float v, TexCoords& c) {
+    const float xf = __builtin_amdgcn_ldexpf(u, (int)lw) - 0.5f, yf = __builtin_amdgcn_ldexpf(v, (int)lh) - 0.5f;
+    const float flx = floorf(xf), fly = floorf(yf);
+    c.fx = xf - flx; c.fy = yf - fly;
+    const uint32_t xi = (uint32_t)(int)flx, yi = (uint32_t)(int)fly;
+    const uint32_t i0 = __builtin_amdgcn_ubfe(xi, 0u, lw), j0 = __builtin_amdgcn_ubfe(yi, 0u, lh), j1 = __builtin_amdgcn_ubfe(yi + 1u, 0u, lh);
+    const uint32_t sh = lw + 2u;
+    c.i0b = i0 << 2;
+    c.o0 = (j0 << sh) | c.i0b; c.o1 = (j1 << sh) | c.i0b;
+    c.wrap = __builtin_amdgcn_ubfe(xi + 1u, 0u, lw) == 0u;
+}
+AWSM_DI void fetch_at(const void* base, const TexCoords& c, Tap& t) {
+    const u32x2a4 p0 = gload<u32x2a4>(base, c.o0), p1 = gload<u32x2a4>(base, c.o1);
+    t.fx = c.fx; t.fy = c.fy;
+    t.t00 = p0.x; t.t10 = p0.y; t.t01 = p1.x; t.t11 = p1.y;
+    if (c.wrap) {
+        t.t10 = gload<uint32_t>(base, c.o0 ^ c.i0b); t.t11 = gload<uint32_t>(base, c.o1 ^ c.i0b);
+    }
+}
+#endif
 template <typename BASE> struct TexGT { BASE base; uint32_t lw, levels, layer, layers; };
 typedef TexGT<const void*> TexG;
 typedef TexGT<unsigned long long> TexGL;
@@ -1898,6 +1932,9 @@
         const unsigned long long rec = (unsigned long long)f.tri_rec, nr = (unsigned long long)f.nrm, tn = (unsigned long long)f.tan, tsh = (unsigned long long)f.tri_shade;
         src_base = j < 5u ? rec + j * 16u : (j < 8u ? nr + (j - 5u) * 16u : (j < 11u ? tn + (j - 8u) * 16u : tsh + (j - 11u) * 16u));
         src_stride = j < 5u ? (uint32_t)kTriRecBytes : (j < 11u ? 48u : 32u);
+#ifndef AWSM_NO_INT_EDGES
+        if (j >= 13u) { src_base = (unsigned long long)f.tri_edge + (j - 13u) * 16u; src_stride = (uint32_t)kTriEdgeIntBytes; }
+#endif
     }
     uint32_t my_slot = kLeanNone, n_slots = 0u;
     while (rem != 0ull && n_slots < kLeanSlots) {
@@ -1916,8 +1953,14 @@
     raw.q0 = bits_float4(rec[0]); raw.q1 = bits_float4(rec[1]); raw.q2 = bits_float4(rec[2]); raw.d3 = bits_double2(rec[3]); raw.d4 = bits_double2(rec[4]);
     float4 n0 = bits_float4(rec[5]), n1 = bits_float4(rec[6]), n2 = bits_float4(rec[7]);
     float4 t0 = bits_float4(rec[8]), t1 = bits_float4(rec[9]), t2 = bits_float4(rec[10]);
+#ifndef AWSM_NO_INT_EDGES
+    uint4 ei0 = rec[13], ei1 = rec[14];
+#endif
     if (hit && !staged) {
         ts0 = as_uint4(gload<u32x4>(f.tri_shade, rank << 5)); ts1 = as_uint4(gload<u32x4>(f.tri_shade, (rank << 5) + 16u));
+#ifndef AWSM_NO_INT_EDGES
+        ei0 = as_uint4(gload<u32x4>(f.tri_edge, rank << 5)); ei1 = as_uint4(gload<u32x4>(f.tri_edge, (rank << 5) + 16u));
+#endif
         const uint32_t ro = rank * (uint32_t)kTriRecBytes, vo = rank * 48u;
         raw.q0 = as_float4(gload<f32x4>(f.tri_rec, ro)); raw.q1 = as_float4(gload<f32x4>(f.tri_rec, ro + 16u)); raw.q2 = as_float4(gload<f32x4>(f.tri_rec, ro + 32u));
         { const f64x2 a = gload<f64x2>(f.tri_rec, ro + 48u), c = gload<f64x2>(f.tri_rec, ro + 64u); raw.d3 = make_double2(a.x, a.y); raw.d4 = make_double2(c.x, c.y); }
@@ -1928,7 +1971,29 @@
     asm volatile("; MARK strict");
     TriSetup t;
     tri_rec_unpack(raw, t);
+#ifndef AWSM_NO_INT_EDGES
+    EdgeF ec, eh, ew;
+    constexpr bool kIntEdges = GRAD == 0 && !MSAA && !ITEMS;
+    if (kIntEdges && __builtin_amdgcn_ballot_w64(hit && ei1.w == 0u) == 0ull) {
+        const int dx = cx - (int)(ei1.z & 0xFFFFu), dy = cy - (int)(ei1.z >> 16);
+        const uint32_t sc0 = tri_edge_int_step(dx, dy);
+        ec = {(float)tri_edge_int_at((int)ei0.x, ei0.w, sc0), (float)tri_edge_int_at((int)ei0.y, ei1.x, sc0), (float)tri_edge_int_at((int)ei0.z, ei1.y, sc0)};
+        eh = ec; ew = ec;
+        if (GRAD != 0) {
+            const uint32_t sh = tri_edge_int_step((cx ^ 1) - (int)(ei1.z & 0xFFFFu), dy), sv = tri_edge_int_step(dx, (cy ^ 1) - (int)(ei1.z >> 16));
+            eh = {(float)tri_edge_int_at((int)ei0.x, ei0.w, sh), (float)tri_edge_int_at((int)ei0.y, ei1.x, sh), (float)tri_edge_int_at((int)ei0.z, ei1.y, sh)};
+            ew = {(float)tri_edge_int_at((int)ei0.x, ei0.w, sv), (float)tri_edge_int_at((int)ei0.y, ei1.x, sv), (float)tri_edge_int_at((int)ei0.z, ei1.y, sv)};
+        }
+    } else {
+        const double Xc = sample_coord((cx << 8) + 128), Yc = sample_coord((cy << 8) + 128);
+        ec = edges_f(t, Xc, Yc);
+        eh = ec; ew = ec;
+        if (GRAD != 0) { eh = edges_f(t, sample_coord(((cx ^ 1) << 8) + 128), Yc); ew = edges_f(t, Xc, sample_coord(((cy ^ 1) << 8) + 128)); }
+    }
+    const GBufferTexel g = reconstruct_from_edges<(GRAD != 0)>(t.iw, n0, n1, n2, t0, t1, t2, cx, cy, ec, eh, ew);
+#else
     const GBufferTexel g = reconstruct_core<(GRAD != 0)>(t, n0, n1, n2, t0, t1, t2, cx, cy);
+#endif
     if (MSAA && hit) f.msaa_cells[pv] = make_uint2(oct_word(mk2(g.packed_nt.x, g.packed_nt.y)), key.y);
     const float bz = (1.0f - g.bx) - g.by;
     float u = interp3_strict(g.bx, g.by, bz, __uint_as_float(ts0.z), __uint_as_float(ts1.x), __uint_as_float(ts1.z));
@@ -2008,11 +2073,40 @@
                 if (ex & 8u) lean::fetch_trilinear(lean::decode_g(G3.x, G3.y, G3.z, G3.w), m2e, uu, vv, tg3);
                 if (ex & 16u) lean::fetch_trilinear(lean::decode_g(G4.x, G4.y, G4.z, G4.w), m2e, uu, vv, tg4);
             } else {
+#ifndef AWSM_NO_SHARED_TEXCOORDS
+                constexpr uint32_t kNoExtent = 0x100u;
+                const uint32_t xk[5] = {(L3.y >> 16) & 0xFFu, (L3.w >> 16) & 0xFFu, (L4.y >> 16) & 0xFFu, (L4.w >> 16) & 0xFFu, (L5.y >> 16) & 0xFFu};
+                const uint32_t exu = exs & tex_mask;
+                uint32_t kA = kNoExtent, kB = kNoExtent, kC = kNoExtent;
+#pragma unroll
+                for (uint32_t k = 0; k < 5u; k++) {
+                    if (!(exu & (1u << k))) continue;
+                    if (kA == kNoExtent) kA = xk[k];
+                    else if (xk[k] != kA) {
+                        if (kB == kNoExtent) kB = xk[k];
+                        else if (xk[k] != kB && kC == kNoExtent) kC = xk[k];
+                    }
+                }
+                lean::TexCoords cA, cB, cC;
+                if (kA != kNoExtent) lean::texcoords_s(kA & 15u, kA >> 4, uu, vv, cA);
+                if (kB != kNoExtent) lean::texcoords_s(kB & 15u, kB >> 4, uu, vv, cB);
+                if (kC != kNoExtent) lean::texcoords_s(kC & 15u, kC >> 4, uu, vv, cC);
+                auto fetch_k = [&](uint32_t k, uint32_t lo_w, uint32_t hi_w, lean::Tap& tp) {
+                    if (!(ex & (1u << k))) return;
+                    const lean::TexS x = lean::decode_s(lo_w, hi_w);
+                    if (xk[k] == kA) lean::fetch_at(x.base, cA, tp);
+                    else if (xk[k] == kB) lean::fetch_at(x.base, cB, tp);
+                    else if (xk[k] == kC) lean::fetch_at(x.base, cC, tp);
+                    else lean::fetch_s(x, uu, vv, tp);
+                };
+                fetch_k(0u, L3.x, L3.y, tp0); fetch_k(1u, L3.z, L3.w, tp1); fetch_k(2u, L4.x, L4.y, tp2); fetch_k(3u, L4.z, L4.w, tp3); fetch_k(4u, L5.x, L5.y, tp4);
+#else
                 if (ex & 1u) lean::fetch_s(lean::decode_s(L3.x, L3.y), uu, vv, tp0);
                 if (ex & 2u) lean::fetch_s(lean::decode_s(L3.z, L3.w), uu, vv, tp1);
                 if (ex & 4u) lean::fetch_s(lean::decode_s(L4.x, L4.y), uu, vv, tp2);
                 if (ex & 8u) lean::fetch_s(lean::decode_s(L4.z, L4.w), uu, vv, tp3);
                 if (ex & 16u) lean::fetch_s(lean::decode_s(L5.x, L5.y), uu, vv, tp4);
+#endif
             }
             exists = exs;
             if (factors) {
diff --git a/awsm-renderer_amd/csrc/raster_setup.hpp b/awsm-renderer_amd/csrc/raster_setup.hpp
--- a/awsm-renderer_amd/csrc/raster_setup.hpp
+++ b/awsm-renderer_amd/csrc/raster_setup.hpp
@@ -154,6 +154,44 @@
     for (int i = 0; i < 3; i++) r.E[i] = fma((double)t.a[i], X, fma((double)t.b[i], Y, t.c[i]));
     return r;
 }
+struct alignas(16) TriEdgeInt {
+    int32_t e[3];
+    uint32_t ab[3];
+    uint32_t org;
+    uint32_t valid;
+};
+static_assert(sizeof(TriEdgeInt) == 32, "TriEdgeInt must be 32 bytes");
+AWSM_DI void tri_edge_int_make(const TriSetup& t, bool ok, TriEdgeInt& r) {
+    r.e[0] = r.e[1] = r.e[2] = 0; r.ab[0] = r.ab[1] = r.ab[2] = 0u; r.org = 0u; r.valid = 0u;
+    if (!(ok && t.small)) return;
+    const EdgeVals ev = tri_edges_d(t, (double)t.minx + 0.5, (double)t.miny + 0.5);
+#pragma unroll
+    for (int i = 0; i < 3; i++) {
+        r.e[i] = (int32_t)ev.E[i];
+        const int32_t ai = (int32_t)(t.a[i] * 0.00390625f), bi = (int32_t)(t.b[i] * 0.00390625f);
+        r.ab[i] = ((uint32_t)ai & 0xFFFFu) | ((uint32_t)bi << 16);
+    }
+    r.org = (uint32_t)t.minx | ((uint32_t)t.miny << 16);
+    r.valid = 1u;
+}
+AWSM_DI uint32_t tri_edge_int_step(int dx, int dy) {
+#if defined(__HIP_DEVICE_COMPILE__)
+    return __builtin_amdgcn_perm((uint32_t)dy, (uint32_t)dx, 0x040C000Cu);
+#else
+    return (((uint32_t)dx & 0xFFu) << 8) | (((uint32_t)dy & 0xFFu) << 24);
+#endif
+}
+AWSM_DI int32_t tri_edge_int_at(int32_t anchor, uint32_t ab, uint32_t step) {
+#if defined(__HIP_DEVICE_COMPILE__)
+    typedef short awsm_s16x2 __attribute__((ext_vector_type(2)));
+    return __builtin_amdgcn_sdot2(__builtin_bit_cast(awsm_s16x2, ab), __builtin_bit_cast(awsm_s16x2, step), anchor, false);
+#else
+    const uint32_t pa = (uint32_t)((int32_t)(int16_t)(ab & 0xFFFFu) * (int32_t)(int16_t)(step & 0xFFFFu));
+    const uint32_t pb = (uint32_t)((int32_t)(int16_t)(ab >> 16) * (int32_t)(int16_t)(step >> 16));
+    return (int32_t)((uint32_t)anchor + pa + pb);
+#endif
+}
+
 AWSM_DI bool edge_inside(double e, float a, float b) {
     return e > 0.0 || (e == 0.0 && (a > 0.0f || (a == 0.0f && b > 0.0f)));
 }
```

Measured after the change: 3289 frames/s. 0.953x the previous value.
